# wgmath/wgmath

Hardware: AMD Instinct MI355X
Metric: gemm_tflops (higher is better)
Workload: dtype f16

## Files before the change

include/wgebra_hip.h:

```cpp
#ifndef WGEBRA_HIP_H
#define WGEBRA_HIP_H

#include <stddef.h>
#include <stdint.h>

#ifdef __cplusplus
extern "C" {
#endif

#define WGEBRA_HIP_ABI_VERSION 5

typedef enum wg_status {
    WG_OK = 0,
    WG_ERR_DIM_MISMATCH = 1,
    WG_ERR_PRECONDITION = 2,
    WG_ERR_INVALID_ARG = 3,
    WG_ERR_OUT_OF_BOUNDS = 4,
    WG_ERR_HIP = 5,
    WG_ERR_UNSUPPORTED = 6,
    WG_ERR_NO_DEVICE = 7,
    WG_ERR_WORKSPACE = 8,
    WG_ERR_ALIASED = 9
} wg_status;

typedef enum wg_dtype { WG_F32 = 0, WG_F16 = 1, WG_BF16 = 2 } wg_dtype;

typedef enum wg_gemm_variant {
    WG_GEMM = 0, WG_GEMM_FAST = 1, WG_GEMM_TR = 2, WG_GEMM_TR_FAST = 3
} wg_gemm_variant;

typedef enum wg_gemv_variant {
    WG_GEMV = 0, WG_GEMV_FAST = 1, WG_GEMV_TR = 2, WG_GEMV_TR_FAST = 3
} wg_gemv_variant;

typedef enum wg_reduce_op {
    WG_REDUCE_MIN = 0, WG_REDUCE_MAX = 1, WG_REDUCE_SUM = 2, WG_REDUCE_PROD = 3, WG_REDUCE_SQNORM = 4
} wg_reduce_op;

typedef enum wg_op_assign_variant {
    WG_OP_ADD = 0, WG_OP_SUB = 1, WG_OP_MUL = 2, WG_OP_DIV = 3, WG_OP_COPY = 4
} wg_op_assign_variant;

enum {
    WG_USAGE_MAP_READ = 1u << 0, WG_USAGE_MAP_WRITE = 1u << 1, WG_USAGE_COPY_SRC = 1u << 2,
    WG_USAGE_COPY_DST = 1u << 3, WG_USAGE_INDEX = 1u << 4, WG_USAGE_VERTEX = 1u << 5,
    WG_USAGE_UNIFORM = 1u << 6, WG_USAGE_STORAGE = 1u << 7, WG_USAGE_INDIRECT = 1u << 8,
    WG_USAGE_QUERY_RESOLVE = 1u << 9
};

typedef struct wg_view_shape {
    uint32_t size[3];
    uint32_t stride;
    uint32_t stride_mat;
    uint32_t offset;
} wg_view_shape;

typedef struct wg_ctx wg_ctx;
typedef struct wg_buf wg_buf;
typedef struct wg_cmdbuf wg_cmdbuf;
typedef struct wg_timestamps wg_timestamps;

int wg_abi_version(void);
const char *wg_last_error_string(void);
int wg_device_count(void);

int wg_ctx_create(int device, wg_ctx **out);
int wg_ctx_create_on_stream(int device, void *hip_stream, wg_ctx **out);
int wg_ctx_create_with_cu_count(int device, uint32_t cu_count, wg_ctx **out);
int wg_ctx_create_with_cu_count_one_xcd(int device, uint32_t cu_count, wg_ctx **out);
int wg_ctx_destroy(wg_ctx *ctx);
int wg_ctx_sync(wg_ctx *ctx);
int wg_ctx_device(const wg_ctx *ctx);
void *wg_ctx_stream(const wg_ctx *ctx);
int wg_ctx_device_info(const wg_ctx *ctx, char *name256, int *compute_units, int *clock_mhz, uint64_t *hbm_bytes);
int wg_ctx_mem_info(const wg_ctx *ctx, uint64_t *free_bytes, uint64_t *total_bytes);
typedef enum wg_geom_op {
    WG_GEOM_INV = 0, WG_GEOM_CHOLESKY = 1, WG_GEOM_LU = 2, WG_GEOM_QR = 3, WG_GEOM_SYM_EIGEN = 4, WG_GEOM_SVD = 5,
    WG_GEOM_ROT2 = 6, WG_GEOM_QUAT = 7, WG_GEOM_SIM2 = 8, WG_GEOM_SIM3 = 9,
    WG_GEOM_QUAT_RAW = 10, WG_GEOM_ROT2_RAW = 11, WG_GEOM_SIM2_RAW = 12, WG_GEOM_SIM3_RAW = 13, WG_GEOM_FROM = 14,
    WG_GEOM_UTILS = 15, WG_GEOM_ROT2_EXT = 16, WG_GEOM_EIGVALS2 = 17, WG_GEOM_SVD_RECOMPOSE = 18
} wg_geom_op;
int wg_geometry_apply(wg_ctx *ctx, wg_geom_op op, uint32_t dim, const wg_buf *in, wg_buf *out, uint32_t count);

int wg_debug_spin(wg_ctx *ctx, uint32_t blocks, uint32_t usec, wg_buf *start_ticks);
int wg_debug_clock_begin(wg_ctx *ctx);
int wg_debug_clock_end(wg_ctx *ctx, double *ghz_mean, double *ghz_min, double *ghz_max, double *seconds);
int wg_debug_mfma_ceiling(wg_ctx *ctx, double min_seconds, double *tflops, double *clock_ghz);
int wg_debug_take_path(wg_ctx *ctx, char *buf, size_t cap);

typedef enum wg_tuning {
    WG_TUNE_F16_TILE = 0,
    WG_TUNE_F16_SCHED = 1,
    WG_TUNE_F32_SKINNY = 2,
    WG_TUNE_F32_PANELS = 3,
    WG_TUNE_F16_BALANCE = 4,
    WG_TUNE_F32_MID = 5,
    WG_TUNE_F32_MID_SPLIT = 6,
    WG_TUNE_GEMVT_LDS = 7,
    WG_TUNE_F16_CONT = 8,
    WG_TUNE_RM_TR_NATIVE = 9,
    WG_TUNE_COUNT_ = 10
} wg_tuning;
int wg_ctx_set_tuning(wg_ctx *ctx, wg_tuning key, int value);
int wg_ctx_f16_balance_info(const wg_ctx *ctx, double *rel8, int *valid, uint32_t *updates, uint32_t *balanced_launches);
int wg_debug_f16_balance_plan(const double *rel8, uint32_t tiles, uint32_t stages, int forced, uint32_t *units, uint32_t capacity, uint32_t *nunits,
                              uint32_t *nworkgroups);
typedef struct wg_gemm16_query {
    uint32_t trans, M, N, K, nmats;
    uint32_t lda, ldb, ldc;
    uint64_t a_batch, b_batch, c_batch;
    uint32_t a_addr, b_addr, c_addr;
    float alpha, beta;
    uint32_t panels;
    uint32_t panel_cols, panel_n_main, panel_n_tail, panel_tail_cols[8];
    uint32_t cus;
    int32_t tile, sched, cont, balance;
    uint32_t uneven_xcds;
    uint32_t recording;
    uint32_t bal_valid;
    uint32_t padded;
} wg_gemm16_query;
typedef enum wg_gemm16_leaf {
    WG_GEMM16_SKINNY = 0,
    WG_GEMM16_T256X128 = 1,
    WG_GEMM16_T128 = 2,
    WG_GEMM16_M16 = 3,
    WG_GEMM16_PAD = 4,
    WG_GEMM16_GENERIC = 5,
    WG_GEMM16_UNSUPPORTED = 6
} wg_gemm16_leaf;
typedef struct wg_gemm16_plan {
    uint32_t leaf;
    uint32_t tiles_m, tiles_n;
    uint32_t nsplit, k_per_split;
    uint32_t c_stream, a_nt;
    uint64_t workspace_bytes;
    uint32_t cont;
    uint32_t queues;
    uint32_t nwg;
    uint32_t bal_eligible, bal_calib, bal_wanted;
    uint32_t tail, tail_split, tail_kps;
    uint32_t Mp, Kp, a_ok, b_ok, c_ok;
    uint32_t c_seed;
    int32_t status;
    char message[128];
} wg_gemm16_plan;
int wg_debug_gemm16_plan(const wg_gemm16_query *query, const char *prefix, wg_gemm16_plan *plan, char *tags, size_t cap, wg_gemm16_query *inner);
int wg_debug_gemm_out32_query(wg_gemm16_query *query);
typedef struct wg_gemm32_query {
    uint32_t trans, M, N, K, nmats;
    uint32_t lda, ldb, ldc;
    uint64_t a_batch, b_batch, c_batch;
    float alpha, beta;
    uint32_t cus;
    int32_t mid, mid_split, skinny, panels;
} wg_gemm32_query;
typedef enum wg_gemm32_leaf {
    WG_GEMM32_NOTHING = 0,
    WG_GEMM32_UNSUPPORTED = 1,
    WG_GEMM32_MID = 2,
    WG_GEMM32_SKINNY = 3,
    WG_GEMM32_SKINNY_PANELS = 4,
    WG_GEMM32_SKINNY_T = 5,
    WG_GEMM32_FEWROW = 6,
    WG_GEMM32_BIG = 7
} wg_gemm32_leaf;
typedef struct wg_gemm32_plan {
    uint32_t leaf;
    uint32_t bm, bn;
    uint32_t nsplit, k_per_split;
    uint32_t npanels;
    uint32_t copy_a;
    uint32_t tail_r, tail_sp, tail_kps;
    uint32_t flat_tiles;
    uint64_t workspace_bytes;
    uint64_t pad_workspace_bytes;
    int32_t status;
    char message[128];
} wg_gemm32_plan;
int wg_debug_gemm32_plan(const wg_gemm32_query *query, wg_gemm32_plan *plan, char *tags, size_t cap, wg_gemm32_query *inner);
typedef struct wg_gemv_q8_query {
    uint32_t trans;
    uint32_t rows, cols, nrhs, mats;
    uint32_t group_rows;
    uint32_t ldm, lds, ldv, ldo;
    uint64_t m_batch, s_batch, v_batch, o_batch;
    uint32_t m_addr16, v_addr16, o_addr16;
    uint32_t cus;
} wg_gemv_q8_query;
typedef enum wg_gemv_q8_leaf {
    WG_GEMV_Q8_NOTHING = 0,
    WG_GEMV_Q8_UNSUPPORTED = 1,
    WG_GEMV_Q8_T = 2,
    WG_GEMV_Q8_N = 3,
    WG_GEMV_Q8_ANY_T = 4,
    WG_GEMV_Q8_ANY_N = 5
} wg_gemv_q8_leaf;
typedef struct wg_gemv_q8_plan {
    uint32_t leaf;
    uint32_t rhs_tile, rhs_groups;
    uint32_t loads, cols;
    uint32_t nsplit, k_per_split;
    uint32_t out_per_block;
    uint32_t grid[3], block;
    uint64_t workspace_bytes;
    int32_t status;
    char message[128];
} wg_gemv_q8_plan;
int wg_debug_gemv_q8_plan(const wg_gemv_q8_query *query, wg_gemv_q8_plan *plan, char *tags, size_t cap);
typedef struct wg_gemv_q4_query {
    uint32_t trans;
    uint32_t rows, cols, nrhs, mats;
    uint32_t group_rows;
    uint32_t ldm, lds, ldv, ldo;
    uint64_t m_batch, s_batch, v_batch, o_batch;
    uint32_t m_addr16, v_addr16;
    uint32_t cus;
} wg_gemv_q4_query;
typedef enum wg_gemv_q4_leaf {
    WG_GEMV_Q4_NOTHING = 0,
    WG_GEMV_Q4_UNSUPPORTED = 1,
    WG_GEMV_Q4_T = 2,
    WG_GEMV_Q4_ANY_T = 3
} wg_gemv_q4_leaf;
typedef struct wg_gemv_q4_plan {
    uint32_t leaf;
    uint32_t rhs_tile, rhs_groups;
    uint32_t loads, cols;
    uint32_t nsplit, k_per_split;
    uint32_t out_per_block;
    uint32_t grid[3], block;
    uint64_t workspace_bytes;
    int32_t status;
    char message[128];
} wg_gemv_q4_plan;
int wg_debug_gemv_q4_plan(const wg_gemv_q4_query *query, wg_gemv_q4_plan *plan, char *tags, size_t cap);
typedef struct wg_gemm_q8_query {
    uint32_t k, outputs, n, mats;
    uint32_t group_rows;
    uint32_t x_bf16;
    uint32_t ldm, lds, ldx, ldo;
    uint64_t m_batch, s_batch, x_batch, o_batch;
    uint32_t m_addr16, x_addr16, o_addr16;
    uint32_t cus;
} wg_gemm_q8_query;
typedef enum wg_gemm_q8_leaf {
    WG_GEMM_Q8_NOTHING = 0,
    WG_GEMM_Q8_UNSUPPORTED = 1,
    WG_GEMM_Q8_MFMA = 2,
    WG_GEMM_Q8_ANY = 3
} wg_gemm_q8_leaf;
typedef struct wg_gemm_q8_plan {
    uint32_t leaf;
    uint32_t col_tiles, col_passes;
    uint32_t out_per_block;
    uint32_t nsplit, k_per_split;
    uint32_t grid[3], block;
    uint64_t workspace_bytes;
    int32_t status;
    char message[128];
} wg_gemm_q8_plan;
int wg_debug_gemm_q8_plan(const wg_gemm_q8_query *query, wg_gemm_q8_plan *plan, char *tags, size_t cap);
typedef struct wg_gemm_q8a8_query {
    uint32_t k, outputs, n, mats;
    uint32_t group_rows, x_group_rows;
    uint32_t ldm, lds, ldx, ldxs, ldo;
    uint64_t m_batch, s_batch, x_batch, xs_batch, o_batch;
    uint32_t m_addr16, x_addr16, o_addr16;
    uint32_t cus;
} wg_gemm_q8a8_query;
typedef enum wg_gemm_q8a8_leaf {
    WG_GEMM_Q8A8_NOTHING = 0,
    WG_GEMM_Q8A8_UNSUPPORTED = 1,
    WG_GEMM_Q8A8_MFMA = 2,
    WG_GEMM_Q8A8_ANY = 3
} wg_gemm_q8a8_leaf;
typedef struct wg_gemm_q8a8_plan {
    uint32_t leaf;
    uint32_t col_tiles, col_passes;
    uint32_t out_per_block;
    uint32_t nsplit, k_per_split;
    uint32_t grid[3], block;
    uint64_t workspace_bytes;
    int32_t status;
    char message[128];
} wg_gemm_q8a8_plan;
int wg_debug_gemm_q8a8_plan(const wg_gemm_q8a8_query *query, wg_gemm_q8a8_plan *plan, char *tags, size_t cap);
typedef struct wg_quantize_q8_query {
    uint32_t rows, cols, mats, group_rows, src_elem;
    uint32_t ldq, ldsrc;
    uint64_t q_batch, src_batch;
    uint32_t q_addr16, src_addr16;
} wg_quantize_q8_query;
typedef enum wg_quantize_q8_leaf {
    WG_QUANTIZE_Q8_NOTHING = 0,
    WG_QUANTIZE_Q8_UNSUPPORTED = 1,
    WG_QUANTIZE_Q8_VEC = 2,
    WG_QUANTIZE_Q8_ANY = 3
// ... 249 lines not shown
```

wgmath_amd/_lib.py:

```python
from __future__ import annotations

import ctypes
import os
import re

_PKG = os.path.dirname(os.path.abspath(__file__))
LIB_PATH = os.environ.get("WGEBRA_HIP_LIB") or os.path.join(_PKG, "libwgebra_hip.so")
HEADER_PATH = os.path.join(os.path.dirname(_PKG), "include", "wgebra_hip.h")

WG_OK, WG_ERR_DIM_MISMATCH, WG_ERR_PRECONDITION, WG_ERR_INVALID_ARG, WG_ERR_OUT_OF_BOUNDS, WG_ERR_HIP, \
    WG_ERR_UNSUPPORTED, WG_ERR_NO_DEVICE, WG_ERR_WORKSPACE, WG_ERR_ALIASED = range(10)
WG_VIEWS_OVERLAP_MAX_RUNS = 4096
WG_GATHER_RCCL, WG_GATHER_NONE, WG_GATHER_PEER_STAGED = 0, 2, 3
WG_COMM_ID_BYTES, WG_IPC_HANDLE_BYTES = 128, 96
ABI_VERSION = 5
WG_F32, WG_F16, WG_BF16 = 0, 1, 2
WG_TUNE_F16_TILE, WG_TUNE_F16_SCHED, WG_TUNE_F32_SKINNY, WG_TUNE_F32_PANELS, WG_TUNE_F16_BALANCE, WG_TUNE_F32_MID, WG_TUNE_F32_MID_SPLIT, WG_TUNE_GEMVT_LDS, WG_TUNE_F16_CONT, WG_TUNE_RM_TR_NATIVE = range(10)


class ViewShapeC(ctypes.Structure):
    _fields_ = [("size", ctypes.c_uint32 * 3), ("stride", ctypes.c_uint32), ("stride_mat", ctypes.c_uint32),
                ("offset", ctypes.c_uint32)]


assert ctypes.sizeof(ViewShapeC) == 24


class Gemm16QueryC(ctypes.Structure):
    _fields_ = ([(n, ctypes.c_uint32) for n in ("trans", "M", "N", "K", "nmats", "lda", "ldb", "ldc")]
                + [(n, ctypes.c_uint64) for n in ("a_batch", "b_batch", "c_batch")]
                + [(n, ctypes.c_uint32) for n in ("a_addr", "b_addr", "c_addr")]
                + [("alpha", ctypes.c_float), ("beta", ctypes.c_float)]
                + [(n, ctypes.c_uint32) for n in ("panels", "panel_cols", "panel_n_main", "panel_n_tail")]
                + [("panel_tail_cols", ctypes.c_uint32 * 8), ("cus", ctypes.c_uint32)]
                + [(n, ctypes.c_int32) for n in ("tile", "sched", "cont", "balance")]
                + [(n, ctypes.c_uint32) for n in ("uneven_xcds", "recording", "bal_valid", "padded")])


GEMM16_LEAVES = ("skinny", "t256x128", "t128", "m16", "pad", "generic", "unsupported")


class Gemm16PlanC(ctypes.Structure):
    _fields_ = ([(n, ctypes.c_uint32) for n in ("leaf", "tiles_m", "tiles_n", "nsplit", "k_per_split", "c_stream", "a_nt")]
                + [("workspace_bytes", ctypes.c_uint64)]
                + [(n, ctypes.c_uint32) for n in ("cont", "queues", "nwg", "bal_eligible", "bal_calib", "bal_wanted", "tail", "tail_split", "tail_kps",
                                                   "Mp", "Kp", "a_ok", "b_ok", "c_ok", "c_seed")]
                + [("status", ctypes.c_int32), ("message", ctypes.c_char * 128)])


class Gemm32QueryC(ctypes.Structure):
    _fields_ = ([(n, ctypes.c_uint32) for n in ("trans", "M", "N", "K", "nmats", "lda", "ldb", "ldc")]
                + [(n, ctypes.c_uint64) for n in ("a_batch", "b_batch", "c_batch")]
                + [("alpha", ctypes.c_float), ("beta", ctypes.c_float), ("cus", ctypes.c_uint32)]
                + [(n, ctypes.c_int32) for n in ("mid", "mid_split", "skinny", "panels")])


GEMM32_LEAVES = ("nothing", "unsupported", "mid", "skinny", "skinny_panels", "skinny_t", "fewrow", "big")


class Gemm32PlanC(ctypes.Structure):
    _fields_ = ([(n, ctypes.c_uint32) for n in ("leaf", "bm", "bn", "nsplit", "k_per_split", "npanels", "copy_a", "tail_r", "tail_sp", "tail_kps", "flat_tiles")]
                + [("workspace_bytes", ctypes.c_uint64), ("pad_workspace_bytes", ctypes.c_uint64)]
                + [("status", ctypes.c_int32), ("message", ctypes.c_char * 128)])


class GemvQ8QueryC(ctypes.Structure):
    _fields_ = ([(n, ctypes.c_uint32) for n in ("trans", "rows", "cols", "nrhs", "mats", "group_rows", "ldm", "lds", "ldv", "ldo")]
                + [(n, ctypes.c_uint64) for n in ("m_batch", "s_batch", "v_batch", "o_batch")]
                + [(n, ctypes.c_uint32) for n in ("m_addr16", "v_addr16", "o_addr16", "cus")])


GEMV_Q8_LEAVES = ("nothing", "unsupported", "t", "n", "any_t", "any_n")


class GemvQ8PlanC(ctypes.Structure):
    _fields_ = ([(n, ctypes.c_uint32) for n in ("leaf", "rhs_tile", "rhs_groups", "loads", "cols", "nsplit", "k_per_split", "out_per_block")]
                + [("grid", ctypes.c_uint32 * 3), ("block", ctypes.c_uint32), ("workspace_bytes", ctypes.c_uint64)]
                + [("status", ctypes.c_int32), ("message", ctypes.c_char * 128)])


class GemvQ4QueryC(ctypes.Structure):
    _fields_ = ([(n, ctypes.c_uint32) for n in ("trans", "rows", "cols", "nrhs", "mats", "group_rows", "ldm", "lds", "ldv", "ldo")]
                + [(n, ctypes.c_uint64) for n in ("m_batch", "s_batch", "v_batch", "o_batch")]
                + [(n, ctypes.c_uint32) for n in ("m_addr16", "v_addr16", "cus")])


GEMV_Q4_LEAVES = ("nothing", "unsupported", "t", "any_t")


class GemvQ4PlanC(ctypes.Structure):
    _fields_ = ([(n, ctypes.c_uint32) for n in ("leaf", "rhs_tile", "rhs_groups", "loads", "cols", "nsplit", "k_per_split", "out_per_block")]
                + [("grid", ctypes.c_uint32 * 3), ("block", ctypes.c_uint32), ("workspace_bytes", ctypes.c_uint64)]
                + [("status", ctypes.c_int32), ("message", ctypes.c_char * 128)])


class GemmQ8QueryC(ctypes.Structure):
    _fields_ = ([(n, ctypes.c_uint32) for n in ("k", "outputs", "n", "mats", "group_rows", "x_bf16", "ldm", "lds", "ldx", "ldo")]
                + [(n, ctypes.c_uint64) for n in ("m_batch", "s_batch", "x_batch", "o_batch")]
                + [(n, ctypes.c_uint32) for n in ("m_addr16", "x_addr16", "o_addr16", "cus")])


GEMM_Q8_LEAVES = ("nothing", "unsupported", "mfma", "any")


class GemmQ8PlanC(ctypes.Structure):
    _fields_ = ([(n, ctypes.c_uint32) for n in ("leaf", "col_tiles", "col_passes", "out_per_block", "nsplit", "k_per_split")]
                + [("grid", ctypes.c_uint32 * 3), ("block", ctypes.c_uint32), ("workspace_bytes", ctypes.c_uint64)]
                + [("status", ctypes.c_int32), ("message", ctypes.c_char * 128)])


class GemmQ8A8QueryC(ctypes.Structure):
    _fields_ = ([(n, ctypes.c_uint32) for n in ("k", "outputs", "n", "mats", "group_rows", "x_group_rows", "ldm", "lds", "ldx", "ldxs", "ldo")]
                + [(n, ctypes.c_uint64) for n in ("m_batch", "s_batch", "x_batch", "xs_batch", "o_batch")]
                + [(n, ctypes.c_uint32) for n in ("m_addr16", "x_addr16", "o_addr16", "cus")])


GEMM_Q8A8_LEAVES = ("nothing", "unsupported", "mfma", "any")


class GemmQ8A8PlanC(ctypes.Structure):
    _fields_ = ([(n, ctypes.c_uint32) for n in ("leaf", "col_tiles", "col_passes", "out_per_block", "nsplit", "k_per_split")]
                + [("grid", ctypes.c_uint32 * 3), ("block", ctypes.c_uint32), ("workspace_bytes", ctypes.c_uint64)]
                + [("status", ctypes.c_int32), ("message", ctypes.c_char * 128)])


class QuantizeQ8QueryC(ctypes.Structure):
    _fields_ = ([(n, ctypes.c_uint32) for n in ("rows", "cols", "mats", "group_rows", "src_elem", "ldq", "ldsrc")]
                + [(n, ctypes.c_uint64) for n in ("q_batch", "src_batch")]
                + [(n, ctypes.c_uint32) for n in ("q_addr16", "src_addr16")])


QUANTIZE_Q8_LEAVES = ("nothing", "unsupported", "vec", "any")


class QuantizeQ8PlanC(ctypes.Structure):
    _fields_ = ([(n, ctypes.c_uint32) for n in ("leaf", "group_lanes", "blocks_per_col")]
                + [("grid", ctypes.c_uint32 * 3), ("block", ctypes.c_uint32)]
                + [("status", ctypes.c_int32), ("message", ctypes.c_char * 128)])


class GemmQ4QueryC(ctypes.Structure):
    _fields_ = ([(n, ctypes.c_uint32) for n in ("k", "outputs", "n", "mats", "group_rows", "x_bf16", "ldm", "lds", "ldx", "ldo")]
                + [(n, ctypes.c_uint64) for n in ("m_batch", "s_batch", "x_batch", "o_batch")]
                + [(n, ctypes.c_uint32) for n in ("m_addr16", "x_addr16", "o_addr16", "cus")])


GEMM_Q4_LEAVES = ("nothing", "unsupported", "mfma", "any")


class GemmQ4PlanC(ctypes.Structure):
    _fields_ = ([(n, ctypes.c_uint32) for n in ("leaf", "step", "col_tiles", "col_passes", "out_per_block", "nsplit", "k_per_split")]
                + [("grid", ctypes.c_uint32 * 3), ("block", ctypes.c_uint32), ("workspace_bytes", ctypes.c_uint64)]
                + [("status", ctypes.c_int32), ("message", ctypes.c_char * 128)])


class GemvQueryC(ctypes.Structure):
    _fields_ = ([(n, ctypes.c_uint32) for n in ("trans", "rows_out", "k", "nrhs", "nmats", "m_elem", "v_elem", "bf16", "gemm16", "ldm", "ldv", "ldo")]
                + [(n, ctypes.c_uint64) for n in ("m_batch", "v_batch", "o_batch")]
                + [(n, ctypes.c_uint32) for n in ("m_addr16", "v_addr16", "cus")] + [("gemvt_lds", ctypes.c_int32)])


GEMV_LEAVES = ("nothing", "unsupported", "small", "n", "t", "tcols", "tlds", "as_gemm32", "as_gemm16")


class GemvPlanC(ctypes.Structure):
    _fields_ = ([(n, ctypes.c_uint32) for n in ("leaf", "rhs_tile", "rhs_groups", "e", "u", "v", "rl", "lds_cols", "lds_threads", "lds_kc", "lds_bytes", "nsplit", "k_per_split")]
                + [("grid", ctypes.c_uint32 * 3), ("block", ctypes.c_uint32), ("combine_grid", ctypes.c_uint32 * 3), ("workspace_bytes", ctypes.c_uint64)]
                + [("status", ctypes.c_int32), ("message", ctypes.c_char * 128), ("gemm32", Gemm32PlanC)])


class GemvAnyPlanC(ctypes.Structure):
    _fields_ = ([(n, ctypes.c_uint32) for n in ("launch", "nsplit", "per_split", "grid_x", "zchunk", "nchunks", "nt")] + [("workspace_bytes", ctypes.c_uint64)]
                + [("status", ctypes.c_int32), ("message", ctypes.c_char * 128), ("tag", ctypes.c_char * 48)])


class WgError(RuntimeError):

    def __init__(self, status: int, message: str):
        super().__init__(message)
        self.status = status


class DimensionMismatch(WgError, AssertionError):
    """What the reference raises as a panic from assert_eq!(..., "... dimension mismatch.")."""


class PreconditionFailed(WgError, AssertionError):
    pass


class NoDevice(WgError):
    pass


class WorkspaceMustGrow(WgError):
    """A context scratch region would have to grow inside a recording (WG_ERR_WORKSPACE): run the call once eagerly first."""


class AliasedOperands(WgError):
    """The written view of a call shares memory with a view the call reads (WG_ERR_ALIASED): nothing was launched. The reference gets a wgpu validation panic
    for binding one buffer read_write and read; here views of one buffer are legal as long as their footprints are disjoint, and OpAssign / Axpy take the
    identical view on both sides (include/wgebra_hip.h, the aliasing rule)."""


def declared_symbols(header_path: str = HEADER_PATH) -> list[str]:
    text = open(header_path).read()
    text = re.sub(r"/\*.*?\*/", "", text, flags=re.S)
    return sorted(set(re.findall(r"\b(wg_[a-z0-9_]+)\s*\(", text)))


def _load() -> ctypes.CDLL:
    if not os.path.exists(LIB_PATH):
        raise ImportError(
            f"{LIB_PATH} is missing: build it with `python -c 'import __graft_entry__ as g; g.build()'` "
            f"or `make -C wgmath_amd/csrc`. There is no CPU fallback.")
    lib = ctypes.CDLL(LIB_PATH)
    pd = ctypes.POINTER(ctypes.c_double)
    vp, cp, ci, u32, u64, sz = ctypes.c_void_p, ctypes.c_char_p, ctypes.c_int, ctypes.c_uint32, ctypes.c_uint64, ctypes.c_size_t
    pvp = ctypes.POINTER(vp)
    S = ViewShapeC
    sig = {
        "wg_abi_version": (ci, []),
        "wg_last_error_string": (cp, []),
        "wg_device_count": (ci, []),
        "wg_ctx_create": (ci, [ci, pvp]),
        "wg_ctx_create_on_stream": (ci, [ci, vp, pvp]),
        "wg_ctx_create_with_cu_count": (ci, [ci, ctypes.c_uint32, ctypes.POINTER(vp)]),
        "wg_ctx_create_with_cu_count_one_xcd": (ci, [ci, ctypes.c_uint32, ctypes.POINTER(vp)]),
        "wg_ctx_destroy": (ci, [vp]),
        "wg_ctx_sync": (ci, [vp]),
        "wg_ctx_device": (ci, [vp]),
        "wg_ctx_stream": (vp, [vp]),
        "wg_ctx_device_info": (ci, [vp, cp, ctypes.POINTER(ci), ctypes.POINTER(ci), ctypes.POINTER(u64)]),
        "wg_ctx_mem_info": (ci, [vp, ctypes.POINTER(u64), ctypes.POINTER(u64)]),
        "wg_ctx_reserve_workspace": (ci, [vp, sz]),
        "wg_debug_f16_balance_plan": (ci, [ctypes.POINTER(ctypes.c_double), u32, u32, ci, ctypes.POINTER(u32), u32, ctypes.POINTER(u32), ctypes.POINTER(u32)]),
        "wg_debug_gemm16_plan": (ci, [ctypes.POINTER(Gemm16QueryC), cp, ctypes.POINTER(Gemm16PlanC), cp, sz, ctypes.POINTER(Gemm16QueryC)]),
        "wg_debug_gemm32_plan": (ci, [ctypes.POINTER(Gemm32QueryC), ctypes.POINTER(Gemm32PlanC), cp, sz, ctypes.POINTER(Gemm32QueryC)]),
        "wg_ctx_f16_balance_info": (ci, [vp, ctypes.POINTER(ctypes.c_double), ctypes.POINTER(ci), ctypes.POINTER(u32), ctypes.POINTER(u32)]),
        "wg_debug_views_overlap": (ci, [S, u64, S, u64, u32, ctypes.POINTER(ci)]),
        "wg_debug_take_path": (ci, [vp, cp, sz]),
        "wg_ctx_set_tuning": (ci, [vp, ci, ci]),
        "wg_ctx_get_tuning": (ci, [vp, ci, ctypes.POINTER(ci)]),
        "wg_debug_spin": (ci, [vp, ctypes.c_uint32, ctypes.c_uint32, vp]),
        "wg_geometry_apply": (ci, [vp, ci, ctypes.c_uint32, vp, vp, ctypes.c_uint32]),
        "wg_buf_create": (ci, [vp, sz, u32, pvp]),
        "wg_buf_create_init": (ci, [vp, vp, sz, u32, pvp]),
        "wg_buf_wrap": (ci, [vp, vp, sz, pvp]),
        "wg_buf_destroy": (ci, [vp]),
        "wg_buf_size": (sz, [vp]),
        "wg_buf_device_ptr": (vp, [vp]),
        "wg_buf_write": (ci, [vp, vp, sz, vp, sz]),
        "wg_buf_read": (ci, [vp, vp, sz, vp, sz]),
        "wg_buf_copy": (ci, [vp, vp, sz, vp, sz, sz]),
        "wg_buf_fill_zero": (ci, [vp, vp]),
        "wg_gemm": (ci, [vp, ci, ci, vp, S, vp, S, vp, S]),
        "wg_gemm_ex": (ci, [vp, ci, ci, ctypes.c_float, ctypes.c_float, vp, S, vp, S, vp, S]),
        "wg_gemv": (ci, [vp, ci, ci, vp, S, vp, S, vp, S]),
        "wg_gemv_mixed": (ci, [vp, ci, ci, vp, S, vp, S, vp, S]),
        "wg_gemv_q8": (ci, [vp, ci, u32, vp, S, vp, S, vp, S, vp, S]),
        "wg_debug_gemv_q8_plan": (ci, [ctypes.POINTER(GemvQ8QueryC), ctypes.POINTER(GemvQ8PlanC), cp, sz]),
        "wg_gemv_q4": (ci, [vp, ci, u32, vp, S, vp, S, vp, S, vp, S]),
        "wg_debug_gemv_q4_plan": (ci, [ctypes.POINTER(GemvQ4QueryC), ctypes.POINTER(GemvQ4PlanC), cp, sz]),
        "wg_gemm_q8": (ci, [vp, ci, u32, ci, vp, S, vp, S, vp, S, vp, S]),
        "wg_debug_gemm_q8_plan": (ci, [ctypes.POINTER(GemmQ8QueryC), ctypes.POINTER(GemmQ8PlanC), cp, sz]),
        "wg_gemm_q4": (ci, [vp, ci, u32, ci, vp, S, vp, S, vp, S, vp, S]),
        "wg_debug_gemm_q4_plan": (ci, [ctypes.POINTER(GemmQ4QueryC), ctypes.POINTER(GemmQ4PlanC), cp, sz]),
        "wg_gemm_q8a8": (ci, [vp, ci, u32, u32, vp, S, vp, S, vp, S, vp, S, vp, S]),
        "wg_debug_gemm_q8a8_plan": (ci, [ctypes.POINTER(GemmQ8A8QueryC), ctypes.POINTER(GemmQ8A8PlanC), cp, sz]),
        "wg_quantize_q8": (ci, [vp, ci, u32, vp, S, vp, S, vp, S]),
        "wg_debug_quantize_q8_plan": (ci, [ctypes.POINTER(QuantizeQ8QueryC), ctypes.POINTER(QuantizeQ8PlanC)]),
        "wg_debug_gemv_plan": (ci, [ctypes.POINTER(GemvQueryC), ctypes.POINTER(GemvPlanC), cp, sz]),
        "wg_debug_gemv_any_plan": (ci, [ctypes.POINTER(GemvQueryC), ctypes.POINTER(GemvAnyPlanC), cp, sz]),
        "wg_gemm_out32": (ci, [vp, ci, ci, ctypes.c_float, ctypes.c_float, vp, S, vp, S, vp, S]),
        "wg_debug_gemm_out32_query": (ci, [ctypes.POINTER(Gemm16QueryC)]),
        "wg_gemm_rm": (ci, [vp, ci, ci, vp, S, vp, S, vp, S]),
        "wg_gemv_rm": (ci, [vp, ci, ci, vp, S, vp, S, vp, S]),
        "wg_gemv_reduce": (ci, [vp, ci, ci, ci, vp, vp, S, vp, S]),
        "wg_reduce": (ci, [vp, ci, ci, vp, S, vp]),
        "wg_reduce_fast": (ci, [vp, ci, ci, vp, S, vp]),
        "wg_reduce_batched": (ci, [vp, ci, ci, vp, S, vp]),
        "wg_op_assign": (ci, [vp, ci, ci, vp, S, vp, S]),
        "wg_axpy": (ci, [vp, ctypes.c_float, ci, vp, S, vp, S]),
        "wg_copy_view": (ci, [vp, ci, vp, S, vp, S]),
        "wg_debug_clock_begin": (ci, [vp]),
        "wg_debug_clock_end": (ci, [vp, pd, pd, pd, pd]),
        "wg_debug_mfma_ceiling": (ci, [vp, ctypes.c_double, pd, pd]),
        "wg_comm_unique_id": (ci, [vp]),
        "wg_comm_create": (ci, [vp, ci, ci, vp, pvp]),
        "wg_comm_destroy": (ci, [vp]),
        "wg_comm_rank": (ci, [vp]),
        "wg_comm_size": (ci, [vp]),
        "wg_comm_has_collectives": (ci, [vp]),
        "wg_comm_reported_size": (ci, [vp, ctypes.POINTER(ci)]),
        "wg_comm_bytes_sent": (u64, [vp]),
        "wg_all_gather": (ci, [vp, ci, vp, u64, u64]),
        "wg_comm_join": (ci, [vp]),
        "wg_comm_set_pipelined": (ci, [vp, ci]),
        "wg_comm_set_one_launch": (ci, [vp, ci]),
        "wg_comm_flush": (ci, [vp]),
        "wg_comm_barrier": (ci, [vp]),
        "wg_buf_ipc_export": (ci, [vp, vp]),
        "wg_buf_ipc_open": (ci, [vp, vp, pvp]),
        "wg_comm_stage_reserve": (ci, [vp, sz, pvp, pvp]),
        "wg_comm_set_peer_stages": (ci, [vp, pvp, pvp]),
        "wg_cube_to_matrix": (ci, [vp, ci, vp, S, vp, S]),
        "wg_gemm_sharded": (ci, [vp, ci, ci, ci, u32, vp, S, vp, S, vp, S]),
        "wg_comm_set_wait_timing": (ci, [vp, ci]),
        "wg_comm_wait_times": (ci, [vp, ctypes.POINTER(u32), ctypes.POINTER(ctypes.c_float), u32, ctypes.POINTER(u32)]),
        "wg_gemm_sharded_panels": (ci, [vp, ci, ci, ci, ctypes.POINTER(u32), u32, vp, S, vp, S, vp, S]),
        "wg_encoder_begin": (ci, [vp]),
        "wg_encoder_finish": (ci, [vp, pvp]),
        "wg_queue_submit": (ci, [vp, vp]),
        "wg_cmdbuf_destroy": (ci, [vp]),
        "wg_timestamps_create": (ci, [vp, u32, pvp]),
        "wg_timestamps_destroy": (ci, [vp]),
        "wg_timestamps_clear": (ci, [vp]),
        "wg_timestamps_write": (ci, [vp, vp, ctypes.POINTER(u32)]),
        "wg_timestamps_reserve": (ci, [vp, u32, ctypes.POINTER(u32)]),
        "wg_timestamps_write_at": (ci, [vp, vp, u32]),
        "wg_timestamps_len": (u32, [vp]),
        "wg_timestamps_wait_for_results_ms": (ci, [vp, ctypes.POINTER(ctypes.c_double), u32]),
    }
    for name, (res, args) in sig.items():
        fn = getattr(lib, name)
        fn.restype = res
        fn.argtypes = args
    lib._wg_signatures = sig
    if lib.wg_abi_version() != ABI_VERSION:
        raise ImportError(f"{LIB_PATH} reports ABI version {lib.wg_abi_version()}, this binding is written for {ABI_VERSION} "
                          f"(include/wgebra_hip.h: WGEBRA_HIP_ABI_VERSION): rebuild with `make -C wgmath_amd/csrc`")
    return lib


def hip_runtime_paths() -> list[str]:
    paths = set()
    try:
        with open("/proc/self/maps") as f:
            for line in f:
                if "libamdhip64" in line:
                    paths.add(line.split()[-1])
    except OSError:
        pass
    return sorted(paths)


def assert_single_hip_runtime() -> None:
    p = hip_runtime_paths()
    if len(p) > 1:
        raise ImportError("two HIP runtimes are loaded in this process: " + ", ".join(p) +
                          ". Import torch BEFORE wgmath_amd so that libwgebra_hip.so binds to torch's bundled runtime.")


lib = _load()

_EXC = {WG_ERR_DIM_MISMATCH: DimensionMismatch, WG_ERR_PRECONDITION: PreconditionFailed, WG_ERR_NO_DEVICE: NoDevice, WG_ERR_WORKSPACE: WorkspaceMustGrow,
        WG_ERR_ALIASED: AliasedOperands}


def check(status: int) -> None:
    if status != WG_OK:
        msg = lib.wg_last_error_string().decode("utf-8", "replace")
        raise _EXC.get(status, WgError)(status, msg or f"wg_status {status}")
```

wgmath_amd/csrc/gemm16_plan.hip:

```cpp
#include "gemm16_plan.hpp"
#include "gemm_plan_common.hpp"

#include <cmath>
#include <cstdarg>
#include <cstring>
#include <string>

using wg16::BalancePlan;
using wg16::bal_decode;
using WG16_NS::BM;
using WG16_NS::BN;
using WG16_NS::BKH;
using WG16_NS::kPanelTail;

namespace {
constexpr double kBalTileOverhead = 5.0;
constexpr double kBalTakeOverhead = 8.5;
constexpr double kBalGiveOverhead = 7.0;
}

uint32_t bal_plan(const double rel[8], uint32_t tiles, uint32_t S, bool forced, BalancePlan &bp) {
    uint32_t n[8];
    double w[8], delta[8], sum_w = 0, sum_inv = 0;
    for (int x = 0; x < 8; ++x) {
        n[x] = tiles / 8u + ((uint32_t)x < tiles % 8u ? 1u : 0u);
        w[x] = ((double)S + kBalTileOverhead) * n[x] / 32.0;
        sum_w += w[x];
        sum_inv += 1.0 / rel[x];
    }
    const double T = sum_w / sum_inv;
    for (int x = 0; x < 8; ++x) delta[x] = T / rel[x] - w[x];
    double want[8], rem[8];
    for (int x = 0; x < 8; ++x) {
        want[x] = delta[x] > 0 ? delta[x] - kBalTakeOverhead : 0.0;
        rem[x] = delta[x] < 0 ? -delta[x] + kBalGiveOverhead : 0.0;
    }
    if (forced) {
        const double s = (double)S, take[8] = { s / 3, 0, s / 2, s / 4, 0, 0, s / 4, 0 }, give[8] = { 0, s / 4, 0, 0, 0, s / 2, 0, s / 2 + s / 4 };
        for (int x = 0; x < 8; ++x) want[x] = take[x], rem[x] = give[x];
    }
    uint32_t rounds_used[8] = { 0 }, max_rounds[8], pairs = 0;
    for (int x = 0; x < 8; ++x) {
        const uint32_t r = n[x] / 64u;
        max_rounds[x] = r > 2u ? 2u : r;
        if (n[x] < 64u) max_rounds[x] = n[x] >= 4u ? 2u : (n[x] >= 2u ? 1u : 0u);
        bp.len[x] = n[x];
        bp.pre_cnt[x] = 0; bp.pre_src[x] = 0; bp.pre_p[x] = bp.pre_slot[x] = bp.pre_pair0[x] = 0;
        for (int r2 = 0; r2 < 2; ++r2) bp.suf_lo[x][r2] = bp.suf_p[x][r2] = bp.suf_pair0[x][r2] = 0, bp.suf_cnt[x][r2] = 0;
    }
    bool taken[8] = { false };
    for (;;) {
        int f = -1;
        for (int x = 0; x < 8; ++x)
            if (!taken[x] && want[x] >= 3.0 && (f < 0 || want[x] > want[f])) f = x;
        if (f < 0) break;
        taken[f] = true;
        int g = -1;
        for (int x = 0; x < 8; ++x)
            if (rem[x] >= 3.0 && rounds_used[x] < max_rounds[x] && (g < 0 || rem[x] > rem[g])) g = x;
        if (g < 0) break;
        double pd = want[f];
        if (pd > rem[g]) pd = rem[g];
        uint32_t p = (uint32_t)(pd + 0.5);
        if (p + 3u > S) p = S - 3u;
        if (p < 3u) continue;
        if (!forced && (double)p < kBalGiveOverhead + 1.0) continue;
        const uint32_t round = n[g] >= 64u ? 32u : (n[g] >= 4u ? n[g] / 4u : 1u);
        const uint32_t cnt = round < 32u ? round : 32u;
        const uint32_t lo = n[g] - round * (rounds_used[g] + 1u);
        if (pairs + cnt > kBalMaxPairs) break;
        bp.pre_cnt[f] = cnt; bp.pre_src[f] = (uint32_t)g; bp.pre_p[f] = p; bp.pre_slot[f] = lo; bp.pre_pair0[f] = pairs;
        bp.len[f] = n[f] + cnt;
        const uint32_t r2 = rounds_used[g]++;
        bp.suf_lo[g][r2] = lo; bp.suf_cnt[g][r2] = cnt; bp.suf_p[g][r2] = p; bp.suf_pair0[g][r2] = pairs;
        pairs += cnt;
        rem[g] -= (double)p;
    }
    return pairs;
}

uint32_t gemm16_c_stream(const wg_gemm16_query &q, uint32_t out_elem_bytes) {
#ifdef WG_FORCE_C_STREAM
    return WG_FORCE_C_STREAM;
#endif
    const uint64_t MiB = 1ull << 20, ab = ((uint64_t)q.M * q.K + (uint64_t)q.K * q.N) * q.nmats * 2u, cb = (uint64_t)q.M * q.N * q.nmats * out_elem_bytes;
    return (q.beta == 0.f && ab <= 256u * MiB && ab + cb > 256u * MiB) ? 1u : 0u;
}

wg_gemm16_query gemm16_out32_query(wg_gemm16_query q) {
    q.cont = 0;
    q.panels = 0; q.panel_cols = q.panel_n_main = q.panel_n_tail = 0;
    for (int t = 0; t < 8; ++t) q.panel_tail_cols[t] = 0;
    return q;
}

namespace {
wg_gemm16_plan no_launch(wg_gemm16_plan p, int status, const char *fmt = nullptr, ...) {
    p.leaf = WG_GEMM16_UNSUPPORTED;
    p.status = status;
    if (fmt) {
        va_list ap;
        va_start(ap, fmt);
        vsnprintf(p.message, sizeof p.message, fmt, ap);
        va_end(ap);
    }
    return p;
}
uint64_t pad_elems(uint64_t elems) { return (elems + 7u) & ~7ull; }
}

wg_gemm16_plan gemm16_plan(const wg_gemm16_query &q) {
    wg_gemm16_plan p = {};
    p.nsplit = 1; p.tail_split = 1;
    const bool trans = q.trans != 0, panels = q.panels != 0;
    const uint32_t M = q.M, N = q.N, K = q.K, nmats = q.nmats, out_ld = q.ldc;
    const uint64_t out_batch = q.c_batch;
    const struct { uint32_t ld; uint64_t batch; uint32_t addr; } m1 = { q.lda, q.a_batch, q.a_addr }, m2 = { q.ldb, q.b_batch, q.b_addr };
    const float alpha = q.alpha, beta = q.beta;
    const int cus = (int)q.cus;
    p.k_per_split = K; p.tail_kps = K;
    if (M == 0 || N == 0 || nmats == 0) return no_launch(p, panels ? WG_ERR_UNSUPPORTED : WG_OK);
    if (nmats > 65535) return no_launch(p, WG_ERR_UNSUPPORTED, "Gemm: more than 65535 matrices in one call");
    {
        const uint64_t MiB = 1ull << 20;
        p.c_stream = gemm16_c_stream(q, 2u);
        p.a_nt = (!trans && N <= 128u && (uint64_t)M * K * 2u >= 384u * MiB) ? 1u : 0u;
    }
    auto al16 = [](uint32_t addr) { return (addr & 15) == 0; };
#ifndef WG_F16_SKINNY
#define WG_F16_SKINNY 1
#endif
    if (WG_F16_SKINNY && trans && !panels && N <= 16u && M >= 512u && M % 4u == 0 && K >= 256u && K % 8u == 0 && m1.ld % 8u == 0 && m2.ld % 8u == 0 &&
        out_ld % 4u == 0 && al16(m1.addr) && al16(m2.addr) && (q.c_addr & 7) == 0 && (nmats == 1 || (m1.batch % 8u == 0 && m2.batch % 8u == 0 && out_batch % 4u == 0)) &&
        (uint64_t)M * K * 2u >= (16ull << 20) && (uint64_t)m1.ld * 32u * 2u < (1ull << 31) && (uint64_t)m2.ld * 32u * 2u < (1ull << 31)) {
        const uint32_t row_blocks = (M + 127u) / 128u;
        uint32_t kps;
        const uint32_t ns = wg_skinny_kcut(M, N, K, nmats, (uint64_t)row_blocks * nmats, (uint64_t)cus, 256u, 64u, 0, &kps);
        if (ns > 65535u || nmats > 65535u) return no_launch(p, WG_ERR_UNSUPPORTED, "Gemm: too many splits or matrices for the skinny path");
        p.leaf = WG_GEMM16_SKINNY;
        p.tiles_m = row_blocks; p.tiles_n = 1;
        p.nsplit = ns; p.k_per_split = kps;
        if (ns > 1) p.workspace_bytes = (uint64_t)ns * M * N * nmats * sizeof(float);
        return p;
    }
    const bool off_ok = (uint64_t)m1.ld * 2u * (trans ? 256u : 32u) < (1ull << 31) && (uint64_t)m2.ld * 2u * 256u < (1ull << 31);
    const uint32_t krem = K % 64u;
    const bool k_big = K % 8u == 0 && K - krem >= 192u, k_small = K % 8u == 0 && K - krem >= 64u;
    const bool a_step_fits = trans || (uint64_t)m1.ld * 64u < (1ull << 32);
    auto al4 = [](uint32_t addr) { return (addr & 3) == 0; };
    const bool a_al = al4(m1.addr) && m1.ld % 2 == 0 && (nmats == 1 || m1.batch % 2 == 0), b_al = al4(m2.addr) && m2.ld % 2 == 0 && (nmats == 1 || m2.batch % 2 == 0);
    const bool fast = (M % 8 == 0) && (k_big || k_small) && a_step_fits && off_ok && a_al && b_al;
    auto panels_ok = [&]() -> bool {
        if (!q.panel_cols || q.panel_cols % 256u || q.panel_n_tail < 1 || q.panel_n_tail > (uint32_t)kPanelTail || q.panel_n_main + q.panel_n_tail < 2) return false;
        uint64_t c0 = (uint64_t)q.panel_n_main * q.panel_cols;
        for (uint32_t t = 0; t + 1u < q.panel_n_tail; ++t) {
            if (q.panel_tail_cols[t] == 0 || q.panel_tail_cols[t] % 256u || q.panel_tail_cols[t] / 256u > 255u) return false;
            c0 += q.panel_tail_cols[t];
        }
        return c0 < N && N - c0 == q.panel_tail_cols[q.panel_n_tail - 1u] && (N - c0 + 255u) / 256u <= 255u;
    };
    if (panels && !(fast && k_big && nmats == 1 && alpha == 1.f && beta == 0.f && panels_ok() &&
                    (uint64_t)((M + BM - 1) / BM) * ((N + BN - 1) / BN) >= (uint64_t)cus))
        return no_launch(p, WG_ERR_UNSUPPORTED);
    if (fast) {
        p.tiles_m = (M + BM - 1) / BM;
        p.tiles_n = (N + BN - 1) / BN;
        const uint64_t tiles = (uint64_t)p.tiles_m * p.tiles_n;
        if (tiles > 0x7fffffffull) return no_launch(p, WG_ERR_UNSUPPORTED, "Gemm: too many tiles");
        bool t256x128 = q.tile == 256128;
        const bool cont_shape = !panels && krem == 0 && K >= 256u && K <= 4096u && tiles * nmats > (uint64_t)cus && beta == 0.f &&
                                q.cont != 0 && q.sched < 0 && q.balance != 1;
        if (q.tile == 0 && !panels && tiles * nmats >= (uint64_t)cus && K <= 1536u) {
            double t_big = (double)((tiles * nmats + cus - 1) / cus) * (12.3 + 0.0213 * K);
            if (cont_shape) {
                const double per = 5.7 + 0.0211 * K;
                const uint64_t all = tiles * nmats;
                const uint32_t r = (uint32_t)(all % (uint64_t)cus);
                t_big = 5.0 + (double)(all / (uint64_t)cus) * per + (r == 0 ? 0.0 : (2u * r <= (uint32_t)cus && K >= 384u && nmats == 1 ? 25.0 + 0.0107 * K : per));
            }
            const double r2 = (double)((uint64_t)((M + 255u) / 256u) * ((N + 127u) / 128u) * nmats) / (2.0 * cus), fl = floor(r2), fr = r2 - fl;
            const double pair = trans ? 5.7 + 0.027 * K : 6.1 + 0.0263 * K;
            t256x128 = fl * pair + (fr > 0.0 ? (fr <= 0.5 ? 0.6 : 1.0) * pair : 0.0) < 0.95 * t_big;
        }
        if (q.tile == 0 && !panels && nmats <= 2u && tiles * nmats < (uint64_t)cus && K >= 512u && K <= 4096u) {
            const uint64_t tt = (uint64_t)((M + 255u) / 256u) * ((N + 127u) / 128u) * nmats;
            if (tt <= (uint64_t)cus && 10u * tt >= 7u * (uint64_t)cus) t256x128 = true;
        }
        if ((krem == 0 || K - krem >= 64u) && !panels && t256x128) {
            const uint32_t tm = (M + 255u) / 256u, tn = (N + 127u) / 128u;
            const uint64_t tiles_t = (uint64_t)tm * tn;
            if (tiles_t <= 0x7fffffffull && nmats <= 65535u) {
                p.leaf = WG_GEMM16_T256X128;
                p.tiles_m = tm; p.tiles_n = tn;
                return p;
            }
        }
        if ((krem == 0 || K - krem >= 64u) && !panels) {
            const double out_bytes = (double)M * N * nmats * 4.0;
            auto slabs = [&](uint32_t ns) { return ns > 1 ? wg_slab_write_us(ns * out_bytes) + wg_slab_reduce_us(ns * out_bytes) : 0.0; };
            const uint32_t tm = (M + 127u) / 128u, tn = (N + 127u) / 128u;
            const uint64_t tiles128 = (uint64_t)tm * tn;
            uint32_t ns = 1;
            if (tiles128 * nmats * 2u <= (uint64_t)cus) {
                ns = (uint32_t)((uint64_t)cus / (tiles128 * nmats));
                if (ns > K / 1024u) ns = K / 1024u;
                while (ns > 1 && (double)ns * out_bytes > (double)(512ull << 20)) --ns;
                if (ns < 2) ns = 1;
            }
#ifdef WG_T128_FORCE_NS
            if (tiles128 * nmats <= (uint64_t)cus && K >= 1024u) ns = WG_T128_FORCE_NS;
#endif
            bool want128 = false;
            if (!k_big) want128 = true;
            else if (q.tile) want128 = q.tile == 128;
            else if (N <= 64u) want128 = true;
            else if (tiles * nmats < (uint64_t)cus) {
                const double w128 = (double)(tiles128 * nmats * ns) / cus, k128 = (double)(((K / 64u + ns - 1) / ns) * 64u);
                const double est128 = (w128 <= 1.0 ? k128 * 0.00875 : w128 * k128 * 0.0108) + 6.0 + slabs(ns);
                const uint32_t ns256 = wg_splitk_plan(tiles * nmats, (uint32_t)cus, K / BKH, 8, (uint64_t)M * N * nmats, 512ull << 20);
                const double k256 = (double)(((K / BKH + ns256 - 1) / ns256) * BKH);
                const double est256 = (ns256 <= 4u ? 0.8 : 1.0) * ((double)((tiles * nmats * ns256 + cus - 1) / cus) * (k256 * 0.0234 + 8.0) + slabs(ns256));
                want128 = est128 < est256;
            }
            if (want128 && tiles128 <= 0x7fffffffull) {
                const uint32_t kps = ns > 1 ? ((K / 64u + ns - 1) / ns) * 64u : K;
                if (ns > 1) ns = (K - krem + kps - 1) / kps;
                if ((uint64_t)nmats * ns <= 65535) {
                    p.leaf = WG_GEMM16_T128;
                    p.tiles_m = tm; p.tiles_n = tn;
                    p.nsplit = ns; p.k_per_split = kps;
                    if (ns > 1) p.workspace_bytes = (uint64_t)ns * M * N * nmats * sizeof(float);
                    return p;
                }
            }
        }
        if (!k_big) return no_launch(p, WG_ERR_UNSUPPORTED, "Gemm: K = %u with %u matrices does not fit the 128 x 128 kernel's launch", K, nmats);
        uint32_t nsplit = panels ? 1u : wg_splitk_plan(tiles * nmats, (uint32_t)cus, K / BKH, 8, (uint64_t)M * N * nmats, 512ull << 20);
        const uint32_t stages = K / 64u;
        auto kps_of = [&](uint32_t ns) { return ((stages + ns - 1u) / ns) * 64u; };
        while (nsplit > 1) {
            const uint32_t kps = kps_of(nsplit), n = (K - krem + kps - 1u) / kps;
            if (n == nsplit && kps >= 192u && K - krem - (n - 1u) * kps >= 192u) break;
            nsplit = n < nsplit ? n : nsplit - 1u;
        }
        p.leaf = WG_GEMM16_M16;
        p.nsplit = nsplit;
        p.k_per_split = nsplit > 1 ? kps_of(nsplit) : K;
        if (nsplit > 1) p.workspace_bytes = (uint64_t)nsplit * M * N * nmats * sizeof(float);
        if ((uint64_t)nmats * nsplit > 65535) return no_launch(p, WG_ERR_UNSUPPORTED, "Gemm: nmats * splits exceeds 65535");
        uint32_t tail = 0, tail_split = 1, tail_kps = K;
#ifndef WG_F16_TAIL_SPLIT
#define WG_F16_TAIL_SPLIT 1
#endif
        if (WG_F16_TAIL_SPLIT && nsplit == 1 && nmats == 1 && tiles > (uint64_t)cus && !panels) {
            const uint32_t r = (uint32_t)(tiles % (uint64_t)cus);
            if (r > 0 && r * 2u <= (uint32_t)cus) {
                uint32_t sp = (uint32_t)cus / r;
                if (sp > stages / 3u) sp = stages / 3u;
                while (sp >= 2) {
                    const uint32_t kps = ((stages + sp - 1) / sp) * 64u;
                    const uint32_t n = (K - krem + kps - 1) / kps, last = K - krem - (n - 1) * kps;
                    if (n >= 2 && last >= 192u && (size_t)n * r * 65536u * sizeof(float) <= (512ull << 20)) { tail = r; tail_split = n; tail_kps = kps; break; }
                    --sp;
                }
            }
        }
        p.tail = tail; p.tail_split = tail_split; p.tail_kps = tail_kps;
        if (tail) p.workspace_bytes = (uint64_t)tail_split * tail * 65536u * sizeof(float);
#ifndef WG_F16_SCHED_ROUNDS
#define WG_F16_SCHED_ROUNDS 16
#endif
        const uint32_t ntiles = (uint32_t)tiles - tail;
        p.nwg = ntiles;
        const int sched_env = q.sched;
        {
            const int cont = q.cont;
            const uint64_t all = (uint64_t)ntiles * nmats;
            const bool applies = nsplit == 1 && !panels && krem == 0 && K >= 256u && all > (uint64_t)cus && all <= 0x7fffffffull && beta == 0.f;
            const bool by_rule = (K <= 4096u || (K <= 8192u && all < (uint64_t)(WG_F16_SCHED_ROUNDS * cus))) && !q.uneven_xcds && sched_env < 0 && q.balance != 1;
            if (cont != 0 && applies && (cont == 1 || by_rule)) {
                p.cont = 1;
                p.nwg = (uint32_t)cus;
                return p;
            }
        }
        const bool dyn = nsplit == 1 && nmats == 1 && (sched_env >= 0 ? sched_env != 0 : ntiles >= (uint32_t)((q.uneven_xcds ? 2 : WG_F16_SCHED_ROUNDS) * cus));
        if (dyn) {
            p.queues = 1;
            p.nwg = (ntiles + ntiles / 8u + 7u) & ~7u;
        }
        const int bal_knob = q.balance;
        const uint32_t S = K / 64u;
        if (bal_knob != 0 && !dyn && !panels && nsplit == 1 && nmats == 1 && cus == 256 && ntiles >= 16u && ntiles < 8u * 65535u && S >= 8u) {
            p.bal_eligible = 1;
            p.bal_calib = ntiles >= (uint32_t)cus;
            const bool want = bal_knob == 1 || (bal_knob < 0 && q.bal_valid && ntiles >= 2u * (uint32_t)cus);
            p.bal_wanted = want && !q.recording;
        }
        return p;
    } else if (!q.padded && (uint64_t)M * N * K >= (1ull << 24) && K > 0 && nmats <= 65535u) {
        const bool k_ok = k_big || k_small;
        const uint32_t Mp = (M + 7u) & ~7u, Kp = k_ok ? K : ((K + 63u) & ~63u);
        const bool a_ok = k_ok && M == Mp && a_al;
        const bool b_ok = k_ok && b_al;
        const bool c_ok = M == Mp;
        const uint64_t a_elems = a_ok ? 0 : (uint64_t)Mp * Kp, b_elems = b_ok ? 0 : (uint64_t)Kp * N, c_elems = c_ok ? 0 : (uint64_t)Mp * N;
        const uint64_t a_sz = pad_elems(a_elems), b_sz = pad_elems(b_elems), c_sz = pad_elems(c_elems);
        p.leaf = WG_GEMM16_PAD;
        p.Mp = Mp; p.Kp = Kp; p.a_ok = a_ok; p.b_ok = b_ok; p.c_ok = c_ok;
        p.c_seed = !c_ok && beta != 0.f;
        p.workspace_bytes = (a_sz + b_sz + c_sz) * nmats * 2u + 16;
        return p;
    } else {
        p.leaf = WG_GEMM16_GENERIC;
        p.tiles_m = (M + 63) / 64;
        p.tiles_n = (N + 63) / 64;
        if (p.tiles_n > 65535) return no_launch(p, WG_ERR_UNSUPPORTED, "Gemm: N too large for the generic f16 path");
        return p;
    }
}

wg_gemm16_query gemm16_pad_inner(const wg_gemm16_query &q, const wg_gemm16_plan &p) {
    wg_gemm16_query in = q;
    in.padded = 1;
    in.M = p.Mp; in.K = p.Kp;
    if (!p.a_ok) { in.lda = q.trans ? p.Kp : p.Mp; in.a_batch = pad_elems((uint64_t)p.Mp * p.Kp); in.a_addr = 0; }
    if (!p.b_ok) { in.ldb = p.Kp; in.b_batch = pad_elems((uint64_t)p.Kp * q.N); in.b_addr = 0; }
    if (!p.c_ok) { in.ldc = p.Mp; in.c_batch = pad_elems((uint64_t)p.Mp * q.N); in.c_addr = 0; }
    return in;
}

Gemm16Tags gemm16_tags(const wg_gemm16_plan &p, const char *prefix, bool bal_on) {
    Gemm16Tags t = {};
    auto add = [&](const char *fmt, auto... a) { snprintf(t.tag[t.n++], sizeof t.tag[0], fmt, prefix, a...); };
    switch (p.leaf) {
    case WG_GEMM16_SKINNY: add("%s.skinny/ns=%u", p.nsplit); break;
    case WG_GEMM16_T256X128: add("%s.t256x128"); break;
    case WG_GEMM16_T128: add("%s.t128/ns=%u", p.nsplit); break;
    case WG_GEMM16_M16:
        if (p.cont) add("%s.cont");
        else add("%s.m16%s/ns=%u", bal_on ? "bal" : p.queues ? "q" : "", p.nsplit);
        if (p.tail) { add("%s.m16tail/ns=%u", p.tail_split); add("%s.tail_reduce"); }
        break;
    case WG_GEMM16_PAD: add("%s.pad%s>", p.c_ok ? "" : p.c_seed ? "/c=seed" : "/c"); break;
    case WG_GEMM16_GENERIC: add("%s.generic"); break;
    default: break;
    }
    return t;
}

extern "C" int wg_debug_f16_balance_plan(const double *rel8, uint32_t tiles, uint32_t stages, int forced, uint32_t *units, uint32_t capacity, uint32_t *nunits,
                                          uint32_t *nworkgroups) {
    if (!rel8 || !nunits || (capacity && !units)) return wg_set_error(WG_ERR_INVALID_ARG, "wg_debug_f16_balance_plan: NULL argument");
    BalancePlan bp = BalancePlan{};
    const uint32_t pairs = bal_plan(rel8, tiles, stages, forced != 0, bp);
    (void)pairs;
    uint32_t mx = 0, n = 0;
    for (int x = 0; x < 8; ++x) mx = bp.len[x] > mx ? bp.len[x] : mx;
    for (uint32_t b = 0; b < 8u * mx; ++b) {
        uint32_t tile, mode, kb, ns, pair;
        if (!bal_decode(bp, b, stages, tile, mode, kb, ns, pair)) continue;
        if (n < capacity) { units[5 * n] = tile; units[5 * n + 1] = mode; units[5 * n + 2] = kb; units[5 * n + 3] = mode ? ns : stages; units[5 * n + 4] = pair; }
        ++n;
    }
    *nunits = n;
    if (nworkgroups) *nworkgroups = 8u * mx;
    return WG_OK;
}

extern "C" int wg_debug_gemm16_plan(const wg_gemm16_query *query, const char *prefix, wg_gemm16_plan *plan, char *tags, size_t cap, wg_gemm16_query *inner) {
    if (!query || !prefix || !plan || (cap && !tags)) return wg_set_error(WG_ERR_INVALID_ARG, "wg_debug_gemm16_plan: NULL argument");
    *plan = gemm16_plan(*query);
    if (inner) *inner = plan->leaf == WG_GEMM16_PAD ? gemm16_pad_inner(*query, *plan) : *query;
    std::string log;
    wg_gemm16_query q = *query;
    for (wg_gemm16_plan p = *plan;; p = gemm16_plan(q)) {
        bool bal_on = false;
        if (p.leaf == WG_GEMM16_M16 && p.bal_wanted) {
            const double flat[8] = { 1, 1, 1, 1, 1, 1, 1, 1 };
            BalancePlan bp = BalancePlan{};
            bal_on = bal_plan(flat, p.nwg, q.K / 64u, q.balance == 1, bp) != 0;
        }
        const Gemm16Tags t = gemm16_tags(p, prefix, bal_on);
        for (int i = 0; i < t.n; ++i) {
            if (!log.empty() && log.back() != '>') log += ' ';
            log += t.tag[i];
        }
        if (p.leaf != WG_GEMM16_PAD) {
            if (p.nsplit > 1) log += " splitk.reduce/ns=" + std::to_string(p.nsplit);
            break;
        }
        q = gemm16_pad_inner(q, p);
    }
    if (cap) snprintf(tags, cap, "%s", log.c_str());
    return WG_OK;
}

extern "C" int wg_debug_gemm_out32_query(wg_gemm16_query *query) {
    if (!query) return wg_set_error(WG_ERR_INVALID_ARG, "wg_debug_gemm_out32_query: NULL argument");
    *query = gemm16_out32_query(*query);
    return WG_OK;
}

extern "C" int wg_ctx_f16_balance_info(const wg_ctx *ctx, double *rel8, int *valid, uint32_t *updates, uint32_t *balanced_launches) {
    if (!ctx) return wg_set_error(WG_ERR_INVALID_ARG, "wg_ctx_f16_balance_info: ctx is NULL");
    if (rel8) for (int x = 0; x < 8; ++x) rel8[x] = ctx->bal.rel[x];
    if (valid) *valid = ctx->bal.valid ? 1 : 0;
    if (updates) *updates = ctx->bal.updates;
    if (balanced_launches) *balanced_launches = ctx->bal.epoch;
    return WG_OK;
}
```

wgmath_amd/csrc/gemm_f16.hip:

```cpp
#include "gemm_f16_common.hpp"
#include "gemm16_plan.hpp"

namespace WG16_NS {
namespace {

#ifndef WG_NN_KEEP
#define WG_NN_KEEP 16
#endif
#ifndef WG_NN_DSTRIDE
#define WG_NN_DSTRIDE 8
#endif
#ifndef WG_NN_DOFF
#define WG_NN_DOFF 3
#endif
#ifndef WG_NN_SYNC_SLOT
#define WG_NN_SYNC_SLOT 60
#endif
#ifndef WG_TN_SYNC_SLOT
#define WG_TN_SYNC_SLOT 56
#endif
#ifndef WG_F16_UNPEELED
#define WG_F16_UNPEELED 1
#endif
#ifndef WG_NN_STAGED
#define WG_NN_STAGED 0
#endif
typedef float floatx4 __attribute__((ext_vector_type(4)));
typedef unsigned uintx2 __attribute__((ext_vector_type(2)));
typedef unsigned uintx4 __attribute__((ext_vector_type(4)));
typedef uintx4 __attribute__((aligned(2))) uintx4_u;

template <class F, int... I>
__device__ __forceinline__ void static_for_impl(F &&f, std::integer_sequence<int, I...>) { (f(std::integral_constant<int, I>{}), ...); }
template <int N, class F>
__device__ __forceinline__ void static_for(F &&f) { static_for_impl(f, std::make_integer_sequence<int, N>{}); }

constexpr int M16_A_RING = 4, M16_B_RING = 3;
constexpr int M16_BS_BYTES = BN * 64 * 2;
constexpr int M16_B_BASE = M16_A_RING * HA_BYTES;
static_assert(M16_B_BASE + M16_B_RING * M16_BS_BYTES == 160 * 1024, "LDS plan");

__device__ __forceinline__ void m16_set_m0(uint32_t lds_dst) {
    if (WG_ABLATE & 2) return;
    asm volatile("s_mov_b32 m0, %0" ::"s"(lds_dst));
}
#ifndef WG_F16_DMA_MUBUF
#define WG_F16_DMA_MUBUF 0
#endif
template <int IMM>
__device__ __forceinline__ void m16_dma_imm(uint32_t voff, const void *sbase) {
    if (WG_ABLATE & 2) return;
    if constexpr (WG_F16_DMA_MUBUF) {
        const uintx4 srd = { (uint32_t)(uintptr_t)sbase, (uint32_t)((uintptr_t)sbase >> 32) & 0xffffu, 0xffffffffu, 0x00020000u };
        asm volatile("buffer_load_dwordx4 %0, %1, 0 offen offset:%c2 lds" ::"v"(voff), "s"(srd), "i"(IMM));
    } else {
        asm volatile("global_load_lds_dwordx4 %0, %1 offset:%c2" ::"v"(voff), "s"(sbase), "i"(IMM));
    }
}
__device__ __forceinline__ void m16_dma(int q, uint32_t voff, const void *sbase) {
    if (q == 0) m16_dma_imm<0>(voff, sbase);
    else if (q == 1) m16_dma_imm<1024>(voff, sbase);
    else if (q == 2) m16_dma_imm<2048>(voff, sbase);
    else m16_dma_imm<3072>(voff, sbase);
}
constexpr uint32_t M16_BIAS = 3072;

template <bool TRANS_A>
__device__ __forceinline__ void m16_tile(const GemmArgs &g, const uint32_t bid, char *const smem, const uint32_t unit_mode = 0, uint32_t unit_kb = 0,
                                         uint32_t unit_ns = 0, const uint32_t unit_pair = 0) {
    const int lane = threadIdx.x & 63;
    const int wave = __builtin_amdgcn_readfirstlane(threadIdx.x >> 6);
    const int wm = wave >> 1, wn = wave & 1;
    const int i16 = lane & 15, kg = lane >> 4;
    const int aq = i16 >> 2, bb = i16 & 3;
    const int gq = (4 - aq) & 3;

#ifdef WG_F16_TRACE
    uint64_t tr_t[5];
    tr_t[0] = __builtin_amdgcn_s_memrealtime();
#define WG_TRACE_POINT(i) do { asm volatile("s_waitcnt lgkmcnt(0)" ::: "memory"); tr_t[i] = __builtin_amdgcn_s_memrealtime(); } while (0)
#else
#define WG_TRACE_POINT(i) do { } while (0)
#endif
#if defined(WG_F16_TRACE) && WG_F16_TRACE >= 2
    uint32_t q_a = 0, q_b = 0, q_c = 0, q_d = 0, s_vm = 0, s_bar = 0, s_probe = 0, m_vm = 0, m_bar = 0, n_adv = 0, loop_t0 = 0, loop_t1 = 0;
#endif
    uint32_t tm, tn, panel = 0;
    uint32_t panel_c0 = 0, panel_np = 0;
    if (g.panel.cols) {
        const uint32_t id = bid + g.tile_base;
        const uint32_t mtn = g.panel.cols / 256u, main_tiles = g.panel.n_main * g.panel.tiles;
        uint32_t loc, ptn, tn0;
        if (id < main_tiles) {
            panel = __builtin_amdgcn_readfirstlane(id / g.panel.tiles);
            loc = id - panel * g.panel.tiles; ptn = mtn; tn0 = panel * mtn;
        } else {
            loc = __builtin_amdgcn_readfirstlane(id - main_tiles);
            tn0 = g.panel.n_main * mtn;
            const uint32_t n_tail = g.panel.npanels - g.panel.n_main;
            uint32_t q = 0;
            uint64_t tail = g.panel.tail_tn;
            ptn = (uint32_t)tail & 0xffu;
            while (q + 1u < n_tail && loc >= g.tiles_m * ptn) { loc -= g.tiles_m * ptn; tn0 += ptn; ++q; tail >>= 8; ptn = (uint32_t)tail & 0xffu; }
            panel = g.panel.n_main + q;
        }
        tile_of(loc, g.tiles_m, ptn, tm, tn);
        tn += tn0;
        panel_c0 = tn0 * 256u;
        panel_np = panel + 1u == g.panel.npanels ? g.N - panel_c0 : ptn * 256u;
    } else tile_of(bid + g.tile_base, g.tiles_m, g.tiles_n, tm, tn);
    panel = __builtin_amdgcn_readfirstlane(panel);
    panel_c0 = __builtin_amdgcn_readfirstlane(panel_c0); panel_np = __builtin_amdgcn_readfirstlane(panel_np);
    tm = __builtin_amdgcn_readfirstlane(tm); tn = __builtin_amdgcn_readfirstlane(tn);
    const uint32_t m0 = tm * BM, n0 = tn * BN;
    const uint32_t z = blockIdx.y / g.nsplit, split = blockIdx.y % g.nsplit;
    uint32_t k_begin = split * g.k_per_split;
    uint32_t K_loc = split + 1u == g.nsplit ? g.K - k_begin : g.k_per_split;
    bool from_partial = false;
    if (unit_mode == 2) {
        if (threadIdx.x == 0) {
            const uint64_t t0 = __builtin_amdgcn_s_memrealtime();
            uint32_t ok = 1;
            while (__hip_atomic_load(g.bal.flags + unit_pair, __ATOMIC_RELAXED, __HIP_MEMORY_SCOPE_SYSTEM) != g.bal.epoch) {
                __builtin_amdgcn_s_sleep(16);
                if (__builtin_amdgcn_s_memrealtime() - t0 > 100000ull) { ok = 0; break; }
            }
            __builtin_amdgcn_fence(__ATOMIC_ACQUIRE, "agent");
            *reinterpret_cast<volatile uint32_t *>(smem) = ok;
        }
        __syncthreads();
        from_partial = __builtin_amdgcn_readfirstlane(*reinterpret_cast<volatile uint32_t *>(smem)) != 0;
        __syncthreads();
    }
    uint32_t rem = 0, rem_k0 = 0;
    if (unit_mode == 1) { k_begin = 0; K_loc = unit_ns * 64u; rem = g.K & 63u; rem_k0 = g.K - rem; }
    else if (unit_mode == 2 && from_partial) { k_begin = unit_kb * 64u; K_loc = (g.K & ~63u) - k_begin; }
    else {
        if (unit_mode == 2) { k_begin = 0; K_loc = g.K; }
        rem = K_loc & 63u; K_loc -= rem; rem_k0 = k_begin + K_loc;
    }
    const wg16_elem_t *A = g.a + z * g.a_batch + (TRANS_A ? (uint64_t)k_begin : (uint64_t)k_begin * g.lda);
    const wg16_elem_t *B = g.b + z * g.b_batch + k_begin;
    wg16_out_t *C = g.c + z * g.c_batch;
    const bool paneled = !kOut32 && g.panel.cols != 0;
    if (paneled) {
        const uint64_t off = (uint64_t)panel_c0 * (g.panel.col_stride - g.ldc) + g.panel.slot_rows * (uint64_t)panel_np - g.panel.slot_rows * (uint64_t)g.panel.cols;
        C += ((uint64_t)(uint32_t)__builtin_amdgcn_readfirstlane((int)(uint32_t)(off >> 32)) << 32) | (uint32_t)__builtin_amdgcn_readfirstlane((int)(uint32_t)off);
    }
    uint32_t *panel_counter = g.panel.counters + panel;
    float *part = unit_mode ? g.bal.part + (uint64_t)unit_pair * 65536u : g.part;
    float alpha = g.alpha, beta = g.beta;
    uint32_t ldc = g.ldc, c_stream = g.c_stream;
    uint32_t *bal_flag = g.bal.flags + unit_pair;
    uint32_t bal_epoch = g.bal.epoch;
    unsigned long long *calib = g.calib;
    asm volatile("" : "+s"(C), "+s"(part), "+s"(alpha), "+s"(beta), "+s"(ldc), "+s"(c_stream), "+s"(bal_flag), "+s"(bal_epoch), "+s"(calib));

    uint32_t a_voff[TRANS_A ? 8 : 4], b_voff[8];
    const wg16_elem_t *a_base, *b_base = B + (uint64_t)n0 * g.ldb;
    if constexpr (TRANS_A) a_base = A + (uint64_t)m0 * g.lda; else a_base = A + m0;
    const uint32_t rem_dk = rem_k0 - k_begin;
    const char *rem_a = TRANS_A ? (const char *)(a_base + rem_dk) : (const char *)(a_base + (uint64_t)rem_dk * g.lda);
    const char *rem_b = (const char *)(b_base + rem_dk);
    if (rem) {
        if constexpr (TRANS_A) a_base -= 64; else a_base -= (uint64_t)64u * g.lda;
        b_base -= 64;
    }
    if constexpr (TRANS_A) {
#pragma unroll
        for (int q = 0; q < 8; ++q) {
            const uint32_t P = 8u * wave + q;
            const uint32_t row = 8u * P + (lane >> 3);
            const uint32_t f = ((4u - ((row >> 3) & 3u)) & 3u) | (((row >> 1) & 1u) << 2);
            const uint32_t chunk = (lane & 7u) ^ f;
            const uint32_t ra = min(row, g.M - 1u - m0);
            a_voff[q] = (ra * g.lda + 8u * chunk) * 2u + (M16_BIAS - 1024u * (q & 3));
        }
    } else {
#pragma unroll
        for (int q = 0; q < 4; ++q) {
            const uint32_t P = 4u * wave + q;
            const uint32_t unit = WG_NN_NOSWAP ? (lane & 3u) ^ ((uint32_t)wave & 1u) : (lane & 3u);
            const uint32_t mpiece = min(128u * (P & 1) + 32u * (lane >> 4) + 8u * unit, g.M - 8u - m0);
            a_voff[q] = ((4u * (P >> 1) + ((lane >> 2) & 3)) * g.lda + mpiece) * 2u + (M16_BIAS - 1024u * q);
        }
    }
#pragma unroll
    for (int q = 0; q < 8; ++q) {
        const uint32_t P = 8u * wave + q;
        const uint32_t row = 8u * P + (lane >> 3);
        const uint32_t f = ((4u - ((row >> 2) & 3u)) & 3u) | (((row >> 1) & 1u) << 2);
        const uint32_t chunk = (lane & 7u) ^ f;
        const uint32_t rb = min(row, g.N - 1u - n0);
        b_voff[q] = (rb * g.ldb + 8u * chunk) * 2u + (M16_BIAS - 1024u * (q & 3));
    }
    const uint32_t lds_base = (uint32_t)(uintptr_t)(WG_AS3 char *)smem;
    const uint32_t lds_a_wave = __builtin_amdgcn_readfirstlane(lds_base + wave * (TRANS_A ? 8192 : 4096));
    const uint32_t lds_b_wave = __builtin_amdgcn_readfirstlane(lds_base + M16_B_BASE + wave * 8192);
    auto a_src = [&](uint32_t H) -> const wg16_elem_t * {
        const char *p0;
        if constexpr (TRANS_A) p0 = (const char *)(a_base + H * 64u); else p0 = (const char *)(a_base + (uint64_t)(H * BKH) * g.lda);
        return (const wg16_elem_t *)(p0 - M16_BIAS);
    };
    auto b_src = [&](uint32_t stage) -> const wg16_elem_t * { return (const wg16_elem_t *)((const char *)(b_base + 64u * stage) - M16_BIAS); };

    uint32_t vbaseA[2], vbaseB[2];
    uint32_t vbaseA1 = 0;
#pragma unroll
    for (int hs = 0; hs < 2; ++hs) {
        const uint32_t chunk = (uint32_t)(((kg ^ gq) | ((hs ^ (bb >> 1)) << 2)) * 16);
        vbaseB[hs] = lds_base + M16_B_BASE + ((uint32_t)128 * wn + i16) * 128u + chunk;
        if constexpr (TRANS_A) vbaseA[hs] = lds_base + (128u * wm + 8u * aq + bb) * 128u + chunk;
    }
    if constexpr (!TRANS_A) {
        if constexpr (WG_NN_NOSWAP) {
            const uint32_t a = (uint32_t)i16 & 3u, krow = (uint32_t)i16 >> 2;
            const uint32_t common = lds_base + (uint32_t)kg * 4096u + (4u * wm) * 256u + krow * 64u + (a ^ ((uint32_t)kg & 1u)) * 16u;
            vbaseA[0] = common + (a & 1u) * 8u;
            vbaseA1 = common + ((a & 1u) ^ 1u) * 8u;
        } else {
            vbaseA[0] = lds_base + (uint32_t)((kg & 2) * 2) * 2048u + (4u * wm) * 256u + (uint32_t)i16 * 16u + (uint32_t)(kg & 1) * 8u;
        }
        vbaseA[1] = vbaseA[0] + HA_BYTES;
    }
    const bool odd_row = !TRANS_A && WG_NN_NOSWAP && (kg & 1);

    floatx4 acc[8][8];
#pragma unroll
    for (int t = 0; t < 8; ++t)
#pragma unroll
        for (int u = 0; u < 8; ++u)
#pragma unroll
            for (int e = 0; e < 4; ++e) acc[t][u][e] = 0.f;
    if (from_partial) {
        const uint32_t pvoff = ((128u * wn + i16) * 256u + 128u * wm + 8u * kg) * 4u;
        const uint32_t pv_even = pvoff + (odd_row ? 16u : 0u), pv_odd = pvoff + (odd_row ? 0u : 16u);
#pragma unroll
        for (int u = 0; u < 8; ++u) {
            const uint32_t vo0 = pv_even + (uint32_t)u * 16384u, vo1 = pv_odd + (uint32_t)u * 16384u;
#pragma unroll
            for (int p = 0; p < 4; ++p) {
                asm volatile("global_load_dwordx4 %0, %1, %2 offset:%c3 sc0 sc1" : "=a"(acc[2 * p][u]) : "v"(vo0), "s"(part), "i"(p * 128));
                asm volatile("global_load_dwordx4 %0, %1, %2 offset:%c3 sc0 sc1" : "=a"(acc[2 * p + 1][u]) : "v"(vo1), "s"(part), "i"(p * 128));
            }
        }
        asm volatile("s_waitcnt vmcnt(0)" ::: "memory");
    }

    uintx4 a_r[2][8];
    half8_t b_f[2][8];

    using c0 = std::integral_constant<int, 0>;
    using c1 = std::integral_constant<int, 1>;
    using yes = std::true_type;
    using no = std::false_type;
    using km1 = std::integral_constant<int, -1>;
    using km2 = std::integral_constant<int, -2>;
    using k0 = std::integral_constant<int, 0>;
    using k4 = std::integral_constant<int, 4>;
    using k8 = std::integral_constant<int, 8>;
    using k12 = std::integral_constant<int, 12>;
    using k16 = std::integral_constant<int, 16>;

    const uint32_t S = K_loc / 64u + (rem ? 1u : 0u);
    uint32_t st = 0;

    uint32_t va, vb;
    uint32_t va1 = 0;
    const char *ga, *gb, *ga2 = nullptr;
    uint32_t oR = 0, oD = 2u * M16_BS_BYTES;
    uint32_t rR = 1u << 14, rD = 0;
    uint32_t oA = 0, oAD = 0;
    uint32_t la = 0, lb = 0;
    const uint64_t a_step = (uint64_t)BKH * g.lda * 2u;
    constexpr bool STAGED = TRANS_A || WG_NN_STAGED;
    const uint32_t a_full = TRANS_A ? 128u : (uint32_t)a_step * (STAGED ? 2u : 1u);
    uint32_t a_inc0 = 0, a_inc1 = 0, b_inc = 0;
    auto ring3 = [](uint32_t o) -> uint32_t { o += (uint32_t)M16_BS_BYTES; return o == 3u * M16_BS_BYTES ? 0u : o; };

    constexpr int kOps = TRANS_A ? 16 : WG_NN_NOSWAP ? 24 : 40;
    auto frag = [&](int op, int set) {
        auto rb = [&](int u) { b_f[set][u] = lds_h8_at(vb + u * 2048); };
        if constexpr (TRANS_A) {
            auto ra = [&](int t) { a_r[set][t] = __builtin_bit_cast(uintx4, lds_h8_at(va + (t & 1) * 512 + (t >> 1) * 4096)); };
            if (op == 0) ra(0);
            else if (op <= 8) rb(op - 1);
            else ra(op - 8);
        } else if constexpr (WG_NN_NOSWAP) {
            auto tr = [&](int p, int i) {
                const int tb = i >> 1, h = i & 1;
                const uintx2 v = __builtin_bit_cast(uintx2, lds_tr_at((tb ? va1 : va) + h * 2048 + p * 256));
                a_r[set][2 * p + tb][2 * h] = v[0];
                a_r[set][2 * p + tb][2 * h + 1] = v[1];
            };
            if (op < 4) tr(0, op);
            else if (op < 8) rb(op - 4);
            else if (op < 12) tr(1, op - 8);
            else if (op < 16) rb(op - 8);
            else if (op < 20) tr(2, op - 16);
            else tr(3, op - 20);
        } else {
            auto tr = [&](int p, int i) {
                const int h = i >> 1, ins = i & 1;
                const uintx2 v = __builtin_bit_cast(uintx2, lds_tr_at(va + (2 * ins + h) * 2048 + p * 256));
                a_r[set][2 * p + ins][2 * h] = v[0];
                a_r[set][2 * p + ins][2 * h + 1] = v[1];
            };
// ... 130 lines not shown
                asm volatile("" : "+s"(ga2));
            }
            if constexpr (HS == 0 && j == LASTB + 1) { oR = ring3(oR); asm volatile("" : "+s"(oR)); }
            if constexpr (j == LASTB + 4) { vb = vbaseB[HS] + oR; asm volatile("" : "+v"(vb)); }
            if constexpr (HS == 0 && j == 47) { oA ^= (uint32_t)M16_BS_BYTES; asm volatile("" : "+s"(oA)); }
            if constexpr (!TRANS_A && WG_NN_NOSWAP && j == 48) { va1 = vbaseA1 + (HS ? (uint32_t)HA_BYTES : 0u) + oA; asm volatile("" : "+v"(va1)); }
            if constexpr (j == 49) { va = vbaseA[HS] + oA; asm volatile("" : "+v"(va)); }
            if constexpr (HS == 1 && j == 52) { ++st; asm volatile("" : "+s"(st)); }
            if constexpr (WG_F16_UNPEELED && HS == 1 && j == 53) { a_inc1 = st + 4u <= S ? a_full : 0u; asm volatile("" : "+s"(a_inc1)); }
            if constexpr (WG_F16_UNPEELED && HS == 1 && j == 54) { b_inc = st + 4u <= S ? 128u : 0u; asm volatile("" : "+s"(b_inc)); }
            if constexpr (j == WG_TN_SYNC_SLOT && SYNC >= -1) sync(sync_c);
            __builtin_amdgcn_sched_barrier(0);
        });
    };

    auto pro_a = [&](int hh) {
#pragma unroll
        for (int q = 0; q < 4; ++q) {
            if (q == 0) { m16_set_m0(lds_a_wave + hh * HA_BYTES); asm volatile("s_nop 0"); }
            m16_dma(q, a_voff[q], a_src(hh));
        }
    };
    auto pro_b = [&](int sb, int nq) {
#pragma unroll
        for (int q = 0; q < 8; ++q) {
            if (q >= nq) break;
            if (sb >= 0) {
                if ((q & 3) == 0) { m16_set_m0(lds_b_wave + sb * M16_BS_BYTES + (q >> 2) * 4096); asm volatile("s_nop 0"); }
                m16_dma(q & 3, b_voff[q], b_src(sb));
            } else if constexpr (TRANS_A) {
                const int sa_ = -1 - sb;
                if ((q & 3) == 0) { m16_set_m0(lds_a_wave + sa_ * M16_BS_BYTES + (q >> 2) * 4096); asm volatile("s_nop 0"); }
                m16_dma(q & 3, a_voff[q], a_src(sa_));
            }
        }
    };
    if (rem) {
        auto put = [&](uint32_t lds_dst, const char *src, bool valid) {
            uintx4 v = { 0u, 0u, 0u, 0u };
            if (valid) v = *reinterpret_cast<const uintx4_u *>(src);
            *(WG_AS3 uintx4 *)(uintptr_t)(lds_dst + 16u * (uint32_t)lane) = v;
        };
        if constexpr (TRANS_A) {
#pragma unroll
            for (int q = 0; q < 8; ++q) {
                const uint32_t row = 8u * (8u * wave + q) + (lane >> 3);
                const uint32_t chunk = (lane & 7u) ^ (((4u - ((row >> 3) & 3u)) & 3u) | (((row >> 1) & 1u) << 2));
                put(lds_a_wave + (uint32_t)(q >> 2) * 4096u + (uint32_t)(q & 3) * 1024u, rem_a + (a_voff[q] - (M16_BIAS - 1024u * (q & 3))), 8u * chunk < rem);
            }
        } else {
#pragma unroll
            for (int h = 0; h < 2; ++h)
#pragma unroll
                for (int q = 0; q < 4; ++q) {
                    const uint32_t k_local = 32u * h + 4u * ((4u * wave + q) >> 1) + ((lane >> 2) & 3u);
                    put(lds_a_wave + (uint32_t)h * HA_BYTES + (uint32_t)q * 1024u, rem_a + (uint64_t)(32u * h) * g.lda * 2u + (a_voff[q] - (M16_BIAS - 1024u * q)), k_local < rem);
                }
        }
#pragma unroll
        for (int q = 0; q < 8; ++q) {
            const uint32_t row = 8u * (8u * wave + q) + (lane >> 3);
            const uint32_t chunk = (lane & 7u) ^ (((4u - ((row >> 2) & 3u)) & 3u) | (((row >> 1) & 1u) << 2));
            put(lds_b_wave + (uint32_t)(q >> 2) * 4096u + (uint32_t)(q & 3) * 1024u, rem_b + (b_voff[q] - (M16_BIAS - 1024u * (q & 3))), 8u * chunk < rem);
        }
        asm volatile("" ::: "memory");
        __builtin_amdgcn_sched_barrier(0);
        if (!(WG_ABLATE & 2)) {
            if constexpr (TRANS_A) { pro_b(-2, 8); pro_b(1, 8); pro_b(2, 4); }
            else { pro_a(2); pro_b(1, 8); pro_a(3); pro_b(2, 4); }
        }
    } else if (!(WG_ABLATE & 2)) {
        if constexpr (TRANS_A) {
            pro_b(-1, 8); pro_b(0, 8);
            pro_b(-2, 8); pro_b(1, 8); pro_b(2, 4);
        } else {
            pro_a(0); pro_b(0, 8); pro_a(1);
            pro_a(2); pro_b(1, 8); pro_a(3); pro_b(2, 4);
        }
    }
    wait_dma_keep<20>();
    __syncthreads();
    va = vbaseA[0]; va1 = vbaseA1; vb = vbaseB[0];
#pragma unroll
    for (int op = 0; op < kOps; ++op) frag(op, 0);
    const uint64_t calib_t0 = __builtin_amdgcn_s_memrealtime();
    __builtin_amdgcn_s_waitcnt(0xc07f);
    if (!(WG_ABLATE & 1)) __builtin_amdgcn_s_barrier();
    vb = vbaseB[1];
    gb = (const char *)b_src(2u);
    if constexpr (TRANS_A) { va = vbaseA[1]; ga = (const char *)a_src(2u); }
    else if constexpr (STAGED) { va = vbaseA[1]; va1 = vbaseA1 + (uint32_t)HA_BYTES; ga = (const char *)a_src(4u); ga2 = (const char *)a_src(5u); }
    else { va = vbaseA[0] + rR; va1 = vbaseA1 + rR; ga = (const char *)a_src(4u); }
    __builtin_amdgcn_sched_barrier(0);
    WG_TRACE_POINT(1);
#if defined(WG_F16_TRACE) && WG_F16_TRACE >= 2
    loop_t0 = (uint32_t)__builtin_amdgcn_s_memtime();
    __builtin_amdgcn_s_waitcnt(0xc07f);
#endif

    const uint32_t s_end = S - 3u;
    if constexpr (WG_F16_UNPEELED) {
        a_inc0 = S >= 3u ? a_full : 0u; a_inc1 = S >= 4u ? a_full : 0u; b_inc = S >= 4u ? 128u : 0u;
        if constexpr (STAGED) {
            while (st < S) {
                half_step_s(c0{}, no{}, yes{}, yes{}, k8{});
                half_step_s(c1{}, yes{}, yes{}, yes{}, km1{});
            }
        } else {
            while (st < S) {
                half_step_nn(c0{}, yes{}, yes{}, yes{}, std::integral_constant<int, WG_NN_KEEP>{});
                half_step_nn(c1{}, yes{}, yes{}, yes{}, std::integral_constant<int, WG_NN_KEEP>{});
            }
        }
    } else if constexpr (STAGED) {
        while (st < s_end) {
            half_step_s(c0{}, no{}, yes{}, yes{}, k8{});
            half_step_s(c1{}, yes{}, yes{}, yes{}, km1{});
        }
        half_step_s(c0{}, no{}, yes{}, yes{}, k8{});
        half_step_s(c1{}, yes{}, no{}, yes{}, km1{});
        half_step_s(c0{}, no{}, no{}, yes{}, k0{});
        half_step_s(c1{}, no{}, no{}, yes{}, km1{});
        half_step_s(c0{}, no{}, no{}, yes{}, km1{});
        half_step_s(c1{}, no{}, no{}, no{}, km2{});
    } else {
        while (st < s_end) {
            half_step_nn(c0{}, yes{}, yes{}, yes{}, std::integral_constant<int, WG_NN_KEEP>{});
            half_step_nn(c1{}, yes{}, yes{}, yes{}, std::integral_constant<int, WG_NN_KEEP>{});
        }
        half_step_nn(c0{}, yes{}, yes{}, yes{}, k16{});
        half_step_nn(c1{}, yes{}, no{}, yes{}, k12{});
        half_step_nn(c0{}, no{}, no{}, yes{}, k4{});
        half_step_nn(c1{}, no{}, no{}, yes{}, k0{});
        half_step_nn(c0{}, no{}, no{}, yes{}, k0{});
        half_step_nn(c1{}, no{}, no{}, no{}, km2{});
    }
    WG_TRACE_POINT(2);
#if defined(WG_F16_TRACE) && WG_F16_TRACE >= 2
    loop_t1 = (uint32_t)__builtin_amdgcn_s_memtime();
    __builtin_amdgcn_s_waitcnt(0xc07f);
#endif
    if (calib) {
        const uint64_t calib_t1 = __builtin_amdgcn_s_memrealtime();
        __builtin_amdgcn_s_waitcnt(0xc07f);
        if (threadIdx.x == 0) {
            const uint32_t x = blockIdx.x & 7u;
            atomicAdd(calib + 2u * x, (unsigned long long)(calib_t1 - calib_t0));
            atomicAdd(calib + 2u * x + 1u, (unsigned long long)S);
        }
    }

    const bool full_tile = (m0 + BM <= g.M) && (n0 + BN <= g.N);
    const uint32_t row0 = m0 + 128u * wm + 8u * kg;
    if (g.tail_tiles > 0 || unit_mode == 1) {
        float *P = unit_mode == 1 ? part : part + ((uint64_t)split * g.tail_tiles + bid) * 65536u;
#pragma unroll
        for (int u = 0; u < 8; ++u) {
            const uint32_t cl = 128u * wn + 16u * u + i16;
            float *pc = P + (uint64_t)cl * 256u + 128u * wm + 8u * kg;
#pragma unroll
            for (int p = 0; p < 4; ++p) {
                float4 *d = reinterpret_cast<float4 *>(pc + 32 * p);
                d[odd_row ? 1 : 0] = make_float4(acc[2 * p][u][0], acc[2 * p][u][1], acc[2 * p][u][2], acc[2 * p][u][3]);
                d[odd_row ? 0 : 1] = make_float4(acc[2 * p + 1][u][0], acc[2 * p + 1][u][1], acc[2 * p + 1][u][2], acc[2 * p + 1][u][3]);
            }
        }
        asm volatile("s_waitcnt vmcnt(0)" ::: "memory");
        if (unit_mode == 1) {
            __syncthreads();
            if (threadIdx.x == 0) {
                __builtin_amdgcn_fence(__ATOMIC_RELEASE, "agent");
                asm volatile("s_waitcnt vmcnt(0)" ::: "memory");
                __hip_atomic_store(bal_flag, bal_epoch, __ATOMIC_RELAXED, __HIP_MEMORY_SCOPE_SYSTEM);
            }
        }
        return;
    }
    if (g.nsplit > 1) {
        float *P = part + ((uint64_t)z * g.nsplit + split) * ((uint64_t)g.M * g.N);
#pragma unroll
        for (int u = 0; u < 8; ++u) {
            const uint32_t col = n0 + 128u * wn + 16u * u + i16;
            if (!full_tile && col >= g.N) continue;
            float *pc = P + (uint64_t)col * g.M + row0;
#pragma unroll
            for (int p = 0; p < 4; ++p) {
                if (!(full_tile || row0 + 32 * p < g.M)) continue;
                float4 *d = reinterpret_cast<float4 *>(pc + 32 * p);
                d[odd_row ? 1 : 0] = make_float4(acc[2 * p][u][0], acc[2 * p][u][1], acc[2 * p][u][2], acc[2 * p][u][3]);
                d[odd_row ? 0 : 1] = make_float4(acc[2 * p + 1][u][0], acc[2 * p + 1][u][1], acc[2 * p + 1][u][2], acc[2 * p + 1][u][3]);
            }
        }
        asm volatile("s_waitcnt vmcnt(0)" ::: "memory");
        return;
    }
#ifndef WG_PANEL_STORE
#define WG_PANEL_STORE 2
#endif
#ifndef WG_EPI_STORE
#define WG_EPI_STORE -1
#endif
    auto pack = [&](int u, int p, bool ok, const wg16_out_t *cc) -> out8_t {
        float r[8];
#pragma unroll
        for (int q = 0; q < 4; ++q) {
            r[q] = odd_row ? acc[2 * p + 1][u][q] : acc[2 * p][u][q];
            r[4 + q] = odd_row ? acc[2 * p][u][q] : acc[2 * p + 1][u][q];
        }
        if (alpha != 1.f) {
#pragma unroll
            for (int q = 0; q < 8; ++q) r[q] *= alpha;
        }
        if (beta != 0.f && ok) {
            const out8_t c = *reinterpret_cast<const out8_u *>(cc + 32 * p);
#pragma unroll
            for (int q = 0; q < 8; ++q) r[q] = fmaf(beta, (float)c[q], r[q]);
        }
        out8_t v;
#pragma unroll
        for (int q = 0; q < 8; ++q) v[q] = (wg16_out_t)r[q];
        return v;
    };
#ifdef WG_GEMM16_OUT32
    auto store8 = [&](float *dst, out8_t v) {
        if (WG_ABLATE & 32) return;
        const floatx4 lo = { v[0], v[1], v[2], v[3] }, hi = { v[4], v[5], v[6], v[7] };
        if (c_stream) {
            asm volatile("global_store_dwordx4 %0, %1, off sc1 nt\n\ts_nop 1" ::"v"(dst), "v"(lo) : "memory");
            asm volatile("global_store_dwordx4 %0, %1, off offset:16 sc1 nt\n\ts_nop 1" ::"v"(dst), "v"(hi) : "memory");
        } else *reinterpret_cast<out8_u *>(dst) = v;
    };
#else
    auto store8 = [&](wg16_elem_t *dst, half8_t v) {
        if (paneled) {
            if constexpr (WG_PANEL_STORE == 0) *reinterpret_cast<half8_u *>(dst) = v;
            else if constexpr (WG_PANEL_STORE == 1) asm volatile("global_store_dwordx4 %0, %1, off sc1\n\ts_nop 1" ::"v"(dst), "v"(v) : "memory");
            else asm volatile("global_store_dwordx4 %0, %1, off sc0 sc1\n\ts_nop 1" ::"v"(dst), "v"(v) : "memory");
        } else if (!(WG_ABLATE & 32)) {
            if constexpr (WG_EPI_STORE == -1) {
                if (c_stream) asm volatile("global_store_dwordx4 %0, %1, off sc1 nt\n\ts_nop 1" ::"v"(dst), "v"(v) : "memory");
                else *reinterpret_cast<half8_u *>(dst) = v;
            } else if constexpr (WG_EPI_STORE == 0) *reinterpret_cast<half8_u *>(dst) = v;
            else if constexpr (WG_EPI_STORE == 1) __builtin_nontemporal_store(v, reinterpret_cast<half8_u *>(dst));
            else if constexpr (WG_EPI_STORE == 2) asm volatile("global_store_dwordx4 %0, %1, off sc1\n\ts_nop 1" ::"v"(dst), "v"(v) : "memory");
            else if constexpr (WG_EPI_STORE == 3) asm volatile("global_store_dwordx4 %0, %1, off sc0 sc1\n\ts_nop 1" ::"v"(dst), "v"(v) : "memory");
            else asm volatile("global_store_dwordx4 %0, %1, off sc1 nt\n\ts_nop 1" ::"v"(dst), "v"(v) : "memory");
        }
    };
#endif
#ifdef WG_GEMM16_OUT32
    if (full_tile && !(WG_ABLATE & 32)) {
#pragma unroll
        for (int u = 0; u < 8; ++u) {
            float *cc = C + (uint64_t)(n0 + 128u * wn + 16u * u + i16) * ldc + row0;
#pragma unroll
            for (int p = 0; p < 4; ++p) {
                const out8_t v = pack(u, p, true, cc);
                uintx4 x = __builtin_bit_cast(uintx4, floatx4{ v[0], v[1], v[2], v[3] }), y = __builtin_bit_cast(uintx4, floatx4{ v[4], v[5], v[6], v[7] });
#pragma unroll
                for (int q = 0; q < 4; ++q) {
                    uintx2 r = __builtin_amdgcn_permlane16_swap(x[q], y[q], false, false);
                    r = __builtin_amdgcn_permlane32_swap(r[0], r[1], false, false);
                    x[q] = r[0]; y[q] = r[1];
                }
                float *d = cc + 32 * p - 4 * kg;
                const floatx4 lo = __builtin_bit_cast(floatx4, x), hi = __builtin_bit_cast(floatx4, y);
                if (c_stream) {
                    asm volatile("global_store_dwordx4 %0, %1, off sc1 nt\n\ts_nop 1" ::"v"(d), "v"(lo) : "memory");
                    asm volatile("global_store_dwordx4 %0, %1, off offset:64 sc1 nt\n\ts_nop 1" ::"v"(d), "v"(hi) : "memory");
                } else {
                    typedef floatx4 __attribute__((aligned(4))) floatx4_u;
                    *reinterpret_cast<floatx4_u *>(d) = lo;
                    *reinterpret_cast<floatx4_u *>(d + 16) = hi;
                }
            }
        }
    } else
#endif
#pragma unroll
    for (int u = 0; u < 8; ++u) {
        const uint32_t col = n0 + 128u * wn + 16u * u + i16;
        if (!full_tile && col >= g.N) continue;
        wg16_out_t *cc = C + (uint64_t)col * ldc + row0;
#pragma unroll
        for (int p = 0; p < 4; ++p) {
            if (!(full_tile || row0 + 32 * p < g.M)) continue;
            store8(cc + 32 * p, pack(u, p, true, cc));
        }
    }
#ifndef WG_F16_TRACE
    asm volatile("s_waitcnt vmcnt(0)" ::: "memory");
#endif
    if (paneled && lane == 0)
        __hip_atomic_fetch_add(panel_counter, 1u, __ATOMIC_RELAXED, __HIP_MEMORY_SCOPE_SYSTEM);
#ifdef WG_F16_TRACE
    WG_TRACE_POINT(3);
    asm volatile("s_waitcnt vmcnt(0)" ::: "memory");
    WG_TRACE_POINT(4);
    if (threadIdx.x == 0 && g.nsplit == 1 && g.part) {
        uint64_t *o = (uint64_t *)g.part + (uint64_t)bid * 8u;
        for (int i = 0; i < 5; ++i) o[i] = tr_t[i];
        o[5] = __builtin_amdgcn_s_getreg((4 << 0) | (0 << 6) | (31 << 11));
        o[6] = __builtin_amdgcn_s_getreg((20 << 0) | (0 << 6) | (31 << 11));
    }
#if WG_F16_TRACE >= 2
    if (lane == 0 && g.nsplit == 1 && g.part) {
        uint32_t *o = (uint32_t *)((uint64_t *)g.part + (uint64_t)g.trace_tiles * 8u) + ((uint64_t)bid * 4u + wave) * 8u;
        o[0] = loop_t1 - loop_t0; o[1] = s_vm; o[2] = s_bar; o[3] = s_probe; o[4] = m_vm; o[5] = m_bar; o[6] = n_adv; o[7] = 0;
    }
#endif
#endif
}

static __device__ uint32_t m16_acquire_tile(const GemmArgs &g) {
    const uint32_t x = __builtin_amdgcn_s_getreg((20 << 0) | (0 << 6) | (3 << 11)) & 7u;
    const uint32_t q = g.sched_tiles / 8u, r = g.sched_tiles % 8u;
    auto len = [&](uint32_t v) { return q + (v < r ? 1u : 0u); };
    unsigned long long old = atomicAdd(&g.sched[16u * x], 1ull);
    uint32_t lo = (uint32_t)old, hi = (uint32_t)(old >> 32);
    if (lo + hi < len(x)) return 8u * lo + x;
    for (int attempt = 0; attempt < 64; ++attempt) {
        uint32_t best = 0, victim = 8;
        for (uint32_t v = 0; v < 8u; ++v) {
            if (v == x) continue;
            const unsigned long long w = __hip_atomic_load(&g.sched[16u * v], __ATOMIC_RELAXED, __HIP_MEMORY_SCOPE_AGENT);
            const uint32_t taken = (uint32_t)w + (uint32_t)(w >> 32), n = len(v);
            if (taken < n && n - taken > best) { best = n - taken; victim = v; }
        }
        if (victim == 8u) return ~0u;
        old = atomicAdd(&g.sched[16u * victim], 1ull << 32);
        lo = (uint32_t)old; hi = (uint32_t)(old >> 32);
        if (lo + hi < len(victim)) return 8u * (len(victim) - 1u - hi) + victim;
    }
    return ~0u;
}

template <bool TRANS_A>
__global__ __launch_bounds__(256, 1) void WG16_SYM(gemm_, _m16_kernel)(GemmArgs g) {
    __shared__ __attribute__((aligned(16))) char smem[160 * 1024];
    uint32_t bid = blockIdx.x;
    uint32_t mode = 0, kb = 0, ns = 0, pair = 0;
    if (g.sched) {
        if (threadIdx.x == 0) *reinterpret_cast<volatile uint32_t *>(smem) = m16_acquire_tile(g);
        __syncthreads();
        bid = __builtin_amdgcn_readfirstlane(*reinterpret_cast<volatile uint32_t *>(smem));
        __syncthreads();
        if (bid == ~0u) return;
    } else if (g.bal.on) {
        if (!bal_decode(g.bal, blockIdx.x, g.K / 64u, bid, mode, kb, ns, pair)) return;
    }
    m16_tile<TRANS_A>(g, bid, smem, mode, kb, ns, pair);
}


#ifndef WG_GEMM16_OUT32
#define WG_ACC_QUADS(X) \
    X(0, 0, 1, 2, 3) X(1, 4, 5, 6, 7) X(2, 8, 9, 10, 11) X(3, 12, 13, 14, 15) \
    X(4, 16, 17, 18, 19) X(5, 20, 21, 22, 23) X(6, 24, 25, 26, 27) X(7, 28, 29, 30, 31) \
    X(8, 32, 33, 34, 35) X(9, 36, 37, 38, 39) X(10, 40, 41, 42, 43) X(11, 44, 45, 46, 47) \
    X(12, 48, 49, 50, 51) X(13, 52, 53, 54, 55) X(14, 56, 57, 58, 59) X(15, 60, 61, 62, 63) \
    X(16, 64, 65, 66, 67) X(17, 68, 69, 70, 71) X(18, 72, 73, 74, 75) X(19, 76, 77, 78, 79) \
    X(20, 80, 81, 82, 83) X(21, 84, 85, 86, 87) X(22, 88, 89, 90, 91) X(23, 92, 93, 94, 95) \
    X(24, 96, 97, 98, 99) X(25, 100, 101, 102, 103) X(26, 104, 105, 106, 107) X(27, 108, 109, 110, 111) \
    X(28, 112, 113, 114, 115) X(29, 116, 117, 118, 119) X(30, 120, 121, 122, 123) X(31, 124, 125, 126, 127) \
    X(32, 128, 129, 130, 131) X(33, 132, 133, 134, 135) X(34, 136, 137, 138, 139) X(35, 140, 141, 142, 143) \
    X(36, 144, 145, 146, 147) X(37, 148, 149, 150, 151) X(38, 152, 153, 154, 155) X(39, 156, 157, 158, 159) \
    X(40, 160, 161, 162, 163) X(41, 164, 165, 166, 167) X(42, 168, 169, 170, 171) X(43, 172, 173, 174, 175) \
    X(44, 176, 177, 178, 179) X(45, 180, 181, 182, 183) X(46, 184, 185, 186, 187) X(47, 188, 189, 190, 191) \
    X(48, 192, 193, 194, 195) X(49, 196, 197, 198, 199) X(50, 200, 201, 202, 203) X(51, 204, 205, 206, 207) \
    X(52, 208, 209, 210, 211) X(53, 212, 213, 214, 215) X(54, 216, 217, 218, 219) X(55, 220, 221, 222, 223) \
    X(56, 224, 225, 226, 227) X(57, 228, 229, 230, 231) X(58, 232, 233, 234, 235) X(59, 236, 237, 238, 239) \
    X(60, 240, 241, 242, 243) X(61, 244, 245, 246, 247) X(62, 248, 249, 250, 251) X(63, 252, 253, 254, 255)
template <int I> struct AccQuad;
#define WG_ACC_QUAD_DEF(I, R0, R1, R2, R3)                                                                                                              \
    template <> struct AccQuad<I> {                                                                                                                     \
        static __device__ __forceinline__ void mfma(half8_t a, half8_t b) {                                                                             \
            asm volatile(WG16_MFMA_ASM " a[" #R0 ":" #R3 "], %0, %1, a[" #R0 ":" #R3 "]" ::"v"(a), "v"(b) : "a" #R0, "a" #R1, "a" #R2, "a" #R3);  \
        }                                                                                                                                               \
        static __device__ __forceinline__ void mfma0(half8_t a, half8_t b) {       \
            asm volatile(WG16_MFMA_ASM " a[" #R0 ":" #R3 "], %0, %1, 0" ::"v"(a), "v"(b) : "a" #R0, "a" #R1, "a" #R2, "a" #R3);                     \
        }                                                                                                                                               \
        static __device__ __forceinline__ void read(float &x0, float &x1, float &x2, float &x3) {                                                       \
            asm volatile("v_accvgpr_read_b32 %0, a" #R0 "\n\tv_accvgpr_read_b32 %1, a" #R1 "\n\tv_accvgpr_read_b32 %2, a" #R2 "\n\tv_accvgpr_read_b32 %3, a" #R3 \
                         : "=v"(x0), "=v"(x1), "=v"(x2), "=v"(x3));                                                                                      \
        }                                                                                                                                               \
    };
WG_ACC_QUADS(WG_ACC_QUAD_DEF)
#undef WG_ACC_QUAD_DEF

template <bool TRANS_A, bool STREAM, bool ALPHA1>
__device__ __forceinline__ void m16_cont(const GemmArgs &g, char *const smem, const uint32_t walk_first, const int32_t walk_stride, const uint32_t walk_count) {
    const int lane = threadIdx.x & 63;
    const int wave = __builtin_amdgcn_readfirstlane(threadIdx.x >> 6);
    const int wm = wave >> 1, wn = wave & 1;
    const int i16 = lane & 15, kg = lane >> 4;
    const int aq = i16 >> 2, bb = i16 & 3;
    const int gq = (4 - aq) & 3;
    const uint32_t S = g.K / 64u;
    uint32_t tile = walk_first;
    uint32_t tiles_left = walk_count;
    uint32_t rem_g = walk_count * S;
    float alpha = g.alpha;
    uint32_t ldc = g.ldc;
    asm volatile("" : "+s"(alpha), "+s"(ldc));

    constexpr int NA = TRANS_A ? 8 : 4;
    uint32_t a_int[NA], b_int[8], a_voff[NA], b_voff[8];
    const uint32_t row_l = 64u * wave + (lane >> 3);
    const uint32_t mp_l = 32u * (lane >> 4) + 8u * (WG_NN_NOSWAP && !TRANS_A ? (lane & 3u) ^ ((uint32_t)wave & 1u) : (lane & 3u));
    if constexpr (TRANS_A) {
#pragma unroll
        for (int q = 0; q < 8; ++q) {
            const uint32_t row = row_l + 8u * q;
            const uint32_t fa = ((4u - ((row >> 3) & 3u)) & 3u) | (((row >> 1) & 1u) << 2);
            a_int[q] = (row * g.lda + 8u * ((lane & 7u) ^ fa)) * 2u + (M16_BIAS - 1024u * (q & 3));
        }
    } else {
#pragma unroll
        for (int q = 0; q < 4; ++q) {
            const uint32_t P = 4u * wave + q;
            a_int[q] = ((4u * (P >> 1) + ((lane >> 2) & 3)) * g.lda + 128u * (P & 1) + mp_l) * 2u + (M16_BIAS - 1024u * q);
        }
    }
#pragma unroll
    for (int q = 0; q < 8; ++q) {
        const uint32_t row = row_l + 8u * q;
        const uint32_t fb = ((4u - ((row >> 2) & 3u)) & 3u) | (((row >> 1) & 1u) << 2);
        b_int[q] = (row * g.ldb + 8u * ((lane & 7u) ^ fb)) * 2u + (M16_BIAS - 1024u * (q & 3));
    }
    auto set_voffs_a = [&](uint32_t lim) {
#pragma unroll
        for (int q = 0; q < NA; ++q) {
            const uint32_t r = TRANS_A ? row_l + 8u * q : 128u * (q & 1) + mp_l;
            const uint32_t over = r > lim ? r - lim : 0u;
            a_voff[q] = a_int[q] - over * (TRANS_A ? g.lda * 2u : 2u);
        }
    };
    auto set_voffs_b = [&](uint32_t lim) {
#pragma unroll
        for (int q = 0; q < 8; ++q) {
            const uint32_t r = row_l + 8u * q;
            const uint32_t over = r > lim ? r - lim : 0u;
            b_voff[q] = b_int[q] - over * (g.ldb * 2u);
        }
    };
    const uint32_t lds_base = (uint32_t)(uintptr_t)(WG_AS3 char *)smem;
    const uint32_t lds_a_wave = __builtin_amdgcn_readfirstlane(lds_base + wave * (TRANS_A ? 8192 : 4096));
    const uint32_t lds_b_wave = __builtin_amdgcn_readfirstlane(lds_base + M16_B_BASE + wave * 8192);
    uint32_t vbaseA[2], vbaseB[2];
#pragma unroll
    for (int hs = 0; hs < 2; ++hs) {
        const uint32_t chunk = (uint32_t)(((kg ^ gq) | ((hs ^ (bb >> 1)) << 2)) * 16);
        vbaseB[hs] = lds_base + M16_B_BASE + ((uint32_t)128 * wn + i16) * 128u + chunk;
        if constexpr (TRANS_A) vbaseA[hs] = lds_base + (128u * wm + 8u * aq + bb) * 128u + chunk;
    }
    uint32_t vbaseA1 = 0;
    if constexpr (!TRANS_A) {
        if constexpr (WG_NN_NOSWAP) {
            const uint32_t a = (uint32_t)i16 & 3u, krow = (uint32_t)i16 >> 2;
            const uint32_t common = lds_base + (uint32_t)kg * 4096u + (4u * wm) * 256u + krow * 64u + (a ^ ((uint32_t)kg & 1u)) * 16u;
            vbaseA[0] = common + (a & 1u) * 8u;
            vbaseA1 = common + ((a & 1u) ^ 1u) * 8u;
        } else {
            vbaseA[0] = lds_base + (uint32_t)((kg & 2) * 2) * 2048u + (4u * wm) * 256u + (uint32_t)i16 * 16u + (uint32_t)(kg & 1) * 8u;
        }
        vbaseA[1] = vbaseA[0];
    }
    const bool odd_row = !TRANS_A && WG_NN_NOSWAP && (kg & 1);
    const uint64_t a_half = TRANS_A ? 64u : (uint64_t)BKH * g.lda * 2u;
    const uint64_t a_full = TRANS_A ? 128u : a_half;
    const uint32_t tiles_per = g.tiles_m * g.tiles_n;
    auto sc64 = [](uint64_t v) -> uint64_t {
        return ((uint64_t)(uint32_t)__builtin_amdgcn_readfirstlane((int)(uint32_t)(v >> 32)) << 32) | (uint32_t)__builtin_amdgcn_readfirstlane((int)(uint32_t)v);
    };
    auto bases = [&](uint32_t id, const char *&a0, const char *&b0, uint32_t &m0, uint32_t &n0, uint64_t &c_off) {
        const uint32_t z = __builtin_amdgcn_readfirstlane(id / tiles_per), t = __builtin_amdgcn_readfirstlane(id - z * tiles_per);
        uint32_t tm, tn;
        tile_of(t, g.tiles_m, g.tiles_n, tm, tn);
        tm = __builtin_amdgcn_readfirstlane(tm); tn = __builtin_amdgcn_readfirstlane(tn);
        m0 = tm * BM; n0 = tn * BN;
        const uint64_t ao = (TRANS_A ? (uint64_t)m0 * g.lda : (uint64_t)m0) + (uint64_t)z * g.a_batch, bo = (uint64_t)n0 * g.ldb + (uint64_t)z * g.b_batch;
        a0 = (const char *)g.a + sc64(ao * 2u) - M16_BIAS;
        b0 = (const char *)g.b + sc64(bo * 2u) - M16_BIAS;
        c_off = sc64((uint64_t)z * g.c_batch);
    };
    const char *a0, *b0;
    uint32_t m0, n0;
    uint64_t c_off;
    bases(tile, a0, b0, m0, n0, c_off);
    auto lim_a = [&](uint32_t m0_) { return TRANS_A ? g.M - 1u - m0_ : g.M - 8u - m0_; };
    set_voffs_a(lim_a(m0)); set_voffs_b(g.N - 1u - n0);
    uint32_t nlim_a = 0, nlim_b = 0;

    uintx4 a_r[2][8];
    half8_t b_f[2][8];
    using c0 = std::integral_constant<int, 0>;
    using c1 = std::integral_constant<int, 1>;
    uint32_t st = 0;
    uint32_t va, vb, va1 = 0;
    const char *ga, *gb;
    uint32_t oR = 0, oD = 2u * M16_BS_BYTES, oA = 0, oAD = 0, la = 0, lb = 0;
    uint32_t rR = 1u << 14, rD = 0;
    uint32_t a_step0 = 0;
    uint64_t a_step1 = 0, b_step = 0;
// ... 240 lines not shown
                    uintx4 w = __builtin_bit_cast(uintx4, v);
#pragma unroll
                    for (int d = 0; d < 4; ++d) w[d] = (uint32_t)__builtin_amdgcn_ds_bpermute((int)perm_src, (int)w[d]);
                    v = __builtin_bit_cast(half8_t, w);
                }
                wg16_elem_t *dst = cc + 32 * p;
#ifndef WG_CONT_ABLATE
#define WG_CONT_ABLATE 0
#endif
                if (ok && !(WG_CONT_ABLATE & 1)) {
                    if constexpr (STREAM) asm volatile("global_store_dwordx4 %0, %1, off sc1 nt\n\ts_nop 1" ::"v"(dst), "v"(v) : "memory");
                    else asm volatile("global_store_dwordx4 %0, %1, off\n\ts_nop 1" ::"v"(dst), "v"(v) : "memory");
                }
                __builtin_amdgcn_sched_barrier(0);
            });
        });
        if (!has_next) break;
        tile = next; --tiles_left; a0 = na0; b0 = nb0; m0 = nm0; n0 = nn0; c_off = nc_off;
        st = 0;
        after_store = (WG_CONT_ABLATE & 1) ? 0u : TRANS_A ? 1u : 2u;
        if (!full_tile) {
            asm volatile("s_waitcnt vmcnt(0)" ::: "memory");
            after_store = 0u;
        }
        asm volatile("" : "+s"(st), "+s"(after_store));
    }
    asm volatile("s_waitcnt vmcnt(0)" ::: "memory");
}

template <bool TRANS_A, bool STREAM, bool ALPHA1>
__global__ __launch_bounds__(256, 1) void WG16_SYM(gemm_, _m16c_kernel)(GemmArgs g) {
    __shared__ __attribute__((aligned(16))) char smem[160 * 1024];
    const uint32_t first = blockIdx.x;
    if (first >= g.sched_tiles) return;
    m16_cont<TRANS_A, STREAM, ALPHA1>(g, smem, first, (int32_t)gridDim.x, (g.sched_tiles - 1u - first) / gridDim.x + 1u);
}
#endif


__global__ __launch_bounds__(256) void WG16_SYM(gemm_, _tail_reduce)(GemmArgs g) {
    uint32_t tm, tn;
    tile_of(blockIdx.x + g.tile_base, g.tiles_m, g.tiles_n, tm, tn);
    const uint32_t row = tm * BM + 4u * (threadIdx.x & 63u), col = tn * BN + blockIdx.y * 4u + (threadIdx.x >> 6);
    if (row >= g.M || col >= g.N) return;
    const float *p = g.part + (uint64_t)blockIdx.x * 65536u + (uint64_t)(col - tn * BN) * 256u + (row - tm * BM);
    float4 s = *reinterpret_cast<const float4 *>(p);
    for (uint32_t i = 1; i < g.nsplit; ++i) {
        const float4 q = *reinterpret_cast<const float4 *>(p + (uint64_t)i * g.tail_tiles * 65536u);
        s.x += q.x; s.y += q.y; s.z += q.z; s.w += q.w;
    }
    wg16_out_t *o = g.c + (uint64_t)col * g.ldc + row;
    typedef out4_u h4;
    if (g.alpha != 1.f) { s.x *= g.alpha; s.y *= g.alpha; s.z *= g.alpha; s.w *= g.alpha; }
    if (g.beta != 0.f) {
        const h4 t = *reinterpret_cast<const h4 *>(o);
        s.x = fmaf(g.beta, (float)t.v[0], s.x); s.y = fmaf(g.beta, (float)t.v[1], s.y);
        s.z = fmaf(g.beta, (float)t.v[2], s.z); s.w = fmaf(g.beta, (float)t.v[3], s.w);
    }
    const h4 r = { { (wg16_out_t)s.x, (wg16_out_t)s.y, (wg16_out_t)s.z, (wg16_out_t)s.w } };
    *reinterpret_cast<h4 *>(o) = r;
}


}
}

using namespace WG16_NS;

namespace {
int bal_prepare(wg_ctx *ctx) {
    wg_ctx::F16Balance &b = ctx->bal;
    if (ctx->recording) return WG_OK;
    if (!b.dev) {
        WG_HIP_TRY(hipMalloc((void **)&b.dev, kBalDevBytes));
        WG_HIP_TRY(hipMemset(b.dev, 0, kBalDevBytes));
        WG_HIP_TRY(hipHostMalloc((void **)&b.host, 16 * sizeof(unsigned long long), hipHostMallocDefault));
        WG_HIP_TRY(hipStreamCreateWithFlags(&b.side, hipStreamNonBlocking));
        WG_HIP_TRY(hipEventCreateWithFlags(&b.ev, hipEventDisableTiming));
    }
    if (b.inflight) {
        const hipError_t q = hipEventQuery(b.ev);
        if (q == hipErrorNotReady) { (void)hipGetLastError(); return WG_OK; }
        WG_HIP_TRY(q);
        b.inflight = false;
        double r[8], mean = 0;
        bool ok = true;
        for (int x = 0; x < 8; ++x) {
            const unsigned long long dt = b.host[2 * x] - b.prev[2 * x], ds = b.host[2 * x + 1] - b.prev[2 * x + 1];
            if (ds < 512) ok = false;
            r[x] = ds ? (double)dt / (double)ds : 0.0;
            mean += r[x] / 8.0;
        }
        if (ok) {
            for (int x = 0; x < 8; ++x) b.prev[2 * x] = b.host[2 * x], b.prev[2 * x + 1] = b.host[2 * x + 1];
            for (int x = 0; x < 8; ++x) ok = ok && r[x] > 0.8 * mean && r[x] < 1.25 * mean;
            if (ok) {
                double m2 = 0;
                for (int x = 0; x < 8; ++x) {
                    const double rn = r[x] / mean;
                    b.rel[x] = b.valid ? 0.5 * b.rel[x] + 0.5 * rn : rn;
                    m2 += b.rel[x] / 8.0;
                }
                for (int x = 0; x < 8; ++x) b.rel[x] /= m2;
                b.valid = true;
                b.updates++;
            }
        }
    }
    static thread_local uint32_t tick = 0;
    if (!b.inflight && (b.updates < 8 || (++tick & 15u) == 0)) {
        WG_HIP_TRY(hipMemcpyAsync(b.host, b.dev, 16 * sizeof(unsigned long long), hipMemcpyDeviceToHost, b.side));
        WG_HIP_TRY(hipEventRecord(b.ev, b.side));
        b.inflight = true;
    }
    return WG_OK;
}

int pad_copy(wg_ctx *ctx, wg16_elem_t *dst, uint32_t ld_dst, uint64_t dst_batch, uint32_t rd, uint32_t cd, const wg16_elem_t *src, uint32_t ld_src,
             uint64_t src_batch, uint32_t rs, uint32_t cs, uint32_t nmats) {
    return wgk_stage_copy(ctx, WG16_DTYPE, dst, ld_dst, dst_batch, rd, cd, src, ld_src, src_batch, rs, cs, nmats);
}

int pad_copy_c(wg_ctx *ctx, wg16_out_t *dst, uint32_t ld_dst, uint64_t dst_batch, uint32_t rd, uint32_t cd, const wg16_out_t *src, uint32_t ld_src,
               uint64_t src_batch, uint32_t rs, uint32_t cs, uint32_t nmats) {
    return wgk_stage_copy(ctx, WG16_OUT_DTYPE, dst, ld_dst, dst_batch, rd, cd, src, ld_src, src_batch, rs, cs, nmats);
}

template <bool TRANS>
void launch_m16(wg_ctx *ctx, dim3 grid, const GemmArgs &g) {
    hipLaunchKernelGGL((WG16_SYM(gemm_, _m16_kernel)<TRANS>), grid, dim3(256), 0, ctx->stream, g);
}

int launch_tiles(wg_ctx *ctx, wg_gemm16_query q, wg_gemm16_plan p, GemmArgs gm, uint32_t ntiles) {
    const bool trans = q.trans != 0;
#ifndef WG_GEMM16_OUT32
    if (p.cont) {
        const dim3 grid(p.nwg), block(256);
        gm.sched = nullptr; gm.sched_tiles = (uint32_t)((uint64_t)ntiles * q.nmats);
        wg_path(ctx, "%s", gemm16_tags(p, WG16_TAG, false).tag[0]);
        auto go = [&](auto tr_c, auto st_c, auto a1_c) {
            hipLaunchKernelGGL((WG16_SYM(gemm_, _m16c_kernel)<decltype(tr_c)::value, decltype(st_c)::value, decltype(a1_c)::value>), grid, block, 0, ctx->stream, gm);
        };
        auto by_alpha = [&](auto tr_c, auto st_c) { if (gm.alpha == 1.f) go(tr_c, st_c, std::true_type{}); else go(tr_c, st_c, std::false_type{}); };
        auto by_stream = [&](auto tr_c) { if (gm.c_stream) by_alpha(tr_c, std::true_type{}); else by_alpha(tr_c, std::false_type{}); };
        if (trans) by_stream(std::true_type{}); else by_stream(std::false_type{});
        return WG_OK;
    }
#else
    if (p.cont) return wg_set_error(WG_ERR_UNSUPPORTED, "Gemm: the continuous walk has no f32-output form");
#endif
    if (p.queues) {
        if (!ctx->tile_queues) {
            if (ctx->recording) return wg_set_error(WG_ERR_WORKSPACE, "Gemm: the tile queues are needed while recording: run the call once outside the recording first");
            WG_HIP_TRY(hipMalloc((void **)&ctx->tile_queues, 8 * 128));
        }
        WG_HIP_TRY(hipMemsetAsync(ctx->tile_queues, 0, 8 * 128, ctx->stream));
        gm.sched = ctx->tile_queues; gm.sched_tiles = ntiles;
    }
    uint32_t nwg = p.nwg;
    if (p.bal_eligible) {
        if (int rc = bal_prepare(ctx)) return rc;
        wg_ctx::F16Balance &b = ctx->bal;
        if (b.valid && !q.bal_valid) { q.bal_valid = 1; p = gemm16_plan(q); }
        if (b.dev && p.bal_calib) gm.calib = b.dev;
        if (p.bal_wanted && b.dev) {
            const uint32_t pairs = bal_plan(b.rel, ntiles, gm.K / 64u, q.balance == 1, gm.bal);
            if (pairs) {
                void *ws = nullptr;
                if (int rc = wg_ctx_bal_workspace(ctx, (size_t)pairs * 65536u * sizeof(float), &ws)) return rc;
                gm.bal.on = 1; gm.bal.epoch = ++b.epoch;
                gm.bal.flags = (uint32_t *)((char *)b.dev + kBalFlagsOffset);
                gm.bal.part = (float *)ws;
                uint32_t mx = 0;
                for (int x = 0; x < 8; ++x) mx = gm.bal.len[x] > mx ? gm.bal.len[x] : mx;
                nwg = 8u * mx;
            } else gm.bal = BalancePlan{};
        }
    }
    wg_path(ctx, "%s", gemm16_tags(p, WG16_TAG, gm.bal.on != 0).tag[0]);
    const dim3 grid(nwg, gm.nsplit * q.nmats);
    if (trans) launch_m16<true>(ctx, grid, gm); else launch_m16<false>(ctx, grid, gm);
    return WG_OK;
}

int run_m16(wg_ctx *ctx, const wg_gemm16_query &q, const wg_gemm16_plan &p, GemmArgs g, const wgk_panels *panels, void *ws) {
    const uint32_t tiles = p.tiles_m * p.tiles_n;
    if (panels) {
        const uint32_t ptn = panels->cols / 256u;
        g.panel.cols = panels->cols; g.panel.n_main = panels->n_main; g.panel.npanels = panels->n_main + panels->n_tail; g.panel.tiles = g.tiles_m * ptn;
        uint32_t tn_left = g.tiles_n - panels->n_main * ptn;
        for (uint32_t t = 0; t < panels->n_tail; ++t) {
            const uint32_t tn = t + 1u == panels->n_tail ? tn_left : panels->tail_cols[t] / 256u;
            g.panel.tail_tn |= (uint64_t)tn << (8u * t);
            tn_left -= tn;
        }
        g.panel.col_stride = panels->col_stride; g.panel.slot_rows = panels->slot_rows;
        g.panel.counters = panels->counters;
    }
#ifdef WG_F16_TRACE
    uint64_t *trace = nullptr;
    if (p.nsplit == 1) {
        WG_HIP_TRY(hipMalloc((void **)&trace, (uint64_t)tiles * q.nmats * 192));
        WG_HIP_TRY(hipMemset(trace, 0, (uint64_t)tiles * q.nmats * 192));
        g.part = (float *)trace;
        g.trace_tiles = (uint32_t)(tiles * q.nmats);
    }
#endif
    if (int rc = launch_tiles(ctx, q, p, g, tiles - p.tail)) return rc;
    if (p.tail) {
        GemmArgs gt = g;
        gt.tile_base = tiles - p.tail; gt.tail_tiles = p.tail; gt.nsplit = p.tail_split; gt.k_per_split = p.tail_kps; gt.part = (float *)ws;
        const Gemm16Tags tags = gemm16_tags(p, WG16_TAG, false);
        wg_path(ctx, "%s", tags.tag[1]);
        wg_path(ctx, "%s", tags.tag[2]);
        if (q.trans) launch_m16<true>(ctx, dim3(p.tail, p.tail_split), gt); else launch_m16<false>(ctx, dim3(p.tail, p.tail_split), gt);
        hipLaunchKernelGGL(WG16_SYM(gemm_, _tail_reduce), dim3(p.tail, 64), dim3(256), 0, ctx->stream, gt);
    }
#ifdef WG_F16_TRACE
    if (trace && !p.tail) {
        WG_HIP_TRY(hipStreamSynchronize(ctx->stream));
        std::vector<uint64_t> h((uint64_t)tiles * q.nmats * 24);
        WG_HIP_TRY(hipMemcpy(h.data(), trace, h.size() * 8, hipMemcpyDeviceToHost));
        if (FILE *f = fopen("/tmp/wg_f16_trace.bin", "wb")) { fwrite(h.data(), 8, h.size(), f); fclose(f); }
        (void)hipFree(trace);
    }
#endif
    WG_HIP_TRY(hipGetLastError());
    return WG_OK;
}

int gemm16(wg_ctx *ctx, bool padded, bool trans, uint32_t M, uint32_t N, uint32_t K, uint32_t nmats, wg16_oext_t *out, uint32_t out_ld, uint64_t out_batch,
           wgk_mat m1, wgk_mat m2, float alpha, float beta, const wgk_panels *panels);

int run_pad(wg_ctx *ctx, const wg_gemm16_query &q, const wg_gemm16_plan &p, wg16_oext_t *out, wgk_mat m1, wgk_mat m2) {
    const wg_gemm16_query in = gemm16_pad_inner(q, p);
    const bool trans = q.trans != 0;
    const uint32_t M = q.M, N = q.N, K = q.K, nmats = q.nmats, Mp = p.Mp, Kp = p.Kp;
    const uint64_t a_sz = p.a_ok ? 0 : in.a_batch, b_sz = p.b_ok ? 0 : in.b_batch;
    void *ws = nullptr;
    const uint64_t c_extra = kOut32 && !p.c_ok ? in.c_batch * nmats * 2u : 0u;
    if (int rc = wg_ctx_pad_workspace(ctx, (size_t)(p.workspace_bytes + c_extra), &ws)) return rc;
    wg16_elem_t *ap = (wg16_elem_t *)ws, *bp = ap + a_sz * nmats;
    wg16_out_t *cp = (wg16_out_t *)(bp + b_sz * nmats);
    wg_path(ctx, "%s", gemm16_tags(p, WG16_TAG, false).tag[0]);
    wgk_mat a2 = m1, b2 = m2;
    if (!p.a_ok) {
        if (trans) { if (int rc = pad_copy(ctx, ap, Kp, a_sz, Kp, Mp, (const wg16_elem_t *)m1.ptr, m1.ld, m1.batch, K, M, nmats)) return rc; }
        else { if (int rc = pad_copy(ctx, ap, Mp, a_sz, Mp, Kp, (const wg16_elem_t *)m1.ptr, m1.ld, m1.batch, M, K, nmats)) return rc; }
        a2 = wgk_mat{ ap, in.lda, in.a_batch };
    }
    if (!p.b_ok) {
        if (int rc = pad_copy(ctx, bp, Kp, b_sz, Kp, N, (const wg16_elem_t *)m2.ptr, m2.ld, m2.batch, K, N, nmats)) return rc;
        b2 = wgk_mat{ bp, in.ldb, in.b_batch };
    }
    if (p.c_ok) return gemm16(ctx, true, trans, in.M, N, in.K, nmats, out, in.ldc, in.c_batch, a2, b2, q.alpha, q.beta, nullptr);
    if (p.c_seed)
        if (int rc = pad_copy_c(ctx, cp, Mp, in.c_batch, Mp, N, (const wg16_out_t *)out, q.ldc, q.c_batch, M, N, nmats)) return rc;
    if (int rc = gemm16(ctx, true, trans, in.M, N, in.K, nmats, (wg16_oext_t *)cp, in.ldc, in.c_batch, a2, b2, q.alpha, q.beta, nullptr)) return rc;
    return pad_copy_c(ctx, (wg16_out_t *)out, q.ldc, q.c_batch, M, N, cp, Mp, in.c_batch, M, N, nmats);
}

int gemm16(wg_ctx *ctx, bool padded, bool trans, uint32_t M, uint32_t N, uint32_t K, uint32_t nmats, wg16_oext_t *out, uint32_t out_ld, uint64_t out_batch,
           wgk_mat m1, wgk_mat m2, float alpha, float beta, const wgk_panels *panels) {
    wg_gemm16_query q = {};
    q.trans = trans; q.M = M; q.N = N; q.K = K; q.nmats = nmats;
    q.lda = m1.ld; q.ldb = m2.ld; q.ldc = out_ld;
    q.a_batch = m1.batch; q.b_batch = m2.batch; q.c_batch = out_batch;
    q.a_addr = (uint32_t)((uintptr_t)m1.ptr & 15); q.b_addr = (uint32_t)((uintptr_t)m2.ptr & 15); q.c_addr = (uint32_t)((uintptr_t)out & 15);
    q.alpha = alpha; q.beta = beta;
    if (panels) {
        q.panels = 1; q.panel_cols = panels->cols; q.panel_n_main = panels->n_main; q.panel_n_tail = panels->n_tail;
        for (int t = 0; t < 8; ++t) q.panel_tail_cols[t] = panels->tail_cols[t];
    }
    q.cus = (uint32_t)(ctx->compute_units > 0 ? ctx->compute_units : 256);
    q.tile = ctx->tuning[WG_TUNE_F16_TILE]; q.sched = ctx->tuning[WG_TUNE_F16_SCHED]; q.cont = ctx->tuning[WG_TUNE_F16_CONT]; q.balance = ctx->tuning[WG_TUNE_F16_BALANCE];
    q.uneven_xcds = ctx->uneven_xcds; q.recording = ctx->recording; q.bal_valid = ctx->bal.valid; q.padded = padded;
    if constexpr (kOut32) q = gemm16_out32_query(q);
    const wg_gemm16_plan p = gemm16_plan(q);

    GemmArgs g;
    g.a = (const wg16_elem_t *)m1.ptr; g.lda = m1.ld; g.a_batch = m1.batch;
    g.b = (const wg16_elem_t *)m2.ptr; g.ldb = m2.ld; g.b_batch = m2.batch;
    g.c = (wg16_out_t *)out; g.ldc = out_ld; g.c_batch = out_batch;
    g.M = M; g.N = N; g.K = K;
    g.alpha = alpha; g.beta = beta;
    g.tiles_m = p.tiles_m; g.tiles_n = p.tiles_n;
    g.nsplit = p.nsplit; g.k_per_split = p.k_per_split; g.part = nullptr;
    g.c_stream = p.c_stream; g.a_nt = p.a_nt;
    if constexpr (kOut32) g.c_stream = gemm16_c_stream(q, sizeof(wg16_out_t));
    g.tile_base = 0; g.tail_tiles = 0;
    g.sched = nullptr; g.sched_tiles = 0;
    g.calib = nullptr; g.bal = BalancePlan{}; g.panel = PanelArgs{};
    if (p.leaf == WG_GEMM16_UNSUPPORTED) return p.message[0] ? wg_set_error(p.status, "%s", p.message) : p.status;
    if (p.leaf == WG_GEMM16_PAD) return run_pad(ctx, q, p, out, m1, m2);
    void *ws = nullptr;
    if (p.workspace_bytes)
        if (int rc = wg_ctx_workspace(ctx, (size_t)p.workspace_bytes, &ws)) return rc;
    if (p.nsplit > 1) g.part = (float *)ws;
    const Gemm16Tags tags = gemm16_tags(p, WG16_TAG, false);
    switch (p.leaf) {
    case WG_GEMM16_SKINNY:
        wg_path(ctx, "%s", tags.tag[0]);
        if (int rc = WG16_SYM(wgk_gemm_, _skinny)(ctx, M, N, K, nmats, out, out_ld, out_batch, m1, m2, alpha, beta, p.nsplit, p.k_per_split, g.part)) return rc;
        break;
    case WG_GEMM16_T256X128:
        wg_path(ctx, "%s", tags.tag[0]);
        return t128_launch(ctx, trans, dim3(p.tiles_m * p.tiles_n, nmats), g, 256);
    case WG_GEMM16_T128:
        wg_path(ctx, "%s", tags.tag[0]);
        if (int rc = t128_launch(ctx, trans, dim3(p.tiles_m * p.tiles_n, nmats * p.nsplit), g)) return rc;
        break;
    case WG_GEMM16_M16:
        if (int rc = run_m16(ctx, q, p, g, panels, ws)) return rc;
        break;
    default:
        wg_path(ctx, "%s", tags.tag[0]);
        if (int rc = generic_launch(ctx, trans, dim3(g.tiles_m, g.tiles_n, nmats), g)) return rc;
        WG_HIP_TRY(hipGetLastError());
        break;
    }
    if (p.nsplit > 1) return wg_splitk_reduce(ctx, g.part, p.nsplit, M, N, nmats, WG16_OUT_DTYPE, out, out_ld, out_batch, alpha, beta);
    return WG_OK;
}
}

int WG16_SYM(wgk_gemm_, )(wg_ctx *ctx, bool trans, uint32_t M, uint32_t N, uint32_t K, uint32_t nmats,
                 wg16_oext_t *out, uint32_t out_ld, uint64_t out_batch, wgk_mat m1, wgk_mat m2, float alpha, float beta, const wgk_panels *panels) {
    return gemm16(ctx, false, trans, M, N, K, nmats, out, out_ld, out_batch, m1, m2, alpha, beta, kOut32 ? nullptr : panels);
}
```

wgmath_amd/csrc/gemm_f16_common.hpp:

```cpp
#pragma once
#include "wg_internal.hpp"

#include <cstdio>
#include <cstdlib>
#include <type_traits>
#include <utility>
#include <vector>

#ifdef WG_GEMM16_BF16
typedef __bf16 wg16_elem_t;
typedef wg_bf16 wg16_ext_t;
#define WG16_DTYPE WG_BF16
#define WG16_MFMA __builtin_amdgcn_mfma_f32_16x16x32_bf16
#define WG16_MFMA_ASM "v_mfma_f32_16x16x32_bf16"
#else
typedef _Float16 wg16_elem_t;
typedef __half wg16_ext_t;
#define WG16_DTYPE WG_F16
#define WG16_MFMA __builtin_amdgcn_mfma_f32_16x16x32_f16
#define WG16_MFMA_ASM "v_mfma_f32_16x16x32_f16"
#endif
#ifdef WG_GEMM16_OUT32
typedef float wg16_out_t;
typedef float wg16_oext_t;
#define WG16_OUT_DTYPE WG_F32
#ifdef WG_GEMM16_BF16
#define WG16_ID bf16o32
#define WG16_TAG "bf16o32"
#else
#define WG16_ID f16o32
#define WG16_TAG "f16o32"
#endif
#else
typedef wg16_elem_t wg16_out_t;
typedef wg16_ext_t wg16_oext_t;
#define WG16_OUT_DTYPE WG16_DTYPE
#ifdef WG_GEMM16_BF16
#define WG16_ID bf16
#define WG16_TAG "bf16"
#else
#define WG16_ID f16
#define WG16_TAG "f16"
#endif
#endif
#define WG16_CAT3_(a, b, c) a##b##c
#define WG16_CAT3(a, b, c) WG16_CAT3_(a, b, c)
#define WG16_SYM(pre, post) WG16_CAT3(pre, WG16_ID, post)
#define WG16_NS WG16_SYM(wg, )

namespace WG16_NS {


#ifndef WG_ABLATE
#define WG_ABLATE 0
#endif

typedef wg16_elem_t half8_t __attribute__((ext_vector_type(8)));
typedef half8_t __attribute__((aligned(2))) half8_u;
constexpr bool kOut32 = sizeof(wg16_out_t) == 4;
typedef wg16_out_t out8_t __attribute__((ext_vector_type(8)));
typedef out8_t __attribute__((aligned(sizeof(wg16_out_t)))) out8_u;
struct alignas(sizeof(wg16_out_t)) out4_u { wg16_out_t v[4]; };
typedef short short4_t __attribute__((ext_vector_type(4)));
typedef short short8_t __attribute__((ext_vector_type(8)));
typedef float floatx16 __attribute__((ext_vector_type(16)));
#define WG_AS1 __attribute__((address_space(1)))
#define WG_AS3 __attribute__((address_space(3)))

constexpr int BM = 256, BN = 256, BKH = 32;
constexpr int HA_BYTES = BM * BKH * 2;
constexpr int HB_BYTES = BN * BKH * 2;
constexpr int HSTAGE_BYTES = HA_BYTES + HB_BYTES;
constexpr int NSLOT = 5;

}

namespace wg16 {
struct BalancePlan {
    uint32_t on, epoch;
    uint32_t *flags;
    float *part;
    uint32_t len[8];
    uint32_t pre_cnt[8], pre_src[8], pre_p[8], pre_slot[8], pre_pair0[8];
    uint32_t suf_lo[8][2], suf_cnt[8][2], suf_p[8][2], suf_pair0[8][2];
};

__host__ __device__ inline bool bal_decode(const BalancePlan &bp, uint32_t b, uint32_t stages, uint32_t &tile, uint32_t &mode, uint32_t &kb, uint32_t &ns,
                                           uint32_t &pair) {
    const uint32_t x = b & 7u, c = b >> 3;
    mode = 0; kb = 0; ns = 0; pair = 0; tile = b;
    if (c >= bp.len[x]) return false;
    const uint32_t npre = bp.pre_cnt[x];
    if (c < npre) {
        mode = 1; ns = bp.pre_p[x]; pair = bp.pre_pair0[x] + c;
        tile = 8u * (bp.pre_slot[x] + c) + bp.pre_src[x];
        return true;
    }
    const uint32_t t = c - npre;
    tile = 8u * t + x;
    for (int r = 0; r < 2; ++r)
        if (t - bp.suf_lo[x][r] < (uint32_t)bp.suf_cnt[x][r]) {
            mode = 2; kb = bp.suf_p[x][r]; ns = stages - kb; pair = bp.suf_pair0[x][r] + (t - bp.suf_lo[x][r]);
        }
    return true;
}
}

namespace WG16_NS {
using wg16::BalancePlan;
using wg16::bal_decode;

constexpr int kPanelTail = 8;
struct PanelArgs {
    uint32_t cols;
    uint32_t npanels, tiles;
    uint32_t n_main;
    uint64_t tail_tn;
    uint64_t col_stride, slot_rows;
    uint32_t *counters;
};

struct GemmArgs {
    const wg16_elem_t *a; uint32_t lda; uint64_t a_batch;
    const wg16_elem_t *b; uint32_t ldb; uint64_t b_batch;
    wg16_out_t *c; uint32_t ldc; uint64_t c_batch;
    uint32_t M, N, K;
    uint32_t tiles_m, tiles_n;
    uint32_t nsplit, k_per_split;
    float *part;
    float alpha, beta;
    uint32_t c_stream;
    uint32_t a_nt;
    uint32_t tile_base, tail_tiles;
    unsigned long long *sched; uint32_t sched_tiles;
    unsigned long long *calib;
    BalancePlan bal;
    PanelArgs panel;
#ifdef WG_F16_TRACE
    uint32_t trace_tiles;
#endif
};

#ifndef WG_NN_NOSWAP
#define WG_NN_NOSWAP 1
#endif

template <int IMM>
static __device__ __forceinline__ void glds16s(uint32_t voff, const void *sbase, uint32_t lds_dst) {
    if (WG_ABLATE & 2) return;
    uint32_t keep;
    asm volatile("s_mov_b32 %0, m0\n\ts_mov_b32 m0, %3\n\ts_nop 0\n\tglobal_load_lds_dwordx4 %1, %2 offset:%c4\n\ts_mov_b32 m0, %0"
                 : "=&s"(keep)
                 : "v"(voff), "s"(sbase), "s"(lds_dst), "i"(IMM));
}
static __device__ __forceinline__ void wait_dma_all() { asm volatile("s_waitcnt vmcnt(0)" ::: "memory"); }
template <int N>
static __device__ __forceinline__ void wait_dma_keep() { asm volatile("s_waitcnt vmcnt(%c0)" ::"i"(N) : "memory"); }
static __device__ __forceinline__ short4_t lds_tr(const char *p) {
    if (WG_ABLATE & 4) { short4_t v; asm volatile("" : "=v"(v)); return v; }
    return __builtin_amdgcn_ds_read_tr16_b64_v4i16((WG_AS3 short4_t *)p);
}
static __device__ __forceinline__ half8_t lds_h8(const char *p) {
    if (WG_ABLATE & 4) { half8_t v; asm volatile("" : "=v"(v)); return v; }
    return *reinterpret_cast<const half8_t *>(p);
}
static __device__ __forceinline__ short4_t lds_tr_at(uint32_t addr) {
    if (WG_ABLATE & 4) { short4_t v; asm volatile("" : "=v"(v)); return v; }
    return __builtin_amdgcn_ds_read_tr16_b64_v4i16((WG_AS3 short4_t *)(uintptr_t)addr);
}
static __device__ __forceinline__ half8_t lds_h8_at(uint32_t addr) {
    if (WG_ABLATE & 4) { half8_t v; asm volatile("" : "=v"(v)); return v; }
    return *(WG_AS3 const half8_t *)(uintptr_t)addr;
}
static __device__ __forceinline__ half8_t cat(short4_t lo, short4_t hi) {
    short8_t v = { lo[0], lo[1], lo[2], lo[3], hi[0], hi[1], hi[2], hi[3] };
    return __builtin_bit_cast(half8_t, v);
}

static __device__ __forceinline__ void tile_strips(uint32_t bid, uint32_t tiles_m, uint32_t tiles_n, uint32_t &tm, uint32_t &tn) {
    const uint32_t nwg = tiles_m * tiles_n;
    const uint32_t q = nwg / 8u, r = nwg % 8u, xcd = bid % 8u, local = bid / 8u;
    const uint32_t o = (xcd < r ? xcd * (q + 1u) : r * (q + 1u) + (xcd - r) * q) + local;
    const uint32_t strip = o / (4u * tiles_n);
    const uint32_t within = o - strip * 4u * tiles_n;
    const uint32_t h = min(4u, tiles_m - 4u * strip);
    tn = within / h;
    tm = 4u * strip + (within - tn * h);
}

static __device__ __forceinline__ void tile_of(uint32_t bid, uint32_t tiles_m, uint32_t tiles_n, uint32_t &tm, uint32_t &tn) {
    if ((tiles_m % 16u) == 0 && (tiles_n % 16u) == 0) {
        const uint32_t super = bid >> 8, within = bid & 255u;
        const uint32_t xcd = within & 7u, local = within >> 3;
        const uint32_t sm = super % (tiles_m / 16u), sn = super / (tiles_m / 16u);
        tm = sm * 16u + (xcd & 3u) * 4u + (local & 3u);
        tn = sn * 16u + (xcd >> 2) * 8u + (local >> 2);
    } else {
        tile_strips(bid, tiles_m, tiles_n, tm, tn);
    }
}


int generic_launch(wg_ctx *ctx, bool trans, dim3 grid, const GemmArgs &g);
int t128_launch(wg_ctx *ctx, bool trans, dim3 grid, const GemmArgs &g, int tm = 128);
int t128_launch_nt(wg_ctx *ctx, dim3 grid, const GemmArgs &g, int tm = 128);

}
```

wgmath_amd/csrc/runtime.hip:

```cpp
#include "wg_internal.hpp"

#include <vector>

#include <cstdlib>
#include <cstring>
#include <new>
#include <string>

namespace {
thread_local std::string g_last_error;
}

int wg_set_error(int status, const char *fmt, ...) {
    char buf[1024];
    va_list ap;
    va_start(ap, fmt);
    vsnprintf(buf, sizeof buf, fmt, ap);
    va_end(ap);
    g_last_error = buf;
    return status;
}
void wg_clear_error() { g_last_error.clear(); }

static int grow_scratch(wg_ctx *ctx, void **region, size_t *region_bytes, size_t bytes, const char *what, void **out) {
    if (bytes > *region_bytes) {
        if (ctx->recording)
            return wg_set_error(WG_ERR_WORKSPACE, "%s of %zu bytes needed while recording: run the call once outside the recording first "
                                "(or wg_ctx_reserve_workspace)", what, bytes);
        WG_HIP_TRY(hipSetDevice(ctx->device));
        WG_HIP_TRY(hipStreamSynchronize(ctx->stream));
        if (*region) {
            if (ctx->live_cmdbufs > 0) ctx->retired_scratch.push_back(*region);
            else WG_HIP_TRY(hipFree(*region));
        }
        *region = nullptr;
        *region_bytes = 0;
        size_t want = (bytes + (1u << 20) - 1) & ~(size_t)((1u << 20) - 1);
        WG_HIP_TRY(hipMalloc(region, want));
        *region_bytes = want;
    }
    *out = *region;
    return WG_OK;
}
int wg_ctx_workspace(wg_ctx *ctx, size_t bytes, void **out) { return grow_scratch(ctx, &ctx->workspace, &ctx->workspace_bytes, bytes, "workspace", out); }
int wg_ctx_tr_workspace(wg_ctx *ctx, size_t bytes, void **out) {
    return grow_scratch(ctx, &ctx->tr_workspace, &ctx->tr_workspace_bytes, bytes, "transpose workspace", out);
}
int wg_ctx_pad_workspace(wg_ctx *ctx, size_t bytes, void **out) {
    return grow_scratch(ctx, &ctx->pad_workspace, &ctx->pad_workspace_bytes, bytes, "padding workspace", out);
}
void wg_ctx_register_async_error(wg_ctx *ctx, uint32_t *word, const char *what, uint32_t *dev_word) { ctx->async_errors.push_back({ word, what, dev_word }); }
void wg_ctx_unregister_async_error(wg_ctx *ctx, uint32_t *word) {
    for (size_t i = 0; i < ctx->async_errors.size(); ++i)
        if (ctx->async_errors[i].word == word) { ctx->async_errors.erase(ctx->async_errors.begin() + (long)i); return; }
}
int wg_ctx_check_async(wg_ctx *ctx) {
    for (const wg_ctx::AsyncError &e : ctx->async_errors) {
        const uint32_t v = *(volatile uint32_t *)e.word;
        if (v) {
            *(volatile uint32_t *)e.word = 0;
            if (e.dev_word) (void)hipMemsetAsync(e.dev_word, 0, sizeof(uint32_t), ctx->stream);
            return wg_set_error(WG_ERR_HIP, "%s %u", e.what, v - 1u);
        }
    }
    return WG_OK;
}

int wg_ctx_stage_workspace(wg_ctx *ctx, size_t bytes, void **out) {
    return grow_scratch(ctx, &ctx->stage_workspace, &ctx->stage_workspace_bytes, bytes, "staging workspace", out);
}
int wg_ctx_bal_workspace(wg_ctx *ctx, size_t bytes, void **out) {
    return grow_scratch(ctx, &ctx->bal.scratch, &ctx->bal.scratch_bytes, bytes, "balance workspace", out);
}

namespace {
thread_local int t_capturing = 0;
thread_local std::shared_ptr<wg_deferred_batch> t_batch;
void capture_began(wg_ctx *ctx) {
    if (t_capturing++ == 0 || !t_batch) t_batch = std::make_shared<wg_deferred_batch>();
    ctx->capture_batch = t_batch;
    ctx->recording_thread = std::this_thread::get_id();
}
std::shared_ptr<wg_deferred_batch> capture_ended(wg_ctx *ctx) {
    std::shared_ptr<wg_deferred_batch> batch = std::move(ctx->capture_batch);
    ctx->capture_batch.reset();
    if (t_capturing > 0 && --t_capturing == 0) t_batch.reset();
    return batch;
}
}
bool wg_defer_if_capturing(std::function<void()> fn, bool is_ctx) {
    if (t_capturing == 0 || !t_batch) return false;
    (is_ctx ? t_batch->ctx_items : t_batch->items).push_back(std::move(fn));
    return true;
}

extern "C" {

int wg_abi_version(void) { return WGEBRA_HIP_ABI_VERSION; }

const char *wg_last_error_string(void) { return g_last_error.c_str(); }

int wg_device_count(void) {
    int n = 0;
    if (hipGetDeviceCount(&n) != hipSuccess) {
        (void)hipGetLastError();
        return 0;
    }
    return n;
}

static int ctx_create_common(int device, hipStream_t stream, bool owns, wg_ctx **out) {
    if (!out) return wg_set_error(WG_ERR_INVALID_ARG, "wg_ctx_create: out is NULL");
    *out = nullptr;
    int n = wg_device_count();
    if (n <= 0) return wg_set_error(WG_ERR_NO_DEVICE, "Failed to initialize gpu adapter.: no HIP device visible");
    if (device < 0 || device >= n) return wg_set_error(WG_ERR_INVALID_ARG, "wg_ctx_create: device %d not in [0,%d)", device, n);
    WG_HIP_TRY(hipSetDevice(device));
    hipDeviceProp_t prop;
    WG_HIP_TRY(hipGetDeviceProperties(&prop, device));
    if (strncmp(prop.gcnArchName, "gfx950", 6) != 0)
        return wg_set_error(WG_ERR_NO_DEVICE, "device %d is %s; this library ships gfx950 (MI355X) code objects only",
                            device, prop.gcnArchName);
    wg_ctx *ctx = new (std::nothrow) wg_ctx();
    if (!ctx) return wg_set_error(WG_ERR_HIP, "out of host memory");
    ctx->device = device;
    ctx->compute_units = prop.multiProcessorCount;
    if (owns) {
        hipError_t e = hipStreamCreateWithFlags(&ctx->stream, hipStreamNonBlocking);
        if (e != hipSuccess) {
            delete ctx;
            return wg_set_error(WG_ERR_HIP, "hipStreamCreate failed: %s", hipGetErrorString(e));
        }
    } else {
        ctx->stream = stream;
    }
    ctx->owns_stream = owns;
    static const struct { const char *env; wg_tuning key; } knobs[] = {
        { "WG_F16_TILE", WG_TUNE_F16_TILE }, { "WG_F16_SCHED", WG_TUNE_F16_SCHED }, { "WG_F32_SKINNY", WG_TUNE_F32_SKINNY },
        { "WG_F32_PANELS", WG_TUNE_F32_PANELS }, { "WG_F16_BALANCE", WG_TUNE_F16_BALANCE }, { "WG_F32_MID", WG_TUNE_F32_MID }, { "WG_F32_MID_SPLIT", WG_TUNE_F32_MID_SPLIT },
        { "WG_GEMVT_LDS", WG_TUNE_GEMVT_LDS }, { "WG_F16_CONT", WG_TUNE_F16_CONT }, { "WG_RM_TR_NATIVE", WG_TUNE_RM_TR_NATIVE } };
    for (const auto &k : knobs)
        if (const char *v = getenv(k.env)) {
            if (wg_ctx_set_tuning(ctx, k.key, atoi(v)) != WG_OK) fprintf(stderr, "libwgebra_hip: ignoring %s=%s (%s)\n", k.env, v, wg_last_error_string());
        }
    *out = ctx;
    return WG_OK;
}

int wg_ctx_create(int device, wg_ctx **out) { return ctx_create_common(device, nullptr, true, out); }
int wg_ctx_create_on_stream(int device, void *hip_stream, wg_ctx **out) {
    return ctx_create_common(device, (hipStream_t)hip_stream, false, out);
}

static int ctx_create_masked(int device, uint32_t cu_count, bool one_xcd, wg_ctx **out) {
    if (!out) return wg_set_error(WG_ERR_INVALID_ARG, "wg_ctx_create_with_cu_count: out is NULL");
    *out = nullptr;
    int n = wg_device_count();
    if (n <= 0) return wg_set_error(WG_ERR_NO_DEVICE, "Failed to initialize gpu adapter.: no HIP device visible");
    if (device < 0 || device >= n) return wg_set_error(WG_ERR_INVALID_ARG, "wg_ctx_create_with_cu_count: device %d not in [0,%d)", device, n);
    WG_HIP_TRY(hipSetDevice(device));
    hipDeviceProp_t prop;
    WG_HIP_TRY(hipGetDeviceProperties(&prop, device));
    const uint32_t total = (uint32_t)prop.multiProcessorCount;
    if (cu_count == 0 || cu_count > total) return wg_set_error(WG_ERR_INVALID_ARG, "wg_ctx_create_with_cu_count: %u not in [1,%u]", cu_count, total);
    std::vector<uint32_t> mask((total + 31) / 32, 0u);
    const uint32_t missing = total - cu_count;
    const bool uneven = one_xcd && missing > 0 && missing < total / 8u;
    if (uneven) {
        for (auto &w : mask) w = 0xffffffffu;
        if (total % 32) mask.back() = (1u << (total % 32)) - 1u;
        for (uint32_t j = 0; j < missing; ++j) {
            const uint32_t bit = 7u + 8u * j;
            if (bit < total) mask[bit / 32] &= ~(1u << (bit % 32));
        }
    } else {
        for (uint32_t i = 0; i < cu_count; ++i) mask[i / 32] |= 1u << (i % 32);
    }
    hipStream_t stream = nullptr;
    hipError_t e = hipExtStreamCreateWithCUMask(&stream, (uint32_t)mask.size(), mask.data());
    if (e != hipSuccess) return wg_set_error(WG_ERR_HIP, "hipExtStreamCreateWithCUMask failed: %s", hipGetErrorString(e));
    int rc = ctx_create_common(device, stream, false, out);
    if (rc) { (void)hipStreamDestroy(stream); return rc; }
    (*out)->owns_stream = true;
    (*out)->uneven_xcds = uneven;
    (*out)->compute_units = (int)cu_count;
    return WG_OK;
}
int wg_ctx_create_with_cu_count(int device, uint32_t cu_count, wg_ctx **out) { return ctx_create_masked(device, cu_count, false, out); }
int wg_ctx_create_with_cu_count_one_xcd(int device, uint32_t cu_count, wg_ctx **out) { return ctx_create_masked(device, cu_count, true, out); }

int wg_ctx_destroy(wg_ctx *ctx) {
    if (!ctx) return WG_OK;
    if (!ctx->recording && wg_defer_if_capturing([ctx] { (void)wg_ctx_destroy(ctx); }, true)) return WG_OK;
    if (ctx->recording) {
        if (ctx->recording_thread != std::this_thread::get_id())
            return wg_set_error(WG_ERR_INVALID_ARG, "wg_ctx_destroy: the context is recording on another thread; finish or destroy it there");
        hipGraph_t g = nullptr;
        (void)hipStreamEndCapture(ctx->stream, &g);
        if (g) (void)hipGraphDestroy(g);
        ctx->recording = false;
        std::shared_ptr<wg_deferred_batch> abandoned = capture_ended(ctx);
        abandoned.reset();
    }
    (void)hipSetDevice(ctx->device);
    (void)hipStreamSynchronize(ctx->stream);
    if (ctx->workspace) (void)hipFree(ctx->workspace);
    if (ctx->tr_workspace) (void)hipFree(ctx->tr_workspace);
    if (ctx->pad_workspace) (void)hipFree(ctx->pad_workspace);
    if (ctx->stage_workspace) (void)hipFree(ctx->stage_workspace);
    for (void *p : ctx->retired_scratch) (void)hipFree(p);
    if (ctx->flags) (void)hipFree(ctx->flags);
    if (ctx->tile_queues) (void)hipFree(ctx->tile_queues);
    if (ctx->bal.side) { (void)hipStreamSynchronize(ctx->bal.side); (void)hipStreamDestroy(ctx->bal.side); }
    if (ctx->bal.ev) (void)hipEventDestroy(ctx->bal.ev);
    if (ctx->bal.dev) (void)hipFree(ctx->bal.dev);
    if (ctx->bal.host) (void)hipHostFree(ctx->bal.host);
    if (ctx->bal.scratch) (void)hipFree(ctx->bal.scratch);
    if (ctx->debug_stamps) (void)hipHostFree(ctx->debug_stamps);
    if (ctx->owns_stream && ctx->stream) (void)hipStreamDestroy(ctx->stream);
    delete ctx;
    return WG_OK;
}

int wg_ctx_sync(wg_ctx *ctx) {
    if (!ctx) return wg_set_error(WG_ERR_INVALID_ARG, "wg_ctx_sync: ctx is NULL");
    if (ctx->recording) return wg_set_error(WG_ERR_INVALID_ARG, "wg_ctx_sync: cannot synchronise while recording");
    WG_HIP_TRY(hipStreamSynchronize(ctx->stream));
    return wg_ctx_check_async(ctx);
}
int wg_ctx_device(const wg_ctx *ctx) { return ctx ? ctx->device : -1; }
void *wg_ctx_stream(const wg_ctx *ctx) { return ctx ? (void *)ctx->stream : nullptr; }

int wg_ctx_device_info(const wg_ctx *ctx, char *name256, int *compute_units, int *clock_mhz, uint64_t *hbm_bytes) {
    if (!ctx) return wg_set_error(WG_ERR_INVALID_ARG, "wg_ctx_device_info: ctx is NULL");
    hipDeviceProp_t prop;
    WG_HIP_TRY(hipGetDeviceProperties(&prop, ctx->device));
    if (name256) snprintf(name256, 256, "%s (%s)", prop.name[0] ? prop.name : "AMD Instinct (name not reported)", prop.gcnArchName);
    if (compute_units) *compute_units = prop.multiProcessorCount;
    if (clock_mhz) *clock_mhz = prop.clockRate / 1000;
    if (hbm_bytes) *hbm_bytes = (uint64_t)prop.totalGlobalMem;
    return WG_OK;
}

int wg_ctx_mem_info(const wg_ctx *ctx, uint64_t *free_bytes, uint64_t *total_bytes) {
    if (!ctx) return wg_set_error(WG_ERR_INVALID_ARG, "wg_ctx_mem_info: ctx is NULL");
    WG_HIP_TRY(hipSetDevice(ctx->device));
    size_t f = 0, t = 0;
    WG_HIP_TRY(hipMemGetInfo(&f, &t));
    if (free_bytes) *free_bytes = (uint64_t)f;
    if (total_bytes) *total_bytes = (uint64_t)t;
    return WG_OK;
}

__global__ void wg_debug_spin_kernel(uint64_t *start_ticks, uint32_t usec) {
    const uint64_t t0 = __builtin_amdgcn_s_memrealtime();
    if (threadIdx.x == 0 && start_ticks) start_ticks[blockIdx.x] = t0;
    while (__builtin_amdgcn_s_memrealtime() - t0 < (uint64_t)usec * 100u) __builtin_amdgcn_s_sleep(16);
}
__global__ void wg_debug_now_kernel(uint64_t *tick) { *tick = __builtin_amdgcn_s_memrealtime(); }

int wg_debug_spin(wg_ctx *ctx, uint32_t blocks, uint32_t usec, wg_buf *start_ticks) {
    if (!ctx || blocks == 0) return wg_set_error(WG_ERR_INVALID_ARG, "wg_debug_spin: bad arguments");
    if (start_ticks && start_ticks->bytes < (size_t)(blocks + 1) * 8) return wg_set_error(WG_ERR_OUT_OF_BOUNDS, "wg_debug_spin: start_ticks too small");
    WG_HIP_TRY(hipSetDevice(ctx->device));
    uint64_t *p = start_ticks ? (uint64_t *)start_ticks->ptr : nullptr;
    if (p) hipLaunchKernelGGL(wg_debug_now_kernel, dim3(1), dim3(1), 0, ctx->stream, p + blocks);
    hipLaunchKernelGGL(wg_debug_spin_kernel, dim3(blocks), dim3(256), 0, ctx->stream, p, usec);
    WG_HIP_TRY(hipGetLastError());
    return WG_OK;
}

int wg_ctx_set_tuning(wg_ctx *ctx, wg_tuning key, int value) {
    if (!ctx || (int)key < 0 || (int)key >= (int)WG_TUNE_COUNT_) return wg_set_error(WG_ERR_INVALID_ARG, "wg_ctx_set_tuning: bad context or key %d", (int)key);
    if (key == WG_TUNE_F16_TILE && value != 0 && value != 128 && value != 256 && value != 256128)
        return wg_set_error(WG_ERR_INVALID_ARG, "wg_ctx_set_tuning: WG_TUNE_F16_TILE takes 0, 128, 256 or 256128, not %d", value);
    if (key == WG_TUNE_F32_MID && (value == 64064 || value == 64128 || value == 128064 || value == 128128 || value == 64032 || value == 32064 || value == 96096 || value == 96064 || value == 64096)) {
        ctx->tuning[key] = value;
        return WG_OK;
    }
    if (key == WG_TUNE_GEMVT_LDS) {
        if (value < 0 || value > 65536) return wg_set_error(WG_ERR_INVALID_ARG, "wg_ctx_set_tuning: WG_TUNE_GEMVT_LDS takes 0 or an output count per CU, not %d", value);
        ctx->tuning[key] = value;
        return WG_OK;
    }
    if (key == WG_TUNE_F32_MID_SPLIT) {
        if (value < 0 || value == 1 || value > 64) return wg_set_error(WG_ERR_INVALID_ARG, "wg_ctx_set_tuning: WG_TUNE_F32_MID_SPLIT takes 0 or 2..64, not %d", value);
        ctx->tuning[key] = value;
        return WG_OK;
    }
    if (key != WG_TUNE_F16_TILE && (value < -1 || value > 1))
        return wg_set_error(WG_ERR_INVALID_ARG, "wg_ctx_set_tuning: knob %d takes -1, 0 or 1, not %d", (int)key, value);
    ctx->tuning[key] = value;
    return WG_OK;
// ... 291 lines not shown
```

wgmath_amd/csrc/wg_internal.hpp:

```cpp
#pragma once

#include <hip/hip_runtime.h>
#include <hip/hip_fp16.h>

#include <cstdarg>
#include <cstdint>
#include <cstdio>
#include <functional>
#include <memory>
#include <string>
#include <thread>
#include <vector>

#include "../../include/wgebra_hip.h"

struct wg_deferred_batch {
    std::vector<std::function<void()>> items, ctx_items;
    ~wg_deferred_batch() {
        for (auto &f : items) f();
        for (auto &f : ctx_items) f();
    }
};

struct wg_ctx {
    int device = 0;
    hipStream_t stream = nullptr;
    bool owns_stream = true;
    bool recording = false;
    std::thread::id recording_thread;
    std::shared_ptr<wg_deferred_batch> capture_batch;
    void *workspace = nullptr;
    size_t workspace_bytes = 0;
    void *tr_workspace = nullptr;
    size_t tr_workspace_bytes = 0;
    void *stage_workspace = nullptr;
    size_t stage_workspace_bytes = 0;
    void *pad_workspace = nullptr;
    size_t pad_workspace_bytes = 0;
    int compute_units = 0;
    bool uneven_xcds = false;
    unsigned *flags = nullptr;
    unsigned long long *tile_queues = nullptr;
    struct F16Balance {
        unsigned long long *dev = nullptr;
        unsigned long long *host = nullptr;
        unsigned long long prev[16] = { 0 };
        hipStream_t side = nullptr;
        hipEvent_t ev = nullptr;
        bool inflight = false, valid = false, have_prev = false;
        double rel[8] = { 1, 1, 1, 1, 1, 1, 1, 1 };
        uint32_t epoch = 0, updates = 0;
        void *scratch = nullptr;
        size_t scratch_bytes = 0;
    } bal;
    int tuning[WG_TUNE_COUNT_] = { 0, -1, -1, -1, 0, -1, 0, 0, -1, -1 };
    void *debug_stamps = nullptr;
    bool debug_clock_open = false;
    uint32_t lds_attr_bits = 0;
    uint32_t func_attr_bits = 0;
    int live_cmdbufs = 0;
    std::vector<void *> retired_scratch;
    struct AsyncError { uint32_t *word; const char *what; uint32_t *dev_word; };
    std::vector<AsyncError> async_errors;
    std::string path_log;
};
static inline int wg_ctx_cus(const wg_ctx *ctx) { return ctx->compute_units > 0 ? ctx->compute_units : 256; }
bool wg_defer_if_capturing(std::function<void()> fn, bool is_ctx = false);
void wg_ctx_register_async_error(wg_ctx *ctx, uint32_t *word, const char *what, uint32_t *dev_word = nullptr);
void wg_ctx_unregister_async_error(wg_ctx *ctx, uint32_t *word);
int wg_ctx_check_async(wg_ctx *ctx);

struct wg_buf {
    wg_ctx *ctx = nullptr;
    void *ptr = nullptr;
    size_t bytes = 0;
    uint32_t usage = 0;
    bool owned = true;
    bool host_pinned = false;
    void *ipc_base = nullptr;
    bool borrowed = false;
};

struct wg_cmdbuf {
    wg_ctx *ctx = nullptr;
    hipGraph_t graph = nullptr;
    hipGraphExec_t exec = nullptr;
    std::shared_ptr<wg_deferred_batch> deferred;
};

struct wg_timestamps {
    wg_ctx *ctx = nullptr;
    std::vector<hipEvent_t> events;
    std::vector<uint8_t> written;
    uint32_t len = 0;
};

constexpr size_t kPathLogCap = 480;
void wg_path(wg_ctx *ctx, const char *fmt, ...) __attribute__((format(printf, 2, 3)));

int wg_set_error(int status, const char *fmt, ...) __attribute__((format(printf, 2, 3)));
void wg_clear_error();

#define WG_HIP_TRY(expr)                                                                              \
    do {                                                                                              \
        hipError_t _e = (expr);                                                                       \
        if (_e != hipSuccess)                                                                         \
            return wg_set_error(WG_ERR_HIP, "%s failed: %s (%s:%d)", #expr, hipGetErrorString(_e),   \
                                __FILE__, __LINE__);                                                  \
    } while (0)

int wg_ctx_workspace(wg_ctx *ctx, size_t bytes, void **out);
int wg_ctx_tr_workspace(wg_ctx *ctx, size_t bytes, void **out);
int wg_ctx_pad_workspace(wg_ctx *ctx, size_t bytes, void **out);
int wg_ctx_bal_workspace(wg_ctx *ctx, size_t bytes, void **out);
int wg_ctx_stage_workspace(wg_ctx *ctx, size_t bytes, void **out);
int wgk_stage_copy(wg_ctx *ctx, wg_dtype dtype, void *dst, uint32_t ld_dst, uint64_t dst_batch, uint32_t rd, uint32_t cd, const void *src,
                   uint32_t ld_src, uint64_t src_batch, uint32_t rs, uint32_t cs, uint32_t nmats);
int wgk_transpose(wg_ctx *ctx, wg_dtype dtype, uint32_t rows, uint32_t cols, uint32_t nmats, const void *src, uint32_t ld_src,
                  uint64_t src_batch, void *dst, uint32_t ld_dst, uint64_t dst_batch);

typedef float wg_f4 __attribute__((ext_vector_type(4)));
__device__ __forceinline__ float4 wg_ld_nt(const float4 *p) {
    wg_f4 v = __builtin_nontemporal_load(reinterpret_cast<const wg_f4 *>(p));
    return make_float4(v.x, v.y, v.z, v.w);
}
typedef wg_f4 __attribute__((aligned(4))) wg_f4_u;
__device__ __forceinline__ float4 wg_ld_nt_u(const float *p) {
    wg_f4 v = __builtin_nontemporal_load(reinterpret_cast<const wg_f4_u *>(p));
    return make_float4(v.x, v.y, v.z, v.w);
}
__device__ __forceinline__ float4 wg_ld_u(const float *p) {
    wg_f4 v = *reinterpret_cast<const wg_f4_u *>(p);
    return make_float4(v.x, v.y, v.z, v.w);
}
__device__ __forceinline__ void wg_st_u(float *p, float4 v) { *reinterpret_cast<wg_f4_u *>(p) = wg_f4{ v.x, v.y, v.z, v.w }; }

static inline size_t wg_dtype_size(wg_dtype d) { return d == WG_F32 ? 4 : 2; }
typedef __bf16 wg_bf16;


struct wgk_mat {
    const void *ptr;
    uint32_t ld;
    uint64_t batch;
};

int wgk_op_assign(wg_ctx *ctx, int op, wg_dtype dtype, void *a, const void *b, uint32_t n, float alpha = 0.f);

int wgk_reduce_fast(wg_ctx *ctx, int op, wg_dtype dtype, const void *base, uint32_t n, void *result);
int wgk_reduce(wg_ctx *ctx, int op, wg_dtype dtype, const void *base, uint32_t n, uint32_t ncols, uint32_t nmats,
               uint32_t stride, uint32_t stride_mat, void *results);

int wgk_gemv(wg_ctx *ctx, bool trans, wg_dtype dtype, uint32_t rows_out, uint32_t k, uint32_t nrhs, uint32_t nmats,
             void *out, uint32_t out_ld, uint64_t out_batch, wgk_mat m, wgk_mat v);

int wgk_gemv_any(wg_ctx *ctx, bool trans, wg_dtype dtype, uint32_t R, uint32_t C, uint32_t nrhs, uint32_t nmats, void *out, uint32_t out_ld, uint64_t out_batch,
                 wgk_mat m, wgk_mat v);
int wgk_gemv_mixed(wg_ctx *ctx, bool trans, wg_dtype m_dtype, uint32_t rows_out, uint32_t k, uint32_t nrhs, uint32_t nmats,
                   float *out, uint32_t out_ld, uint64_t out_batch, wgk_mat m, wgk_mat v);
int wgk_gemv_any_mixed(wg_ctx *ctx, bool trans, wg_dtype m_dtype, uint32_t R, uint32_t C, uint32_t nrhs, uint32_t nmats, float *out, uint32_t out_ld, uint64_t out_batch,
                       wgk_mat m, wgk_mat v);
int wgk_gemv_q8(wg_ctx *ctx, const wg_gemv_q8_plan &p, bool trans, uint32_t group_rows, uint32_t rows, uint32_t cols, uint32_t nrhs, uint32_t nmats, float *out, uint32_t out_ld,
                uint64_t out_batch, wgk_mat m, wgk_mat s, wgk_mat v);
int wgk_gemv_q4(wg_ctx *ctx, const wg_gemv_q4_plan &p, uint32_t group_rows, uint32_t k, uint32_t rows_out, uint32_t nrhs, uint32_t nmats, float *out, uint32_t out_ld,
                uint64_t out_batch, wgk_mat m, wgk_mat s, wgk_mat v);
int wgk_gemm_q8(wg_ctx *ctx, const wg_gemm_q8_plan &p, bool bf16, uint32_t group_rows, uint32_t k, uint32_t outputs, uint32_t n, uint32_t nmats, float *out, uint32_t out_ld,
                uint64_t out_batch, wgk_mat m, wgk_mat s, wgk_mat x);
int wgk_gemm_q4(wg_ctx *ctx, const wg_gemm_q4_plan &p, bool bf16, uint32_t group_rows, uint32_t k, uint32_t outputs, uint32_t n, uint32_t nmats, float *out, uint32_t out_ld,
                uint64_t out_batch, wgk_mat m, wgk_mat s, wgk_mat x);
int wgk_gemm_q8a8(wg_ctx *ctx, const wg_gemm_q8a8_plan &p, uint32_t group_rows, uint32_t x_group_rows, uint32_t k, uint32_t outputs, uint32_t n, uint32_t nmats, float *out,
                  uint32_t out_ld, uint64_t out_batch, wgk_mat m, wgk_mat s, wgk_mat x, wgk_mat xs);
wg_quantize_q8_plan quantize_q8_plan(const wg_quantize_q8_query &q);
int wgk_quantize_q8(wg_ctx *ctx, const wg_quantize_q8_plan &p, wg_dtype src_dtype, uint32_t group_rows, uint32_t rows, uint32_t cols, uint32_t nmats, int8_t *q, uint32_t q_ld,
                    uint64_t q_batch, float *s, uint32_t s_ld, uint64_t s_batch, wgk_mat src);
wg_gemv_query wgk_gemv_query(const wg_ctx *ctx, bool trans, wg_dtype m_dtype, wg_dtype v_dtype, bool gemm16, uint32_t rows_out, uint32_t k, uint32_t nrhs, uint32_t nmats,
                             uint32_t out_ld, uint64_t out_batch, wgk_mat m, wgk_mat v);
int wgk_gemv_small_reduce(wg_ctx *ctx, const wg_gemv_plan &p, int op, uint32_t rows_out, uint32_t k, float *y, wgk_mat m, wgk_mat v, unsigned *counter, float *result);

int wgk_gemm_f32(wg_ctx *ctx, bool trans, uint32_t M, uint32_t N, uint32_t K, uint32_t nmats,
                 float *out, uint32_t out_ld, uint64_t out_batch, wgk_mat m1, wgk_mat m2, float alpha = 1.f, float beta = 0.f);
int wgk_gemm_f32_mid(wg_ctx *ctx, const wg_gemm32_plan &p, bool trans, uint32_t M, uint32_t N, uint32_t K, uint32_t nmats, float *out, uint32_t out_ld, uint64_t out_batch,
                     wgk_mat m1, wgk_mat m2, float alpha, float beta);
int wgk_gemm_f32_skinny(wg_ctx *ctx, const wg_gemm32_plan &p, bool trans, uint32_t M, uint32_t N, uint32_t K, uint32_t nmats, float *out, uint32_t out_ld, uint64_t out_batch,
                        wgk_mat m1, wgk_mat m2, float alpha, float beta, uint32_t out_row_stride = 1, bool m2_kmajor = false);
int wgk_gemm_f16_skinny(wg_ctx *ctx, uint32_t M, uint32_t N, uint32_t K, uint32_t nmats, __half *out, uint32_t out_ld, uint64_t out_batch, wgk_mat m1, wgk_mat m2,
                        float alpha, float beta, uint32_t ns, uint32_t kps, float *part);
int wgk_gemm_bf16_skinny(wg_ctx *ctx, uint32_t M, uint32_t N, uint32_t K, uint32_t nmats, wg_bf16 *out, uint32_t out_ld, uint64_t out_batch, wgk_mat m1, wgk_mat m2,
                         float alpha, float beta, uint32_t ns, uint32_t kps, float *part);
struct wgk_panels {
    uint32_t cols = 0, n_main = 0, n_tail = 0;
    uint32_t tail_cols[8] = { 0 };
    uint64_t col_stride = 0, slot_rows = 0;
    uint32_t *counters = nullptr;
};
static inline uint32_t wgk_panel_goal(uint32_t M, uint32_t np) { return 4u * ((M + 255u) / 256u) * ((np + 255u) / 256u); }
int wgk_gemm_f16(wg_ctx *ctx, bool trans, uint32_t M, uint32_t N, uint32_t K, uint32_t nmats,
                 __half *out, uint32_t out_ld, uint64_t out_batch, wgk_mat m1, wgk_mat m2, float alpha = 1.f, float beta = 0.f,
                 const wgk_panels *panels = nullptr);
int wgk_gemm_bf16(wg_ctx *ctx, bool trans, uint32_t M, uint32_t N, uint32_t K, uint32_t nmats,
                  wg_bf16 *out, uint32_t out_ld, uint64_t out_batch, wgk_mat m1, wgk_mat m2, float alpha = 1.f, float beta = 0.f,
                  const wgk_panels *panels = nullptr);
int wgk_gemm_f16o32(wg_ctx *ctx, bool trans, uint32_t M, uint32_t N, uint32_t K, uint32_t nmats,
                    float *out, uint32_t out_ld, uint64_t out_batch, wgk_mat m1, wgk_mat m2, float alpha = 1.f, float beta = 0.f,
                    const wgk_panels *panels = nullptr);
int wgk_gemm_bf16o32(wg_ctx *ctx, bool trans, uint32_t M, uint32_t N, uint32_t K, uint32_t nmats,
                     float *out, uint32_t out_ld, uint64_t out_batch, wgk_mat m1, wgk_mat m2, float alpha = 1.f, float beta = 0.f,
                     const wgk_panels *panels = nullptr);
int wgk_gemm_f16o32_skinny(wg_ctx *ctx, uint32_t M, uint32_t N, uint32_t K, uint32_t nmats, float *out, uint32_t out_ld, uint64_t out_batch, wgk_mat m1, wgk_mat m2,
// ... 19 lines not shown
```

wgmath_amd/wgcore.py:

```python
from __future__ import annotations

import ctypes
import enum
from dataclasses import dataclass, replace
from typing import Optional, Sequence

import numpy as np

from . import _lib
from ._lib import ViewShapeC, check, lib

bfloat16 = np.dtype([("bits", "<u2")])

_DT = {np.dtype(np.float32): _lib.WG_F32, np.dtype(np.float16): _lib.WG_F16, bfloat16: _lib.WG_BF16}


def wg_dtype(dtype) -> int:
    try:
        return _DT[np.dtype(dtype)]
    except KeyError:
        raise TypeError(f"element type {dtype} is not supported by the dense kernels (f32 / f16 / bf16: numpy.float32, numpy.float16, wgmath_amd.bfloat16)") from None


def to_bfloat16(values) -> np.ndarray:
# ... 149 lines not shown

    def compute_pass(self, label: str, timestamps: Optional["GpuTimestamps"] = None) -> ComputePass:
        if self._record and timestamps is not None:
            raise ValueError("timestamps cannot be captured into a recorded command buffer")
        return ComputePass(self, label, timestamps)

    def begin_compute_pass(self, label: str = "") -> ComputePass:
        return ComputePass(self, label, None)

    def finish(self) -> CommandBuffer:
        if self._finished:
            raise RuntimeError("CommandEncoder.finish called twice")
        self._finished = True
        if self._record:
            h = ctypes.c_void_p()
            self._ctx.recording = False
            check(lib.wg_encoder_finish(self._ctx.handle, ctypes.byref(h)))
            return CommandBuffer(self._ctx, h.value)
        return CommandBuffer(self._ctx, None)


class Device:

    def __init__(self, ctx: _Ctx):
        self._ctx = ctx

    def create_command_encoder(self, desc=None, record: bool = False) -> CommandEncoder:
        return CommandEncoder(self._ctx, record=record)

    def poll_wait(self) -> None:
        check(lib.wg_ctx_sync(self._ctx.handle))

    def reserve_workspace(self, nbytes: int) -> None:
        check(lib.wg_ctx_reserve_workspace(self._ctx.handle, nbytes))


class Queue:

    def __init__(self, ctx: _Ctx):
        self._ctx = ctx

    def submit(self, command_buffers) -> None:
        if isinstance(command_buffers, CommandBuffer):
            command_buffers = [command_buffers]
        for cb in command_buffers or []:
            if cb is not None and cb._h:
                check(lib.wg_queue_submit(self._ctx.handle, cb._h))

    def get_timestamp_period(self) -> float:
        return 1.0

    def write_buffer(self, tensor: "GpuTensor", offset_bytes: int, data) -> None:
        arr = np.ascontiguousarray(data)
        check(lib.wg_buf_write(self._ctx.handle, tensor._h, offset_bytes, arr.ctypes.data_as(ctypes.c_void_p), arr.nbytes))


class ClockProbe:

    def __init__(self, gpu):
        self._gpu = gpu
        self._open = lib.wg_debug_clock_begin(gpu._ctx.handle) == _lib.WG_OK

    def end(self):
        if not self._open:
            return None
        self._open = False
        mean, lo, hi, secs = ctypes.c_double(), ctypes.c_double(), ctypes.c_double(), ctypes.c_double()
        if lib.wg_debug_clock_end(self._gpu._ctx.handle, ctypes.byref(mean), ctypes.byref(lo), ctypes.byref(hi), ctypes.byref(secs)) != _lib.WG_OK:
            return None
        return {"mean": mean.value, "min": lo.value, "max": hi.value, "seconds": secs.value}


class GpuInstance:

    def __init__(self, ctx: _Ctx):
        self._ctx = ctx
        self._device = Device(ctx)
        self._queue = Queue(ctx)

    @staticmethod
    def new(device_index: int = 0, stream: Optional[int] = None, cu_count: Optional[int] = None, one_xcd: bool = False) -> "GpuInstance":
        _lib.assert_single_hip_runtime()
        h = ctypes.c_void_p()
        if cu_count is not None:
            create = lib.wg_ctx_create_with_cu_count_one_xcd if one_xcd else lib.wg_ctx_create_with_cu_count
            check(create(device_index, int(cu_count), ctypes.byref(h)))
            inst = GpuInstance(_Ctx(h.value, device_index))
            inst._stream_compute_units = int(cu_count)
            return inst
        elif stream is None:
            check(lib.wg_ctx_create(device_index, ctypes.byref(h)))
        else:
            check(lib.wg_ctx_create_on_stream(device_index, ctypes.c_void_p(stream), ctypes.byref(h)))
        return GpuInstance(_Ctx(h.value, device_index))

    without_gl = new
    with_backends = new

    @staticmethod
    def with_backends(backends=None, device_index: int = 0) -> "GpuInstance":
        return GpuInstance.new(device_index)

    @staticmethod
    def without_gl(device_index: int = 0) -> "GpuInstance":
        return GpuInstance.new(device_index)

    def device_arc(self) -> "Device":
        return self.device()

    @staticmethod
    def device_count() -> int:
        return lib.wg_device_count()

    def adapter(self) -> dict:
        name = ctypes.create_string_buffer(256)
        cus, mhz, hbm = ctypes.c_int(), ctypes.c_int(), ctypes.c_uint64()
        check(lib.wg_ctx_device_info(self._ctx.handle, name, ctypes.byref(cus), ctypes.byref(mhz), ctypes.byref(hbm)))
        info = {"name": name.value.decode(), "compute_units": cus.value, "clock_mhz": mhz.value, "hbm_bytes": hbm.value}
        if getattr(self, "_stream_compute_units", None):
            info["stream_compute_units"] = int(self._stream_compute_units)
        return info

    def mem_info(self) -> tuple:
        free, total = ctypes.c_uint64(), ctypes.c_uint64()
        check(lib.wg_ctx_mem_info(self._ctx.handle, ctypes.byref(free), ctypes.byref(total)))
        return free.value, total.value

    def device(self) -> Device:
        return self._device

    device_arc = device

    def queue(self) -> Queue:
        return self._queue

    def stream(self) -> int:
        return lib.wg_ctx_stream(self._ctx.handle) or 0

    def sync(self) -> None:
        check(lib.wg_ctx_sync(self._ctx.handle))

    def clock_probe(self) -> "ClockProbe":
        return ClockProbe(self)

    def mfma_ceiling(self, min_seconds: float = 0.5) -> dict:
        tf, ghz = ctypes.c_double(), ctypes.c_double()
        check(lib.wg_debug_mfma_ceiling(self._ctx.handle, float(min_seconds), ctypes.byref(tf), ctypes.byref(ghz)))
        return {"tflops": tf.value, "clock_ghz": ghz.value}

    def close(self) -> None:
        self._ctx.close()

    _TUNING = {"f16_tile": _lib.WG_TUNE_F16_TILE, "f16_sched": _lib.WG_TUNE_F16_SCHED, "f32_skinny": _lib.WG_TUNE_F32_SKINNY,
               "f32_panels": _lib.WG_TUNE_F32_PANELS, "f16_balance": _lib.WG_TUNE_F16_BALANCE, "f32_mid": _lib.WG_TUNE_F32_MID, "f32_mid_split": _lib.WG_TUNE_F32_MID_SPLIT, "gemvt_lds": _lib.WG_TUNE_GEMVT_LDS, "f16_cont": _lib.WG_TUNE_F16_CONT, "rm_tr_native": _lib.WG_TUNE_RM_TR_NATIVE}

    def set_tuning(self, knob: str, value: int) -> int:
        old = self.get_tuning(knob)
        check(lib.wg_ctx_set_tuning(self._ctx.handle, self._TUNING[knob], int(value)))
        return old

    def f16_balance_info(self) -> dict:
        rel, valid, upd, n = (ctypes.c_double * 8)(), ctypes.c_int(), ctypes.c_uint32(), ctypes.c_uint32()
        check(lib.wg_ctx_f16_balance_info(self._ctx.handle, rel, ctypes.byref(valid), ctypes.byref(upd), ctypes.byref(n)))
        return {"rel": [round(float(v), 4) for v in rel], "valid": bool(valid.value), "updates": upd.value, "balanced_launches": n.value}

    def take_path(self) -> str:
        buf = ctypes.create_string_buffer(1024)
        check(lib.wg_debug_take_path(self._ctx.handle, buf, len(buf)))
        return buf.value.decode()

    def get_tuning(self, knob: str) -> int:
        v = ctypes.c_int()
        check(lib.wg_ctx_get_tuning(self._ctx.handle, self._TUNING[knob], ctypes.byref(v)))
        return v.value


def _prod(shape: Sequence[int]) -> int:
    n = 1
    for s in shape:
        n *= int(s)
    return n


def _flat_col_major(data, dtype) -> np.ndarray:
    arr = np.asarray(data, dtype=dtype)
    return np.ascontiguousarray(arr.reshape(-1, order="F") if arr.ndim > 1 else arr)


class TensorBuilder:

    def __init__(self, shape: Sequence[int], usage: BufferUsages):
        self.shape = tuple(int(s) for s in shape)
        self.usage = BufferUsages(usage)
        self._label = None
        for s in self.shape:
            if not 0 <= s < 2 ** 32:
                raise ValueError("tensor dimensions are u32")

    @staticmethod
    def scalar(usage) -> "TensorBuilder":
        return TensorBuilder((), usage)

    @staticmethod
    def vector(dim: int, usage) -> "TensorBuilder":
        return TensorBuilder((dim,), usage)

    @staticmethod
    def matrix(nrows: int, ncols: int, usage) -> "TensorBuilder":
        return TensorBuilder((nrows, ncols), usage)

    @staticmethod
    def tensor(shape: Sequence[int], usage) -> "TensorBuilder":
        return TensorBuilder(shape, usage)

    def len(self) -> int:
        return _prod(self.shape)

    def label(self, label: str) -> "TensorBuilder":
        self._label = label
        return self

    def build(self, device: Device, dtype=np.float32) -> "GpuTensor":
        dt = np.dtype(dtype)
        h = ctypes.c_void_p()
        check(lib.wg_buf_create(device._ctx.handle, self.len() * dt.itemsize, int(self.usage), ctypes.byref(h)))
        return GpuTensor(device._ctx, h.value, self.shape, dt, self.usage)

    def build_init(self, device: Device, data, dtype=None) -> "GpuTensor":
        dt = np.dtype(dtype if dtype is not None else getattr(data, "dtype", np.float32))
        if dt == bfloat16 and getattr(data, "dtype", None) != bfloat16:
            data = to_bfloat16(data)
        flat = _flat_col_major(data, dt)
        n = self.len()
        assert flat.size >= n, (
            "Incorrect number of elements provided for initializing Tensor."
            f"Expected at least {n}, found {flat.size}")
        flat = flat[:n]
        h = ctypes.c_void_p()
        check(lib.wg_buf_create_init(device._ctx.handle, flat.ctypes.data_as(ctypes.c_void_p), flat.nbytes, int(self.usage),
                                     ctypes.byref(h)))
        return GpuTensor(device._ctx, h.value, self.shape, dt, self.usage)

    def build_bytes(self, device: Device, data: bytes, dtype=np.float32) -> "GpuTensor":
        buf = np.frombuffer(data, dtype=np.uint8)
        h = ctypes.c_void_p()
        check(lib.wg_buf_create_init(device._ctx.handle, buf.ctypes.data_as(ctypes.c_void_p), buf.nbytes, int(self.usage),
                                     ctypes.byref(h)))
        return GpuTensor(device._ctx, h.value, self.shape, np.dtype(dtype), self.usage)


    def build_uninit_encased(self, device: Device, item_dtype) -> "GpuTensor":
        return self.build(device, np.dtype(item_dtype))

    def build_encase(self, device: Device, data) -> "GpuTensor":
        arr = np.ascontiguousarray(data)
        assert arr.size >= self.len(), (
            "Incorrect number of elements provided for initializing Tensor."
            f"Expected at least {self.len()}, found {arr.size}")
        return self.build_bytes(device, arr.reshape(-1)[: self.len()].tobytes(), arr.dtype)


class GpuBuffer:

    def __init__(self, ctx: _Ctx, handle, nbytes: int):
        self._ctx, self._h, self.size = ctx, handle, int(nbytes)

    def device_ptr(self) -> int:
        return lib.wg_buf_device_ptr(self._h) or 0

    def destroy(self):
        h = getattr(self, "_h", None)
        if h:
            if self._ctx.handle:
                lib.wg_buf_destroy(h)
            self._h = None

    __del__ = destroy


class GpuTensor:

    def __init__(self, ctx: _Ctx, handle: int, shape: Sequence[int], dtype: np.dtype, usage=BufferUsages.STORAGE, owned=True):
        self._ctx = ctx
        self._h = ctypes.c_void_p(handle)
        self._shape = tuple(int(s) for s in shape)
        self.dtype = np.dtype(dtype)
        self.usage = usage
        self._keepalive = None

    @staticmethod
    def wrap(device: Device, device_ptr: int, shape: Sequence[int], dtype=np.float32, keepalive=None) -> "GpuTensor":
        dt = np.dtype(dtype)
        h = ctypes.c_void_p()
        check(lib.wg_buf_wrap(device._ctx.handle, ctypes.c_void_p(device_ptr), _prod(shape) * dt.itemsize, ctypes.byref(h)))
        t = GpuTensor(device._ctx, h.value, shape, dt)
        t._keepalive = keepalive
        return t

    def __del__(self):
        h = getattr(self, "_h", None)
        if h:
            if self._ctx.handle:
                lib.wg_buf_destroy(h)
            self._h = None

    def destroy(self):
        self.__del__()

    @property
    def DIM(self) -> int:
        return len(self._shape)

    def is_empty(self) -> bool:
        return self.len() == 0

    def len(self) -> int:
        return _prod(self._shape)
# ... 276 lines not shown
```

Measured before the change: 1480.

## Add split-K finish units for tail tiles in dynamic f16 tile queue

Adds an optional finishing phase to the dynamic m16 tile queue. The last few tiles per XCD are split along K into chained units that pass fp32 partials through a workspace and wait on per-slot flags, which is meant to shorten the wave-quantization tail. The queue now resets itself on device: the last idle workgroup zeroes the counters and bumps an epoch, so the per-launch hipMemsetAsync is dropped. Surplus workgroups are sized as a fraction of the claim count. Finish mode is off by default (kFinishBySize=false, knob -1), so by default the changes are the removed memset and the new self-reset path.

New measurement: 1482 (median of 2 runs). About the same (+0.1%).

```diff
diff --git a/include/wgebra_hip.h b/include/wgebra_hip.h
--- a/include/wgebra_hip.h
+++ b/include/wgebra_hip.h
@@ -99,10 +99,13 @@
     WG_TUNE_GEMVT_LDS = 7,
     WG_TUNE_F16_CONT = 8,
     WG_TUNE_RM_TR_NATIVE = 9,
-    WG_TUNE_COUNT_ = 10
+    WG_TUNE_F16_FINISH = 10,
+    WG_TUNE_COUNT_ = 11
 } wg_tuning;
 int wg_ctx_set_tuning(wg_ctx *ctx, wg_tuning key, int value);
 int wg_ctx_f16_balance_info(const wg_ctx *ctx, double *rel8, int *valid, uint32_t *updates, uint32_t *balanced_launches);
+int wg_debug_f16_queue_words(wg_ctx *ctx, uint64_t *words11, int *have);
+int wg_debug_f16_finish_units(uint32_t tiles, uint32_t stages, uint32_t fin_tiles, uint32_t fin_units, uint32_t *units, uint32_t capacity, uint32_t *nunits);
 int wg_debug_f16_balance_plan(const double *rel8, uint32_t tiles, uint32_t stages, int forced, uint32_t *units, uint32_t capacity, uint32_t *nunits,
                               uint32_t *nworkgroups);
 typedef struct wg_gemm16_query {
@@ -119,6 +122,7 @@
     uint32_t recording;
     uint32_t bal_valid;
     uint32_t padded;
+    int32_t finish;
 } wg_gemm16_query;
 typedef enum wg_gemm16_leaf {
     WG_GEMM16_SKINNY = 0,
@@ -144,6 +148,7 @@
     uint32_t c_seed;
     int32_t status;
     char message[128];
+    uint32_t fin_tiles, fin_units;
 } wg_gemm16_plan;
 int wg_debug_gemm16_plan(const wg_gemm16_query *query, const char *prefix, wg_gemm16_plan *plan, char *tags, size_t cap, wg_gemm16_query *inner);
 int wg_debug_gemm_out32_query(wg_gemm16_query *query);
diff --git a/wgmath_amd/_lib.py b/wgmath_amd/_lib.py
--- a/wgmath_amd/_lib.py
+++ b/wgmath_amd/_lib.py
@@ -15,7 +15,7 @@
 WG_COMM_ID_BYTES, WG_IPC_HANDLE_BYTES = 128, 96
 ABI_VERSION = 5
 WG_F32, WG_F16, WG_BF16 = 0, 1, 2
-WG_TUNE_F16_TILE, WG_TUNE_F16_SCHED, WG_TUNE_F32_SKINNY, WG_TUNE_F32_PANELS, WG_TUNE_F16_BALANCE, WG_TUNE_F32_MID, WG_TUNE_F32_MID_SPLIT, WG_TUNE_GEMVT_LDS, WG_TUNE_F16_CONT, WG_TUNE_RM_TR_NATIVE = range(10)
+WG_TUNE_F16_TILE, WG_TUNE_F16_SCHED, WG_TUNE_F32_SKINNY, WG_TUNE_F32_PANELS, WG_TUNE_F16_BALANCE, WG_TUNE_F32_MID, WG_TUNE_F32_MID_SPLIT, WG_TUNE_GEMVT_LDS, WG_TUNE_F16_CONT, WG_TUNE_RM_TR_NATIVE, WG_TUNE_F16_FINISH = range(11)
 
 
 class ViewShapeC(ctypes.Structure):
@@ -34,7 +34,8 @@
                 + [(n, ctypes.c_uint32) for n in ("panels", "panel_cols", "panel_n_main", "panel_n_tail")]
                 + [("panel_tail_cols", ctypes.c_uint32 * 8), ("cus", ctypes.c_uint32)]
                 + [(n, ctypes.c_int32) for n in ("tile", "sched", "cont", "balance")]
-                + [(n, ctypes.c_uint32) for n in ("uneven_xcds", "recording", "bal_valid", "padded")])
+                + [(n, ctypes.c_uint32) for n in ("uneven_xcds", "recording", "bal_valid", "padded")]
+                + [("finish", ctypes.c_int32)])
 
 
 GEMM16_LEAVES = ("skinny", "t256x128", "t128", "m16", "pad", "generic", "unsupported")
@@ -45,7 +46,8 @@
                 + [("workspace_bytes", ctypes.c_uint64)]
                 + [(n, ctypes.c_uint32) for n in ("cont", "queues", "nwg", "bal_eligible", "bal_calib", "bal_wanted", "tail", "tail_split", "tail_kps",
                                                    "Mp", "Kp", "a_ok", "b_ok", "c_ok", "c_seed")]
-                + [("status", ctypes.c_int32), ("message", ctypes.c_char * 128)])
+                + [("status", ctypes.c_int32), ("message", ctypes.c_char * 128)]
+                + [("fin_tiles", ctypes.c_uint32), ("fin_units", ctypes.c_uint32)])
 
 
 class Gemm32QueryC(ctypes.Structure):
@@ -237,6 +239,8 @@
         "wg_debug_f16_balance_plan": (ci, [ctypes.POINTER(ctypes.c_double), u32, u32, ci, ctypes.POINTER(u32), u32, ctypes.POINTER(u32), ctypes.POINTER(u32)]),
         "wg_debug_gemm16_plan": (ci, [ctypes.POINTER(Gemm16QueryC), cp, ctypes.POINTER(Gemm16PlanC), cp, sz, ctypes.POINTER(Gemm16QueryC)]),
         "wg_debug_gemm32_plan": (ci, [ctypes.POINTER(Gemm32QueryC), ctypes.POINTER(Gemm32PlanC), cp, sz, ctypes.POINTER(Gemm32QueryC)]),
+        "wg_debug_f16_finish_units": (ci, [u32, u32, u32, u32, ctypes.POINTER(u32), u32, ctypes.POINTER(u32)]),
+        "wg_debug_f16_queue_words": (ci, [vp, ctypes.POINTER(ctypes.c_uint64), ctypes.POINTER(ci)]),
         "wg_ctx_f16_balance_info": (ci, [vp, ctypes.POINTER(ctypes.c_double), ctypes.POINTER(ci), ctypes.POINTER(u32), ctypes.POINTER(u32)]),
         "wg_debug_views_overlap": (ci, [S, u64, S, u64, u32, ctypes.POINTER(ci)]),
         "wg_debug_take_path": (ci, [vp, cp, sz]),
diff --git a/wgmath_amd/csrc/gemm16_plan.hip b/wgmath_amd/csrc/gemm16_plan.hip
--- a/wgmath_amd/csrc/gemm16_plan.hip
+++ b/wgmath_amd/csrc/gemm16_plan.hip
@@ -17,6 +17,8 @@
 constexpr double kBalTileOverhead = 5.0;
 constexpr double kBalTakeOverhead = 8.5;
 constexpr double kBalGiveOverhead = 7.0;
+constexpr double kFinishTailTiles = 0.94;
+constexpr bool kFinishBySize = false;
 }
 
 uint32_t bal_plan(const double rel[8], uint32_t tiles, uint32_t S, bool forced, BalancePlan &bp) {
@@ -287,7 +289,21 @@
         const bool dyn = nsplit == 1 && nmats == 1 && (sched_env >= 0 ? sched_env != 0 : ntiles >= (uint32_t)((q.uneven_xcds ? 2 : WG_F16_SCHED_ROUNDS) * cus));
         if (dyn) {
             p.queues = 1;
-            p.nwg = (ntiles + ntiles / 8u + 7u) & ~7u;
+            const uint32_t whole_stages = K / 64u;
+            if (q.finish == 1 || (q.finish < 0 && kFinishBySize && sched_env < 0 && !q.uneven_xcds && ntiles >= (uint32_t)(WG_F16_SCHED_ROUNDS * cus))) {
+                uint32_t f = ((uint32_t)std::ceil(kFinishTailTiles * (double)cus) + 7u) / 8u;
+                if (f > 32u) f = 32u;
+                if (f > ntiles / 8u) f = ntiles / 8u;
+                uint32_t u = whole_stages / 3u;
+                if (u > wg16::kFinMaxUnits) u = wg16::kFinMaxUnits;
+                if (f && u) { p.fin_tiles = f; p.fin_units = u; }
+            }
+            const uint32_t claims = ntiles + 8u * p.fin_tiles * (p.fin_units ? p.fin_units - 1u : 0u);
+#ifndef WG_F16_SURPLUS_32NDS
+#define WG_F16_SURPLUS_32NDS 4
+#endif
+            const uint32_t surplus = (uint32_t)((uint64_t)WG_F16_SURPLUS_32NDS * claims / 32u);
+            p.nwg = (claims + (surplus < 8u ? 8u : surplus) + 7u) & ~7u;
         }
         const int bal_knob = q.balance;
         const uint32_t S = K / 64u;
@@ -339,7 +355,7 @@
     case WG_GEMM16_T128: add("%s.t128/ns=%u", p.nsplit); break;
     case WG_GEMM16_M16:
         if (p.cont) add("%s.cont");
-        else add("%s.m16%s/ns=%u", bal_on ? "bal" : p.queues ? "q" : "", p.nsplit);
+        else add("%s.m16%s/ns=%u", bal_on ? "bal" : p.queues ? (p.fin_tiles ? "qf" : "q") : "", p.nsplit);
         if (p.tail) { add("%s.m16tail/ns=%u", p.tail_split); add("%s.tail_reduce"); }
         break;
     case WG_GEMM16_PAD: add("%s.pad%s>", p.c_ok ? "" : p.c_seed ? "/c=seed" : "/c"); break;
@@ -368,6 +384,21 @@
     return WG_OK;
 }
 
+extern "C" int wg_debug_f16_finish_units(uint32_t tiles, uint32_t stages, uint32_t fin_tiles, uint32_t fin_units, uint32_t *units, uint32_t capacity, uint32_t *nunits) {
+    if (!nunits || (capacity && !units)) return wg_set_error(WG_ERR_INVALID_ARG, "wg_debug_f16_finish_units: NULL argument");
+    if (fin_tiles > tiles / 8u || fin_tiles > 32u || fin_units > wg16::kFinMaxUnits || (fin_units && stages < 3u * fin_units))
+        return wg_set_error(WG_ERR_INVALID_ARG, "wg_debug_f16_finish_units: %u tiles x %u units of %u tiles x %u stages", fin_tiles, fin_units, tiles, stages);
+    uint32_t n = 0;
+    for (uint32_t t = 0;; ++t) {
+        uint32_t tile, mode, kb, ns, in, out;
+        if (!wg16::fin_decode(tiles, fin_tiles, fin_units, stages, t, tile, mode, kb, ns, in, out)) break;
+        if (n < capacity) { uint32_t *u = units + 6u * n; u[0] = tile; u[1] = mode; u[2] = kb; u[3] = mode == 2u ? stages - kb : ns; u[4] = in; u[5] = out; }
+        ++n;
+    }
+    *nunits = n;
+    return WG_OK;
+}
+
 extern "C" int wg_debug_gemm16_plan(const wg_gemm16_query *query, const char *prefix, wg_gemm16_plan *plan, char *tags, size_t cap, wg_gemm16_query *inner) {
     if (!query || !prefix || !plan || (cap && !tags)) return wg_set_error(WG_ERR_INVALID_ARG, "wg_debug_gemm16_plan: NULL argument");
     *plan = gemm16_plan(*query);
diff --git a/wgmath_amd/csrc/gemm_f16.hip b/wgmath_amd/csrc/gemm_f16.hip
--- a/wgmath_amd/csrc/gemm_f16.hip
+++ b/wgmath_amd/csrc/gemm_f16.hip
@@ -66,8 +66,8 @@
 constexpr uint32_t M16_BIAS = 3072;
 
 template <bool TRANS_A>
-__device__ __forceinline__ void m16_tile(const GemmArgs &g, const uint32_t bid, char *const smem, const uint32_t unit_mode = 0, uint32_t unit_kb = 0,
-                                         uint32_t unit_ns = 0, const uint32_t unit_pair = 0) {
+__device__ __forceinline__ void m16_tile(const GemmArgs &g, const uint32_t bid, char *const smem, const uint32_t unit_mode, uint32_t unit_kb,
+                                         uint32_t unit_ns, const uint32_t unit_pair, const uint32_t unit_out, const uint32_t unit_epoch) {
     const int lane = threadIdx.x & 63;
     const int wave = __builtin_amdgcn_readfirstlane(threadIdx.x >> 6);
     const int wm = wave >> 1, wn = wave & 1;
@@ -117,11 +117,11 @@
     uint32_t k_begin = split * g.k_per_split;
     uint32_t K_loc = split + 1u == g.nsplit ? g.K - k_begin : g.k_per_split;
     bool from_partial = false;
-    if (unit_mode == 2) {
+    if (unit_mode >= 2) {
         if (threadIdx.x == 0) {
             const uint64_t t0 = __builtin_amdgcn_s_memrealtime();
             uint32_t ok = 1;
-            while (__hip_atomic_load(g.bal.flags + unit_pair, __ATOMIC_RELAXED, __HIP_MEMORY_SCOPE_SYSTEM) != g.bal.epoch) {
+            while (__hip_atomic_load(g.bal.flags + unit_pair, __ATOMIC_RELAXED, __HIP_MEMORY_SCOPE_SYSTEM) != unit_epoch) {
                 __builtin_amdgcn_s_sleep(16);
                 if (__builtin_amdgcn_s_memrealtime() - t0 > 100000ull) { ok = 0; break; }
             }
@@ -134,7 +134,8 @@
     }
     uint32_t rem = 0, rem_k0 = 0;
     if (unit_mode == 1) { k_begin = 0; K_loc = unit_ns * 64u; rem = g.K & 63u; rem_k0 = g.K - rem; }
-    else if (unit_mode == 2 && from_partial) { k_begin = unit_kb * 64u; K_loc = (g.K & ~63u) - k_begin; }
+    else if (unit_mode >= 2 && from_partial) { k_begin = unit_kb * 64u; K_loc = unit_mode == 3 ? unit_ns * 64u : (g.K & ~63u) - k_begin; }
+    else if (unit_mode == 3) { k_begin = 0; K_loc = (unit_kb + unit_ns) * 64u; rem = g.K & 63u; rem_k0 = g.K - rem; }
     else {
         if (unit_mode == 2) { k_begin = 0; K_loc = g.K; }
         rem = K_loc & 63u; K_loc -= rem; rem_k0 = k_begin + K_loc;
@@ -152,7 +153,7 @@
     float alpha = g.alpha, beta = g.beta;
     uint32_t ldc = g.ldc, c_stream = g.c_stream;
     uint32_t *bal_flag = g.bal.flags + unit_pair;
-    uint32_t bal_epoch = g.bal.epoch;
+    uint32_t bal_epoch = unit_epoch;
     unsigned long long *calib = g.calib;
     asm volatile("" : "+s"(C), "+s"(part), "+s"(alpha), "+s"(beta), "+s"(ldc), "+s"(c_stream), "+s"(bal_flag), "+s"(bal_epoch), "+s"(calib));
 
@@ -589,8 +590,8 @@
 
     const bool full_tile = (m0 + BM <= g.M) && (n0 + BN <= g.N);
     const uint32_t row0 = m0 + 128u * wm + 8u * kg;
-    if (g.tail_tiles > 0 || unit_mode == 1) {
-        float *P = unit_mode == 1 ? part : part + ((uint64_t)split * g.tail_tiles + bid) * 65536u;
+    if (g.tail_tiles > 0 || (unit_mode & 1u)) {
+        float *P = (unit_mode & 1u) ? part + ((int64_t)unit_out - (int64_t)unit_pair) * 65536 : part + ((uint64_t)split * g.tail_tiles + bid) * 65536u;
 #pragma unroll
         for (int u = 0; u < 8; ++u) {
             const uint32_t cl = 128u * wn + 16u * u + i16;
@@ -603,12 +604,12 @@
             }
         }
         asm volatile("s_waitcnt vmcnt(0)" ::: "memory");
-        if (unit_mode == 1) {
+        if (unit_mode & 1u) {
             __syncthreads();
             if (threadIdx.x == 0) {
                 __builtin_amdgcn_fence(__ATOMIC_RELEASE, "agent");
                 asm volatile("s_waitcnt vmcnt(0)" ::: "memory");
-                __hip_atomic_store(bal_flag, bal_epoch, __ATOMIC_RELAXED, __HIP_MEMORY_SCOPE_SYSTEM);
+                __hip_atomic_store(bal_flag + ((int32_t)unit_out - (int32_t)unit_pair), bal_epoch, __ATOMIC_RELAXED, __HIP_MEMORY_SCOPE_SYSTEM);
             }
         }
         return;
@@ -749,14 +750,15 @@
 #endif
 }
 
-static __device__ uint32_t m16_acquire_tile(const GemmArgs &g) {
+static __device__ void m16_acquire_tile(const GemmArgs &g, volatile uint32_t *claim) {
     const uint32_t x = __builtin_amdgcn_s_getreg((20 << 0) | (0 << 6) | (3 << 11)) & 7u;
-    const uint32_t q = g.sched_tiles / 8u, r = g.sched_tiles % 8u;
+    const uint32_t q = g.sched_tiles / 8u - g.fin_tiles, r = g.sched_tiles % 8u;
     auto len = [&](uint32_t v) { return q + (v < r ? 1u : 0u); };
+    claim[1] = 0;
     unsigned long long old = atomicAdd(&g.sched[16u * x], 1ull);
     uint32_t lo = (uint32_t)old, hi = (uint32_t)(old >> 32);
-    if (lo + hi < len(x)) return 8u * lo + x;
-    for (int attempt = 0; attempt < 64; ++attempt) {
+    if (lo + hi < len(x)) { claim[0] = 8u * lo + x; return; }
+    for (;;) {
         uint32_t best = 0, victim = 8;
         for (uint32_t v = 0; v < 8u; ++v) {
             if (v == x) continue;
@@ -764,29 +766,55 @@
             const uint32_t taken = (uint32_t)w + (uint32_t)(w >> 32), n = len(v);
             if (taken < n && n - taken > best) { best = n - taken; victim = v; }
         }
-        if (victim == 8u) return ~0u;
+        if (victim == 8u) break;
         old = atomicAdd(&g.sched[16u * victim], 1ull << 32);
         lo = (uint32_t)old; hi = (uint32_t)(old >> 32);
-        if (lo + hi < len(victim)) return 8u * (len(victim) - 1u - hi) + victim;
-    }
-    return ~0u;
+        if (lo + hi < len(victim)) { claim[0] = 8u * (len(victim) - 1u - hi) + victim; return; }
+    }
+    uint32_t units = 0;
+    if (g.fin_tiles) {
+        uint32_t epoch = (uint32_t)__hip_atomic_load(&g.sched[wg16::kQueueEpoch], __ATOMIC_RELAXED, __HIP_MEMORY_SCOPE_AGENT) + 1u;
+        asm volatile("" : "+v"(epoch) : : "memory");
+        const uint32_t ticket = (uint32_t)atomicAdd(&g.sched[wg16::kQueueTicket], 1ull);
+        uint32_t tile, mode, kb, ns, in, out;
+        units = 8u * g.fin_tiles * g.fin_units;
+        if (ticket < units && wg16::fin_decode(g.sched_tiles, g.fin_tiles, g.fin_units, g.K / 64u, ticket, tile, mode, kb, ns, in, out)) {
+            claim[0] = tile; claim[1] = mode; claim[2] = kb; claim[3] = ns; claim[4] = in; claim[5] = out; claim[6] = epoch;
+            return;
+        }
+    }
+    claim[0] = ~0u;
+    const uint32_t claims = g.sched_tiles + (units ? units - 8u * g.fin_tiles : 0u);
+    const unsigned long long left = atomicAdd(&g.sched[wg16::kQueueLeft], 1ull);
+    if (left + 1ull == (unsigned long long)(gridDim.x - claims)) {
+        const unsigned long long epoch = __hip_atomic_load(&g.sched[wg16::kQueueEpoch], __ATOMIC_RELAXED, __HIP_MEMORY_SCOPE_AGENT);
+        for (uint32_t v = 0; v < 10u; ++v) __hip_atomic_store(&g.sched[16u * v], 0ull, __ATOMIC_RELAXED, __HIP_MEMORY_SCOPE_AGENT);
+        if (g.fin_tiles) __hip_atomic_store(&g.sched[wg16::kQueueEpoch], epoch + 1ull, __ATOMIC_RELAXED, __HIP_MEMORY_SCOPE_AGENT);
+    }
 }
 
 template <bool TRANS_A>
 __global__ __launch_bounds__(256, 1) void WG16_SYM(gemm_, _m16_kernel)(GemmArgs g) {
     __shared__ __attribute__((aligned(16))) char smem[160 * 1024];
     uint32_t bid = blockIdx.x;
-    uint32_t mode = 0, kb = 0, ns = 0, pair = 0;
+    uint32_t mode = 0, kb = 0, ns = 0, pair = 0, out = 0, epoch = g.bal.epoch;
     if (g.sched) {
-        if (threadIdx.x == 0) *reinterpret_cast<volatile uint32_t *>(smem) = m16_acquire_tile(g);
+        volatile uint32_t *claim = reinterpret_cast<volatile uint32_t *>(smem);
+        if (threadIdx.x == 0) m16_acquire_tile(g, claim);
         __syncthreads();
-        bid = __builtin_amdgcn_readfirstlane(*reinterpret_cast<volatile uint32_t *>(smem));
+        bid = __builtin_amdgcn_readfirstlane(claim[0]);
+        mode = __builtin_amdgcn_readfirstlane(claim[1]);
+        if (mode) {
+            kb = __builtin_amdgcn_readfirstlane(claim[2]); ns = __builtin_amdgcn_readfirstlane(claim[3]);
+            pair = __builtin_amdgcn_readfirstlane(claim[4]); out = __builtin_amdgcn_readfirstlane(claim[5]); epoch = __builtin_amdgcn_readfirstlane(claim[6]);
+        }
         __syncthreads();
         if (bid == ~0u) return;
     } else if (g.bal.on) {
         if (!bal_decode(g.bal, blockIdx.x, g.K / 64u, bid, mode, kb, ns, pair)) return;
-    }
-    m16_tile<TRANS_A>(g, bid, smem, mode, kb, ns, pair);
+        out = pair;
+    }
+    m16_tile<TRANS_A>(g, bid, smem, mode, kb, ns, pair, out, epoch);
 }
 
 
@@ -1333,10 +1361,17 @@
     if (p.queues) {
         if (!ctx->tile_queues) {
             if (ctx->recording) return wg_set_error(WG_ERR_WORKSPACE, "Gemm: the tile queues are needed while recording: run the call once outside the recording first");
-            WG_HIP_TRY(hipMalloc((void **)&ctx->tile_queues, 8 * 128));
-        }
-        WG_HIP_TRY(hipMemsetAsync(ctx->tile_queues, 0, 8 * 128, ctx->stream));
+            WG_HIP_TRY(hipMalloc((void **)&ctx->tile_queues, wg16::kQueueBytes));
+            WG_HIP_TRY(hipMemsetAsync(ctx->tile_queues, 0, wg16::kQueueBytes, ctx->stream));
+        }
         gm.sched = ctx->tile_queues; gm.sched_tiles = ntiles;
+        if (p.fin_tiles && p.fin_units > 1u) {
+            void *ws = nullptr;
+            if (int rc = wg_ctx_bal_workspace(ctx, (size_t)8u * p.fin_tiles * (p.fin_units - 1u) * 65536u * sizeof(float), &ws)) return rc;
+            gm.bal.part = (float *)ws;
+            gm.bal.flags = (uint32_t *)((char *)ctx->tile_queues + wg16::kQueueFlagsOffset);
+        }
+        gm.fin_tiles = p.fin_tiles; gm.fin_units = p.fin_units;
     }
     uint32_t nwg = p.nwg;
     if (p.bal_eligible) {
@@ -1455,6 +1490,7 @@
     }
     q.cus = (uint32_t)(ctx->compute_units > 0 ? ctx->compute_units : 256);
     q.tile = ctx->tuning[WG_TUNE_F16_TILE]; q.sched = ctx->tuning[WG_TUNE_F16_SCHED]; q.cont = ctx->tuning[WG_TUNE_F16_CONT]; q.balance = ctx->tuning[WG_TUNE_F16_BALANCE];
+    q.finish = ctx->tuning[WG_TUNE_F16_FINISH];
     q.uneven_xcds = ctx->uneven_xcds; q.recording = ctx->recording; q.bal_valid = ctx->bal.valid; q.padded = padded;
     if constexpr (kOut32) q = gemm16_out32_query(q);
     const wg_gemm16_plan p = gemm16_plan(q);
@@ -1470,7 +1506,7 @@
     g.c_stream = p.c_stream; g.a_nt = p.a_nt;
     if constexpr (kOut32) g.c_stream = gemm16_c_stream(q, sizeof(wg16_out_t));
     g.tile_base = 0; g.tail_tiles = 0;
-    g.sched = nullptr; g.sched_tiles = 0;
+    g.sched = nullptr; g.sched_tiles = 0; g.fin_tiles = g.fin_units = 0;
     g.calib = nullptr; g.bal = BalancePlan{}; g.panel = PanelArgs{};
     if (p.leaf == WG_GEMM16_UNSUPPORTED) return p.message[0] ? wg_set_error(p.status, "%s", p.message) : p.status;
     if (p.leaf == WG_GEMM16_PAD) return run_pad(ctx, q, p, out, m1, m2);
diff --git a/wgmath_amd/csrc/gemm_f16_common.hpp b/wgmath_amd/csrc/gemm_f16_common.hpp
--- a/wgmath_amd/csrc/gemm_f16_common.hpp
+++ b/wgmath_amd/csrc/gemm_f16_common.hpp
@@ -104,6 +104,23 @@
         }
     return true;
 }
+
+constexpr uint32_t kFinMaxUnits = 4, kFinMaxSlots = 8u * 32u * (kFinMaxUnits - 1u);
+constexpr uint32_t kQueueLeft = 16u * 8u, kQueueTicket = 16u * 9u, kQueueEpoch = 16u * 10u, kQueueFlagsOffset = 2048u, kQueueBytes = kQueueFlagsOffset + 4u * kFinMaxSlots;
+__host__ __device__ inline bool fin_decode(uint32_t ntiles, uint32_t F, uint32_t U, uint32_t S, uint32_t ticket, uint32_t &tile, uint32_t &mode, uint32_t &kb,
+                                           uint32_t &ns, uint32_t &in, uint32_t &out) {
+    const uint32_t n = 8u * F;
+    if (n == 0u || U == 0u || ticket >= n * U) return false;
+    const uint32_t phase = ticket / n, r = ticket % n, x = r / F, j = r % F;
+    const uint32_t len = ntiles / 8u + (x < ntiles % 8u ? 1u : 0u);
+    tile = 8u * (len - F + j) + x;
+    kb = (uint32_t)((uint64_t)phase * S / U);
+    ns = (uint32_t)((uint64_t)(phase + 1u) * S / U) - kb;
+    mode = U == 1u ? 0u : phase == 0u ? 1u : phase + 1u == U ? 2u : 3u;
+    in = r * (U - 1u) + (phase ? phase - 1u : 0u);
+    out = phase + 1u < U ? r * (U - 1u) + phase : in;
+    return true;
+}
 }
 
 namespace WG16_NS {
@@ -133,6 +150,7 @@
     uint32_t a_nt;
     uint32_t tile_base, tail_tiles;
     unsigned long long *sched; uint32_t sched_tiles;
+    uint32_t fin_tiles, fin_units;
     unsigned long long *calib;
     BalancePlan bal;
     PanelArgs panel;
diff --git a/wgmath_amd/csrc/runtime.hip b/wgmath_amd/csrc/runtime.hip
--- a/wgmath_amd/csrc/runtime.hip
+++ b/wgmath_amd/csrc/runtime.hip
@@ -69,6 +69,17 @@
 int wg_ctx_stage_workspace(wg_ctx *ctx, size_t bytes, void **out) {
     return grow_scratch(ctx, &ctx->stage_workspace, &ctx->stage_workspace_bytes, bytes, "staging workspace", out);
 }
+int wg_debug_f16_queue_words(wg_ctx *ctx, uint64_t *words11, int *have) {
+    if (!ctx || !words11 || !have) return wg_set_error(WG_ERR_INVALID_ARG, "wg_debug_f16_queue_words: NULL argument");
+    for (int i = 0; i < 11; ++i) words11[i] = 0;
+    *have = ctx->tile_queues ? 1 : 0;
+    if (!ctx->tile_queues) return WG_OK;
+    WG_HIP_TRY(hipSetDevice(ctx->device));
+    WG_HIP_TRY(hipStreamSynchronize(ctx->stream));
+    WG_HIP_TRY(hipMemcpy2D(words11, 8, ctx->tile_queues, 128, 8, 11, hipMemcpyDeviceToHost));
+    return WG_OK;
+}
+
 int wg_ctx_bal_workspace(wg_ctx *ctx, size_t bytes, void **out) {
     return grow_scratch(ctx, &ctx->bal.scratch, &ctx->bal.scratch_bytes, bytes, "balance workspace", out);
 }
@@ -138,7 +149,8 @@
     static const struct { const char *env; wg_tuning key; } knobs[] = {
         { "WG_F16_TILE", WG_TUNE_F16_TILE }, { "WG_F16_SCHED", WG_TUNE_F16_SCHED }, { "WG_F32_SKINNY", WG_TUNE_F32_SKINNY },
         { "WG_F32_PANELS", WG_TUNE_F32_PANELS }, { "WG_F16_BALANCE", WG_TUNE_F16_BALANCE }, { "WG_F32_MID", WG_TUNE_F32_MID }, { "WG_F32_MID_SPLIT", WG_TUNE_F32_MID_SPLIT },
-        { "WG_GEMVT_LDS", WG_TUNE_GEMVT_LDS }, { "WG_F16_CONT", WG_TUNE_F16_CONT }, { "WG_RM_TR_NATIVE", WG_TUNE_RM_TR_NATIVE } };
+        { "WG_GEMVT_LDS", WG_TUNE_GEMVT_LDS }, { "WG_F16_CONT", WG_TUNE_F16_CONT }, { "WG_RM_TR_NATIVE", WG_TUNE_RM_TR_NATIVE },
+        { "WG_F16_FINISH", WG_TUNE_F16_FINISH } };
     for (const auto &k : knobs)
         if (const char *v = getenv(k.env)) {
             if (wg_ctx_set_tuning(ctx, k.key, atoi(v)) != WG_OK) fprintf(stderr, "libwgebra_hip: ignoring %s=%s (%s)\n", k.env, v, wg_last_error_string());
diff --git a/wgmath_amd/csrc/wg_internal.hpp b/wgmath_amd/csrc/wg_internal.hpp
--- a/wgmath_amd/csrc/wg_internal.hpp
+++ b/wgmath_amd/csrc/wg_internal.hpp
@@ -53,7 +53,7 @@
         void *scratch = nullptr;
         size_t scratch_bytes = 0;
     } bal;
-    int tuning[WG_TUNE_COUNT_] = { 0, -1, -1, -1, 0, -1, 0, 0, -1, -1 };
+    int tuning[WG_TUNE_COUNT_] = { 0, -1, -1, -1, 0, -1, 0, 0, -1, -1, -1 };
     void *debug_stamps = nullptr;
     bool debug_clock_open = false;
     uint32_t lds_attr_bits = 0;
diff --git a/wgmath_amd/wgcore.py b/wgmath_amd/wgcore.py
--- a/wgmath_amd/wgcore.py
+++ b/wgmath_amd/wgcore.py
@@ -325,7 +325,8 @@
         self._ctx.close()
 
     _TUNING = {"f16_tile": _lib.WG_TUNE_F16_TILE, "f16_sched": _lib.WG_TUNE_F16_SCHED, "f32_skinny": _lib.WG_TUNE_F32_SKINNY,
-               "f32_panels": _lib.WG_TUNE_F32_PANELS, "f16_balance": _lib.WG_TUNE_F16_BALANCE, "f32_mid": _lib.WG_TUNE_F32_MID, "f32_mid_split": _lib.WG_TUNE_F32_MID_SPLIT, "gemvt_lds": _lib.WG_TUNE_GEMVT_LDS, "f16_cont": _lib.WG_TUNE_F16_CONT, "rm_tr_native": _lib.WG_TUNE_RM_TR_NATIVE}
+               "f32_panels": _lib.WG_TUNE_F32_PANELS, "f16_balance": _lib.WG_TUNE_F16_BALANCE, "f32_mid": _lib.WG_TUNE_F32_MID, "f32_mid_split": _lib.WG_TUNE_F32_MID_SPLIT, "gemvt_lds": _lib.WG_TUNE_GEMVT_LDS, "f16_cont": _lib.WG_TUNE_F16_CONT, "rm_tr_native": _lib.WG_TUNE_RM_TR_NATIVE,
+               "f16_finish": _lib.WG_TUNE_F16_FINISH}
 
     def set_tuning(self, knob: str, value: int) -> int:
         old = self.get_tuning(knob)
@@ -336,6 +337,13 @@
         rel, valid, upd, n = (ctypes.c_double * 8)(), ctypes.c_int(), ctypes.c_uint32(), ctypes.c_uint32()
         check(lib.wg_ctx_f16_balance_info(self._ctx.handle, rel, ctypes.byref(valid), ctypes.byref(upd), ctypes.byref(n)))
         return {"rel": [round(float(v), 4) for v in rel], "valid": bool(valid.value), "updates": upd.value, "balanced_launches": n.value}
+
+    def f16_queue_words(self) -> dict:
+        w, have = (ctypes.c_uint64 * 11)(), ctypes.c_int()
+        check(lib.wg_debug_f16_queue_words(self._ctx.handle, w, ctypes.byref(have)))
+        if not have.value:
+            return None
+        return {"queues": [int(v) for v in w[:8]], "left": int(w[8]), "ticket": int(w[9]), "epoch": int(w[10])}
 
     def take_path(self) -> str:
         buf = ctypes.create_string_buffer(1024)
```
